# yhlleo/DWC-GAN

Hardware: AMD Instinct MI355X
Metric: CelebA 128x128 training images/sec (higher is better)
Workload: dtype f32; 1 GPU; BASELINE configs[1]: CelebA-shaped 128x128, per-GPU batch 16, fp32, full iteration (dis_update + gen_update + EMA + LR step), vgg_w=0, stride-1 3x3 / 5x5 and stride-2 4x4 layers (forward, data and weight gradient) as fp32-accurate TWO-plane f16 split products on the f16 MFMA (hi + lo 2^-11 per operand, per-tensor power-of-two scales, 3 products per multiply-add, matrix-core partial sums flushed to; image_size=128, per_gpu_batch=16, global_batch=16, parallelism=dp1

## Files before the change

dwc-gan_amd/csrc/conv_fold.h:

```cpp
#pragma once
#include "conv_geom.h"

namespace {

__device__ __forceinline__ int reflect_src(int p, int n, int pad, int (&out)[3]) {
    int c = 0;
    out[c++] = p + pad;
    if (p >= 1 && p <= pad) out[c++] = pad - p;
    if (p >= n - 1 - pad && p <= n - 2) out[c++] = pad + 2 * (n - 1) - p;
    return c;
}

template <typename T>
__global__ void fold_reflect_kernel(const T* __restrict__ gp, T* __restrict__ dx, int B, int H, int W, int C4, int pad,
                                    int Wp) {
    const size_t idx = (size_t)blockIdx.x * blockDim.x + threadIdx.x;
    const size_t total = (size_t)B * H * W * C4;
    if (idx >= total) return;
    const int c = idx % C4;
    size_t r = idx / C4;
    const int w = r % W;
    r /= W;
    const int h = r % H;
    const int n = r / H;
    const int Hp = H + 2 * pad;
    int hs[3], ws[3];
    const int nh = reflect_src(h, H, pad, hs), nw = reflect_src(w, W, pad, ws);
    f32x4 s = {0.f, 0.f, 0.f, 0.f};
    for (int a = 0; a < nh; ++a)
        for (int b = 0; b < nw; ++b) s += ld4(gp, ((size_t)(n * Hp + hs[a]) * Wp + ws[b]) * C4 + c);
    st4(dx, idx, s);
}

template <typename T>
int fold_reflect(const T* gp, T* dx, int B, int H, int W, int C4, int pad, int Wp, hipStream_t st) {
    const size_t total = (size_t)B * H * W * C4;
    hipLaunchKernelGGL(fold_reflect_kernel<T>, dim3((unsigned)((total + 255) / 256)), dim3(256), 0, st, gp, dx, B, H, W, C4, pad, Wp);
    DWC_LAUNCH_CHECK();
    return DWC_OK;
}

template <typename T>
__global__ __launch_bounds__(256) void fold_band_kernel(const T* __restrict__ gp, T* __restrict__ dx, int B, int H, int W, int CV,
                                                        int pad, int Wp) {
    constexpr int V = VecOf<T>::V;
    const size_t idx = (size_t)blockIdx.x * 256 + threadIdx.x;
    const int rows_done = 2 * pad, rest = H - 2 * pad;
    const int band = rows_done * W + rest * 2 * pad;
    const size_t total = (size_t)B * band * CV;
    if (idx >= total) return;
    const int c = idx % CV;
    size_t r = idx / CV;
    const int q = r % band;
    const size_t n = r / band;
    const int Hp = H + 2 * pad;
    int h, w;
    if (q < rows_done * W) {
        const int br = q / W;
        w = q - br * W;
        h = br < pad ? 1 + br : H - 1 - pad + (br - pad);
    } else {
        const int q2 = q - rows_done * W;
        const int hr = q2 / (2 * pad), k = q2 - hr * 2 * pad;
        h = hr == 0 ? 0 : (hr == rest - 1 ? H - 1 : pad + hr);
        w = k < pad ? 1 + k : W - 1 - pad + (k - pad);
    }
    int hs[3], ws[3];
    const int nh = reflect_src(h, H, pad, hs), nw = reflect_src(w, W, pad, ws);
    if (nh * nw == 1) return;
    const size_t o = ((n * H + h) * (size_t)W + w) * CV + c;
    float s[V], v[V];
    ldv(dx, o, s);
    for (int a = 0; a < nh; ++a)
        for (int b = 0; b < nw; ++b) {
            if (a == 0 && b == 0) continue;
            ldv(gp, ((n * Hp + hs[a]) * (size_t)Wp + ws[b]) * CV + c, v);
#pragma unroll
            for (int k = 0; k < V; ++k) s[k] += v[k];
        }
    stv(dx, o, s);
}

template <typename T>
int fold_band(const T* gp, T* dx, int B, int H, int W, int C, int pad, hipStream_t st) {
    const int CV = C / VecOf<T>::V;
    const size_t band_items = (size_t)B * (2 * pad * W + (H - 2 * pad) * 2 * pad) * CV;
    hipLaunchKernelGGL(fold_band_kernel<T>, dim3((unsigned)((band_items + 255) / 256)), dim3(256), 0, st, gp, dx, B, H, W, CV, pad,
                       W + 2 * pad);
    DWC_LAUNCH_CHECK();
    return DWC_OK;
}

template <typename T>
__global__ void fold_ring_kernel(T* __restrict__ dx, const float* __restrict__ ring, size_t off_bottom, size_t off_left,
                                 size_t off_right, int parts, size_t part_stride, int B, int H, int W, int C4, int pad) {
    const size_t idx = (size_t)blockIdx.x * blockDim.x + threadIdx.x;
    const int band = 2 * pad * (W + H);
    const size_t total = (size_t)B * band * C4;
    if (idx >= total) return;
    const int c = idx % C4;
    size_t r = idx / C4;
    const int q = r % band;
    const int n = r / band;
    int h, w;
    if (q < 2 * pad * W) {
        const int br = q / W;
        w = q - br * W;
        h = br < pad ? 1 + br : H - 1 - pad + (br - pad);
    } else {
        const int q2 = q - 2 * pad * W, bc = q2 / H;
        h = q2 - bc * H;
        w = bc < pad ? 1 + bc : W - 1 - pad + (bc - pad);
        if ((h >= 1 && h <= pad) || (h >= H - 1 - pad && h <= H - 2)) return;
    }
    if (h < 0 || h >= H || w < 0 || w >= W) return;
    const int Wp = W + 2 * pad;
    int hs[3], ws[3];
    const int nh = reflect_src(h, H, pad, hs), nw = reflect_src(w, W, pad, ws);
    const size_t o = ((size_t)(n * H + h) * W + w) * C4 + c;
    f32x4 s = ld4(dx, o);
    for (int a = 0; a < nh; ++a)
        for (int b = 0; b < nw; ++b) {
            if (a == 0 && b == 0) continue;
            const int rh = hs[a], rw = ws[b];
            size_t e;
            if (rh < pad) e = ((size_t)(n * pad + rh) * Wp + rw) * C4;
            else if (rh >= pad + H) e = off_bottom / 4 + ((size_t)(n * pad + rh - pad - H) * Wp + rw) * C4;
            else if (rw < pad) e = off_left / 4 + ((size_t)(n * H + rh - pad) * pad + rw) * C4;
            else e = off_right / 4 + ((size_t)(n * H + rh - pad) * pad + rw - pad - W) * C4;
            for (int p = 0; p < parts; ++p) s += ld4(ring + p * part_stride, e + c);
        }
    st4(dx, o, s);
}

template <typename T>
int fold_ring(T* dx, const float* ring, const SameDgrad& f, int B, int H, int W, int C, int pad, hipStream_t st) {
    const size_t total = (size_t)B * 2 * pad * (W + H) * (C / 4);
    hipLaunchKernelGGL(fold_ring_kernel<T>, dim3((unsigned)((total + 255) / 256)), dim3(256), 0, st, dx, ring, f.ring_elems[0],
                       f.ring_elems[0] + f.ring_elems[1], f.ring_elems[0] + f.ring_elems[1] + f.ring_elems[2], f.parts, f.ring_total,
                       B, H, W, C / 4, pad);
    DWC_LAUNCH_CHECK();
    return DWC_OK;
}

template <typename T>
__global__ __launch_bounds__(256) void splitk_reduce_kernel(const float* __restrict__ part, T* __restrict__ dst,
                                                            const float* __restrict__ bias, size_t total4, size_t stride4, int splits,
                                                            int N, int act) {
    const int nq = N >> 2;
    for (size_t i = (size_t)blockIdx.x * blockDim.x + threadIdx.x; i < total4; i += (size_t)gridDim.x * blockDim.x) {
        f32x4 s = ld4(part, i);
        for (int z = 1; z < splits; ++z) s += ld4(part, (size_t)z * stride4 + i);
        const int c4 = i % nq;
        if (bias) s += ld4(bias, c4);
#pragma unroll
        for (int k = 0; k < 4; ++k) s[k] = dwc_act_apply(s[k], act, c4 * 4 + k);
        st4(dst, i, s);
    }
}

template <typename T>
int splitk_reduce(const float* part, T* dst, const float* bias, size_t dst_elems, int splits, int N, int act, hipStream_t st) {
    const size_t total4 = dst_elems / 4;
    size_t blocks = (total4 + 255) / 256;
    if (blocks > 2048) blocks = 2048;
    hipLaunchKernelGGL(splitk_reduce_kernel<T>, dim3((unsigned)blocks), dim3(256), 0, st, part, dst, bias, total4, total4, splits, N, act);
    DWC_LAUNCH_CHECK();
    return DWC_OK;
}

template <typename T>
__global__ void weight_prepare_fwd_kernel(const float* __restrict__ w, T* __restrict__ out, int Cout, int Cin, int KHW,
                                          int cout_pad, int cin_pad, int Kp) {
    const size_t idx = (size_t)blockIdx.x * blockDim.x + threadIdx.x;
    if (idx >= (size_t)cout_pad * Kp) return;
    const int k = idx % Kp, co = idx / Kp;
    const int ci = k % cin_pad, tap = k / cin_pad;
    float v = 0.f;
    if (co < Cout && ci < Cin && tap < KHW) v = w[((size_t)co * Cin + ci) * KHW + tap];
    out[idx] = (T)v;
}

template <typename T>
__global__ void weight_prepare_dgrad_kernel(const float* __restrict__ w, T* __restrict__ out, int Cout, int Cin, int KH, int KW,
                                            int stride, int cout_pad, int cin_pad, int Kp) {
    const size_t idx = (size_t)blockIdx.x * blockDim.x + threadIdx.x;
    const size_t per_class = (size_t)cin_pad * Kp;
    const int classes = stride == 1 ? 1 : 4;
    if (idx >= per_class * classes) return;
    const int cls = idx / per_class;
    const size_t r = idx % per_class;
    const int k = r % Kp, ci = r / Kp;
    const int co = k % cout_pad, tapo = k / cout_pad;
    int kh, kw;
    bool ok = co < Cout && ci < Cin;
    if (stride == 1) {
        ok = ok && tapo < KH * KW;
        kh = KH - 1 - tapo / KW;
        kw = KW - 1 - tapo % KW;
    } else {
        ok = ok && tapo < 4;
        kh = (cls >> 1) + 2 * (tapo >> 1);
        kw = (cls & 1) + 2 * (tapo & 1);
    }
    out[idx] = (T)(ok ? w[((size_t)co * Cin + ci) * KH * KW + kh * KW + kw] : 0.f);
}

inline int weight_prepared_kp(int taps, int c_pad, int bk) { return (taps * c_pad + bk - 1) / bk * bk; }

inline size_t weight_prepared_elems(int KH, int KW, int stride, int cout_pad, int cin_pad, int for_dgrad, int bk) {
    if (!for_dgrad) return (size_t)cout_pad * weight_prepared_kp(KH * KW, cin_pad, bk);
    if (stride == 1) return (size_t)cin_pad * weight_prepared_kp(KH * KW, cout_pad, bk);
    return (size_t)4 * cin_pad * weight_prepared_kp(4, cout_pad, bk);
}

template <typename T>
int weight_prepare_fwd(const float* w, T* out, int Cout, int Cin, int KH, int KW, int cout_pad, int cin_pad, int bk, hipStream_t st) {
    const int Kp = weight_prepared_kp(KH * KW, cin_pad, bk);
    const size_t total = (size_t)cout_pad * Kp;
    hipLaunchKernelGGL(weight_prepare_fwd_kernel<T>, dim3((unsigned)((total + 255) / 256)), dim3(256), 0, st, w, out, Cout, Cin, KH * KW,
                       cout_pad, cin_pad, Kp);
    DWC_LAUNCH_CHECK();
    return DWC_OK;
}

template <typename T>
int weight_prepare_dgrad(const float* w, T* out, int Cout, int Cin, int KH, int KW, int stride, int cout_pad, int cin_pad, int bk,
                         hipStream_t st) {
    const int Kp = weight_prepared_kp(stride == 1 ? KH * KW : 4, cout_pad, bk);
    const size_t total = (size_t)(stride == 1 ? 1 : 4) * cin_pad * Kp;
    hipLaunchKernelGGL(weight_prepare_dgrad_kernel<T>, dim3((unsigned)((total + 255) / 256)), dim3(256), 0, st, w, out, Cout, Cin, KH, KW,
                       stride, cout_pad, cin_pad, Kp);
    DWC_LAUNCH_CHECK();
    return DWC_OK;
}

}
```

dwc-gan_amd/csrc/conv_igemm.hip:

```cpp
#include <type_traits>

#include <atomic>

#include "conv_im2col_entry.h"

namespace {

constexpr int BK = 32;


__device__ __attribute__((aligned(16))) float g_zero_page[64];

#ifdef DWC_CLOCK_PROBE
__device__ unsigned long long g_clock_probe[2];
struct ClockProbe {
    long long c0, r0;
    __device__ ClockProbe() : c0(clock64()), r0(wall_clock64()) {}
    __device__ ~ClockProbe() {
        if (blockIdx.x == 0 && blockIdx.y == 0 && blockIdx.z == 0 && threadIdx.x == 0) {
            atomicAdd(&g_clock_probe[0], (unsigned long long)(clock64() - c0));
            atomicAdd(&g_clock_probe[1], (unsigned long long)(wall_clock64() - r0));
        }
    }
};
#define DWC_PROBE() ClockProbe clock_probe_
#else
#define DWC_PROBE()
#endif

__device__ __forceinline__ void lds_dma_barrier() {
    asm volatile("s_waitcnt vmcnt(0)" ::: "memory");
    __syncthreads();
}

typedef __bf16 gx3_bf16x8 __attribute__((ext_vector_type(8)));
typedef unsigned gx3_u32x4 __attribute__((ext_vector_type(4)));

__device__ __forceinline__ void gx3_split8(const f32x4& a, const f32x4& b, gx3_bf16x8& p0, gx3_bf16x8& p1, gx3_bf16x8& p2) {
    unsigned h[8], m[8], l[8];
#pragma unroll
    for (int k = 0; k < 8; ++k) {
        const float v = k < 4 ? a[k] : b[k - 4];
        const unsigned hb = __float_as_uint(v) & 0xffff0000u;
        const float r = v - __uint_as_float(hb);
        const unsigned mb = __float_as_uint(r) & 0xffff0000u;
        const float q = r - __uint_as_float(mb);
        h[k] = hb; m[k] = mb; l[k] = __float_as_uint(q);
    }
    gx3_u32x4 u0, u1, u2;
#pragma unroll
    for (int k = 0; k < 4; ++k) {
        u0[k] = __builtin_amdgcn_perm(h[2 * k + 1], h[2 * k], 0x07060302u);
        u1[k] = __builtin_amdgcn_perm(m[2 * k + 1], m[2 * k], 0x07060302u);
        u2[k] = __builtin_amdgcn_perm(l[2 * k + 1], l[2 * k], 0x07060302u);
    }
    p0 = __builtin_bit_cast(gx3_bf16x8, u0);
    p1 = __builtin_bit_cast(gx3_bf16x8, u1);
    p2 = __builtin_bit_cast(gx3_bf16x8, u2);
}

template <int BM, int BN, int WM, int WN, int TM, int TN, bool X3 = false>
__device__ __forceinline__ void conv_gemm_body(const Gather& g, const float* __restrict__ wmat, const Scatter& o,
                                               const float* __restrict__ bias, int act, int tiles_n, int kt0, int kt1_in,
                                               size_t part_offset, bool partial, int oph, int opw, int bid, int nb) {
    static_assert(WM * WN == 4 && WM * TM * 32 == BM && WN * TN * 32 == BN, "tile shape");
    constexpr int A_PASSES = BM / 32, B_PASSES = BN / 32;
    constexpr int A_TILE = BM * BK, B_TILE = BN * BK;
    __shared__ __attribute__((aligned(16))) float smem[2 * (A_TILE + B_TILE)];
    float* sA = smem;
    float* sB = smem + 2 * A_TILE;

    const int t = threadIdx.x;
    const int lane = t & 63, wave = __builtin_amdgcn_readfirstlane(t >> 6);
    const int wm = wave / WN, wn = wave % WN;
    const int l31 = lane & 31, hi = lane >> 5;

    if (nb >= 16) {
        const int q = nb >> 3, r = nb & 7, x = bid & 7, y = bid >> 3;
        bid = (x < r ? x * (q + 1) : r * (q + 1) + (x - r) * q) + y;
    }
    const int tile_m = bid / tiles_n, tile_n = bid % tiles_n;
    const int m0 = tile_m * BM, n0 = tile_n * BN;

    const int arow = t >> 3;
    const int acol = (((t & 7) ^ ((arow >> 1) & 7))) * 4;
    int a_bh[A_PASSES], a_bw[A_PASSES], a_img[A_PASSES];
    const int ohw = g.OH * g.OW;
#pragma unroll
    for (int i = 0; i < A_PASSES; ++i) {
        const int mm = min(m0 + arow + 32 * i, g.M - 1);
        const int n = mm / ohw;
        const int rem = mm - n * ohw;
        const int oh = rem / g.OW, ow = rem - oh * g.OW;
        a_bh[i] = oh * g.mul_h + g.off_h;
        a_bw[i] = ow * g.mul_w + g.off_w;
        a_img[i] = n * g.SH * g.SW;
    }
    const int Kp = (g.K + BK - 1) / BK * BK;
    const float* b_ptr[B_PASSES];
#pragma unroll
    for (int p = 0; p < B_PASSES; ++p) b_ptr[p] = wmat + (size_t)min(n0 + arow + 32 * p, o.N - 1) * Kp + acol;

    const int nk_all = Kp / BK;
    const int kt1 = min(nk_all, kt1_in);
    const int n_taps = g.KH * g.KW;

    int cur_tap = -1;
    const float* a_src[A_PASSES];
    const bool tap_uniform = g.SC >= BK;
    auto row_sources = [&](int tap, int ci) {
        int kh = (tap * g.kw_magic) >> 16;
        int kw = tap - kh * g.KW;
        if (g.tap_t) {
            const int x = kh;
            kh = kw;
            kw = x;
        }
#pragma unroll
        for (int i = 0; i < A_PASSES; ++i) {
            int h = a_bh[i] + kh * g.kstep;
            int w = a_bw[i] + kw * g.kstep;
            bool inb = true;
            if (g.reflect) {
                h = reflect_idx(h, g.SH);
                w = reflect_idx(w, g.SW);
            } else {
                inb = h >= 0 && h < g.SH && w >= 0 && w < g.SW;
                h = min(max(h, 0), g.SH - 1);
                w = min(max(w, 0), g.SW - 1);
            }
            const float* p = (const float*)g.src + ((a_img[i] + h * g.SW + w) << g.logSC) + ci;
            a_src[i] = inb ? p : g_zero_page;
        }
    };
    auto stage_slab = [&](int kt, int buf) {
        int coff;
        if (tap_uniform) {
            const int kg0 = kt * BK;
            const int tap = min(kg0 >> g.logSC, n_taps - 1);
            if (tap != cur_tap) {
                row_sources(tap, acol);
                cur_tap = tap;
            }
            coff = kg0 & (g.SC - 1);
        } else {
            const int kg = kt * BK + acol;
            row_sources(min(kg >> g.logSC, n_taps - 1), kg & (g.SC - 1));
            coff = 0;
        }
        float* la = sA + buf * A_TILE + wave * (8 * BK);
        float* lb = sB + buf * B_TILE + wave * (8 * BK);
#pragma unroll
        for (int i = 0; i < A_PASSES; ++i) {
            const float* s = a_src[i];
            if (s != g_zero_page) s += coff;
            __builtin_amdgcn_global_load_lds((const __attribute__((address_space(1))) void*)s,
                                             (__attribute__((address_space(3))) void*)(la + i * 32 * BK), 16, 0, 0);
        }
#pragma unroll
        for (int p = 0; p < B_PASSES; ++p)
            __builtin_amdgcn_global_load_lds((const __attribute__((address_space(1))) void*)(b_ptr[p] + kt * BK),
                                             (__attribute__((address_space(3))) void*)(lb + p * 32 * BK), 16, 0, 0);
    };

    f32x16 acc[TM][TN];
#pragma unroll
    for (int i = 0; i < TM; ++i)
#pragma unroll
        for (int j = 0; j < TN; ++j)
#pragma unroll
            for (int r = 0; r < 16; ++r) acc[i][j][r] = 0.f;

    const int fsw = (l31 >> 1) & 7;
    int frag_off[4];
#pragma unroll
    for (int q = 0; q < 4; ++q) frag_off[q] = ((2 * q + hi) ^ fsw) * 4;
    const int a_row = (wm * TM * 32 + l31) * BK;
    const int b_row = (wn * TN * 32 + l31) * BK;
    f32x4 fa[2][TM], fb[2][TN];
    auto load_frags = [&](int set, int buf, int q) {
        const float* a = sA + buf * A_TILE + a_row + frag_off[q];
        const float* b = sB + buf * B_TILE + b_row + frag_off[q];
#pragma unroll
        for (int i = 0; i < TM; ++i) fa[set][i] = *reinterpret_cast<const f32x4*>(a + i * 32 * BK);
#pragma unroll
        for (int n = 0; n < TN; ++n) fb[set][n] = *reinterpret_cast<const f32x4*>(b + n * 32 * BK);
    };
    auto mfma_group = [&](int set) {
#pragma unroll
        for (int j = 0; j < 4; ++j)
#pragma unroll
            for (int i = 0; i < TM; ++i)
#pragma unroll
                for (int n = 0; n < TN; ++n)
                    acc[i][n] = __builtin_amdgcn_mfma_f32_32x32x2f32(fa[set][i][j], fb[set][n][j], acc[i][n], 0, 0, 0);
    };

    if constexpr (X3) {
        static_assert(TM * TN <= 2, "split accumulators: at most two 32x32 tiles per wave");
        f32x16 lo[TM][TN];
#pragma unroll
        for (int i = 0; i < TM; ++i)
#pragma unroll
            for (int j = 0; j < TN; ++j)
#pragma unroll
                for (int r = 0; r < 16; ++r) lo[i][j][r] = 0.f;
        int xoff[2][2];
#pragma unroll
        for (int ss = 0; ss < 2; ++ss)
#pragma unroll
            for (int e = 0; e < 2; ++e) xoff[ss][e] = ((4 * ss + 2 * hi + e) ^ fsw) * 4;
        gx3_bf16x8 pa[3][TM], pb[3][TN];
        auto frags_x3 = [&](int buf, int ss) {
            const float* a = sA + buf * A_TILE + a_row;
            const float* b = sB + buf * B_TILE + b_row;
#pragma unroll
            for (int i = 0; i < TM; ++i)
                gx3_split8(*reinterpret_cast<const f32x4*>(a + i * 32 * BK + xoff[ss][0]),
                           *reinterpret_cast<const f32x4*>(a + i * 32 * BK + xoff[ss][1]), pa[0][i], pa[1][i], pa[2][i]);
#pragma unroll
            for (int n = 0; n < TN; ++n)
                gx3_split8(*reinterpret_cast<const f32x4*>(b + n * 32 * BK + xoff[ss][0]),
                           *reinterpret_cast<const f32x4*>(b + n * 32 * BK + xoff[ss][1]), pb[0][n], pb[1][n], pb[2][n]);
        };
        auto mfma_x3 = [&]() {
            constexpr int TA[6] = {0, 1, 0, 2, 1, 0}, TB[6] = {0, 0, 1, 0, 1, 2};
#pragma unroll
            for (int term = 0; term < 6; ++term)
#pragma unroll
                for (int i = 0; i < TM; ++i)
#pragma unroll
                    for (int n = 0; n < TN; ++n) {
                        if (term == 0) acc[i][n] = __builtin_amdgcn_mfma_f32_32x32x16_bf16(pa[TA[term]][i], pb[TB[term]][n], acc[i][n], 0, 0, 0);
                        else lo[i][n] = __builtin_amdgcn_mfma_f32_32x32x16_bf16(pa[TA[term]][i], pb[TB[term]][n], lo[i][n], 0, 0, 0);
                    }
        };
        if (kt0 < kt1) {
            stage_slab(kt0, 0);
            lds_dma_barrier();
            int buf = 0;
            for (int kt = kt0; kt < kt1; ++kt) {
                if (kt + 1 < kt1) stage_slab(kt + 1, buf ^ 1);
                frags_x3(buf, 0);
                mfma_x3();
                frags_x3(buf, 1);
                lds_dma_barrier();
                mfma_x3();
                buf ^= 1;
            }
        }
#pragma unroll
        for (int i = 0; i < TM; ++i)
#pragma unroll
            for (int j = 0; j < TN; ++j)
#pragma unroll
                for (int r = 0; r < 16; ++r) acc[i][j][r] += lo[i][j][r];
    } else if (kt0 < kt1) {
        stage_slab(kt0, 0);
        lds_dma_barrier();
        int buf = 0;
        load_frags(0, 0, 0);
        for (int kt = kt0; kt < kt1; ++kt) {
            const bool more = kt + 1 < kt1;
            if (more) stage_slab(kt + 1, buf ^ 1);
            load_frags(1, buf, 1);
            mfma_group(0);
            load_frags(0, buf, 2);
            mfma_group(1);
            load_frags(1, buf, 3);
            mfma_group(0);
            lds_dma_barrier();
            if (more) load_frags(0, buf ^ 1, 0);
            mfma_group(1);
            buf ^= 1;
        }
    }

    float* dst = (float*)o.dst + part_offset;
    const float slope = dwc_act_slope(act);
    float bcol[TN];
#pragma unroll
    for (int n = 0; n < TN; ++n) bcol[n] = 0.f;
    if (bias && !partial) {
#pragma unroll
        for (int n = 0; n < TN; ++n) bcol[n] = bias[min(n0 + (wn * TN + n) * 32 + l31, o.N - 1)];
    }
    auto store = [&](auto general) {
#pragma unroll
        for (int i = 0; i < TM; ++i) {
#pragma unroll
            for (int r = 0; r < 16; ++r) {
                const int row = (wm * TM + i) * 32 + (r & 3) + 8 * (r >> 2) + 4 * hi;
                const int m = m0 + row;
                if (m >= g.M) continue;
                const int n_img = m / ohw;
                const int rem = m - n_img * ohw;
                const int oh = rem / g.OW, ow = rem - oh * g.OW;
                const int py = oh * o.os + oph, px = ow * o.os + opw;
                float* drow = dst + (((size_t)n_img * o.OHf + py) * o.OWf + px) * o.N;
                if (o.crop && !partial) {
                    const int yy = py - o.crop, xx = px - o.crop;
                    if ((unsigned)yy < (unsigned)o.IH && (unsigned)xx < (unsigned)o.IW)
                        drow = (float*)o.inner + (((size_t)n_img * o.IH + yy) * o.IW + xx) * o.N;
                }
#pragma unroll
                for (int n = 0; n < TN; ++n) {
                    const int col = n0 + (wn * TN + n) * 32 + l31;
                    if (col < o.N) {
                        float v = acc[i][n][r];
                        if (!partial) {
                            v += bcol[n];
                            if constexpr (decltype(general)::value) v = dwc_act_apply(v, act, col);
                            else v = dwc_act_simple(v, slope);
                        }
                        drow[col] = v;
                    }
                }
            }
        }
    };
    if (dwc_act_is_simple(act)) store(std::false_type{});
    else store(std::true_type{});
}

template <int BM, int BN, int WM, int WN, int TM, int TN, bool X3 = false>
__global__ __launch_bounds__(256) void conv_gemm_kernel(Gather g, const float* __restrict__ wmat, size_t w_class_stride,
                                                             Scatter o, const float* __restrict__ bias, int act, int tiles_n,
                                                             int kt_per_split, size_t part_stride) {
    DWC_PROBE();
    const int cls = blockIdx.z, split = blockIdx.y;
    conv_gemm_body<BM, BN, WM, WN, TM, TN, X3>(g, wmat + (size_t)cls * w_class_stride, o, bias, act, tiles_n, split * kt_per_split,
                                           (split + 1) * kt_per_split, (size_t)split * part_stride, part_stride != 0, cls >> 1,
                                           cls & 1, blockIdx.x, gridDim.x);
}

template <int BM, int BN, int WM, int WN, int TM, int TN, bool X3 = false>
__global__ __launch_bounds__(256) void conv_gemm_strips_kernel(StripSet ss) {
    const Strip& s = ss.s[blockIdx.z];
    if ((int)blockIdx.x >= s.tiles) return;
    const int kt0 = s.kt0 + blockIdx.y * ss.kt_per_part;
    conv_gemm_body<BM, BN, WM, WN, TM, TN, X3>(s.g, (const float*)s.w, s.o, nullptr, DWC_ACT_NONE, s.tiles_n, kt0, min(s.kt1, kt0 + ss.kt_per_part),
                                           blockIdx.y * ss.part_stride, false, s.oph, s.opw, blockIdx.x, s.tiles);
}

template <int BN, int WM, int WN, int TM, int TN, bool X3 = false>
__global__ __launch_bounds__(256) void conv_wgrad_kernel(Gather g, const float* __restrict__ dy, int N, float* __restrict__ slab,
                                                         int m_chunk, int splits_per_class = 0, size_t src_class_stride = 0,
                                                         size_t dy_class_stride = 0) {
    static_assert(WM * WN == 4 && WM * TM * 32 == 128 && WN * TN * 32 == BN, "tile shape");
    DWC_PROBE();
    constexpr int A_TILE = 32 * 128, B_TILE = 32 * BN;
    __shared__ __attribute__((aligned(16))) float smem[2 * (A_TILE + B_TILE)];
    float* sA = smem;
    float* sB = smem + 2 * A_TILE;
    const int t = threadIdx.x;
    const int lane = t & 63, wave = t >> 6;
    const int wm = wave / WN, wn = wave % WN;
    const int l31 = lane & 31, hi = lane >> 5;
    const int k0 = blockIdx.x * 128, n0 = blockIdx.y * BN;
    int split = blockIdx.z;
    if (splits_per_class > 0) {
        const int cls = blockIdx.z / splits_per_class;
        split = blockIdx.z - cls * splits_per_class;
        g.src = (const float*)g.src + (size_t)cls * src_class_stride;
        dy += (size_t)cls * dy_class_stride;
    }
    const int m_begin = split * m_chunk;
    const int m_end = min(g.M, m_begin + m_chunk);

    const int kg = k0 + (t & 31) * 4;
    const int tap = min(kg >> g.logSC, g.KH * g.KW - 1);
    const int ci = kg & (g.SC - 1);
    const int kh = (tap * g.kw_magic) >> 16;
    const int kw = tap - kh * g.KW;
    const int dh = kh * g.kstep + g.off_h, dw = kw * g.kstep + g.off_w;
    const int arow = t >> 5;
    constexpr int B_F4 = BN / 4;
    constexpr int B_ROWS_PER_PASS = 256 / B_F4;
    constexpr int B_PASSES = 32 / B_ROWS_PER_PASS;
    const int brow = t / B_F4, bcol = (t % B_F4) * 4;
    const int ohw = g.OH * g.OW;

    const int bcol_c = min(n0 + bcol, N - 4);
    const int wave_u = __builtin_amdgcn_readfirstlane(wave);
    auto stage_slab = [&](int mb, int buf) {
        float* la = sA + buf * A_TILE + wave_u * 256;
        float* lb = sB + buf * B_TILE + wave_u * 256;
#pragma unroll
        for (int i = 0; i < 4; ++i) {
            const int m = min(mb + arow + 8 * i, g.M - 1);
            int n, oh, ow;
            if (g.logOW >= 0) {
                n = m >> g.logOHW;
                const int rem = m & (ohw - 1);
                oh = rem >> g.logOW;
                ow = rem & (g.OW - 1);
            } else {
                n = m / ohw;
                const int rem = m - n * ohw;
                oh = rem / g.OW;
                ow = rem - oh * g.OW;
            }
            const int h = reflect_idx(oh * g.mul_h + dh, g.SH);
            const int w = reflect_idx(ow * g.mul_w + dw, g.SW);
            const float* s = (const float*)g.src + (((n * g.SH + h) * g.SW + w) << g.logSC) + ci;
            __builtin_amdgcn_global_load_lds((const __attribute__((address_space(1))) void*)s,
                                             (__attribute__((address_space(3))) void*)(la + i * 8 * 128), 16, 0, 0);
        }
#pragma unroll
        for (int p = 0; p < B_PASSES; ++p) {
            const int m = mb + brow + p * B_ROWS_PER_PASS;
            const float* s = m < m_end ? dy + (size_t)m * N + bcol_c : g_zero_page;
            __builtin_amdgcn_global_load_lds((const __attribute__((address_space(1))) void*)s,
                                             (__attribute__((address_space(3))) void*)(lb + p * B_ROWS_PER_PASS * BN), 16, 0, 0);
        }
    };

    f32x16 acc[TM][TN];
#pragma unroll
    for (int i = 0; i < TM; ++i)
#pragma unroll
        for (int j = 0; j < TN; ++j)
#pragma unroll
            for (int r = 0; r < 16; ++r) acc[i][j][r] = 0.f;

    float av[2][4][TM], bv[2][4][TN];
    auto load_ops = [&](int set, int buf, int grp) {
        const float* a = sA + buf * A_TILE + (wm * TM) * 32 + l31;
        const float* b = sB + buf * B_TILE + (wn * TN) * 32 + l31;
#pragma unroll
        for (int s = 0; s < 4; ++s) {
            const int ml = 2 * (4 * grp + s) + hi;
#pragma unroll
            for (int i = 0; i < TM; ++i) av[set][s][i] = a[ml * 128 + i * 32];
#pragma unroll
            for (int n = 0; n < TN; ++n) bv[set][s][n] = b[ml * BN + n * 32];
        }
    };
    auto mfma_ops = [&](int set) {
#pragma unroll
        for (int s = 0; s < 4; ++s)
#pragma unroll
            for (int i = 0; i < TM; ++i)
#pragma unroll
                for (int n = 0; n < TN; ++n)
                    acc[i][n] = __builtin_amdgcn_mfma_f32_32x32x2f32(av[set][s][i], bv[set][s][n], acc[i][n], 0, 0, 0);
    };
    if constexpr (X3) {
        f32x16 lo[TM][TN];
#pragma unroll
        for (int i = 0; i < TM; ++i)
#pragma unroll
            for (int j = 0; j < TN; ++j)
#pragma unroll
                for (int r = 0; r < 16; ++r) lo[i][j][r] = 0.f;
        gx3_bf16x8 pa[3][TM], pb[3][TN];
        auto ops_x3 = [&](int buf, int ss) {
            const float* a = sA + buf * A_TILE + (wm * TM) * 32 + l31 + (16 * ss + 8 * hi) * 128;
            const float* b = sB + buf * B_TILE + (wn * TN) * 32 + l31 + (16 * ss + 8 * hi) * BN;
#pragma unroll
            for (int i = 0; i < TM; ++i)
                gx3_split8(f32x4{a[i * 32], a[128 + i * 32], a[2 * 128 + i * 32], a[3 * 128 + i * 32]},
                           f32x4{a[4 * 128 + i * 32], a[5 * 128 + i * 32], a[6 * 128 + i * 32], a[7 * 128 + i * 32]}, pa[0][i], pa[1][i],
                           pa[2][i]);
#pragma unroll
            for (int n = 0; n < TN; ++n)
                gx3_split8(f32x4{b[n * 32], b[BN + n * 32], b[2 * BN + n * 32], b[3 * BN + n * 32]},
                           f32x4{b[4 * BN + n * 32], b[5 * BN + n * 32], b[6 * BN + n * 32], b[7 * BN + n * 32]}, pb[0][n], pb[1][n],
                           pb[2][n]);
        };
        auto mfma_x3 = [&]() {
            constexpr int TA[6] = {0, 1, 0, 2, 1, 0}, TB[6] = {0, 0, 1, 0, 1, 2};
#pragma unroll
            for (int term = 0; term < 6; ++term)
#pragma unroll
                for (int i = 0; i < TM; ++i)
#pragma unroll
                    for (int n = 0; n < TN; ++n) {
                        if (term == 0) acc[i][n] = __builtin_amdgcn_mfma_f32_32x32x16_bf16(pa[TA[term]][i], pb[TB[term]][n], acc[i][n], 0, 0, 0);
                        else lo[i][n] = __builtin_amdgcn_mfma_f32_32x32x16_bf16(pa[TA[term]][i], pb[TB[term]][n], lo[i][n], 0, 0, 0);
                    }
        };
        if (m_begin < m_end) {
            stage_slab(m_begin, 0);
            lds_dma_barrier();
            int buf = 0;
            for (int mb = m_begin; mb < m_end; mb += 32) {
                if (mb + 32 < m_end) stage_slab(mb + 32, buf ^ 1);
                ops_x3(buf, 0);
                mfma_x3();
                ops_x3(buf, 1);
                lds_dma_barrier();
                mfma_x3();
                buf ^= 1;
            }
        }
#pragma unroll
        for (int i = 0; i < TM; ++i)
#pragma unroll
            for (int j = 0; j < TN; ++j)
#pragma unroll
                for (int r = 0; r < 16; ++r) acc[i][j][r] += lo[i][j][r];
    } else if (m_begin < m_end) {
        stage_slab(m_begin, 0);
        lds_dma_barrier();
        int buf = 0;
        load_ops(0, 0, 0);
        for (int mb = m_begin; mb < m_end; mb += 32) {
            const bool more = mb + 32 < m_end;
            if (more) stage_slab(mb + 32, buf ^ 1);
            load_ops(1, buf, 1);
            mfma_ops(0);
            load_ops(0, buf, 2);
            mfma_ops(1);
            load_ops(1, buf, 3);
            mfma_ops(0);
            lds_dma_barrier();
            if (more) load_ops(0, buf ^ 1, 0);
            mfma_ops(1);
            buf ^= 1;
        }
    }
    float* out = slab + (size_t)blockIdx.z * g.K * N;
#pragma unroll
    for (int i = 0; i < TM; ++i)
#pragma unroll
        for (int r = 0; r < 16; ++r) {
            const int k = k0 + (wm * TM + i) * 32 + (r & 3) + 8 * (r >> 2) + 4 * hi;
            if (k >= g.K) continue;
#pragma unroll
            for (int n = 0; n < TN; ++n) {
                const int col = n0 + (wn * TN + n) * 32 + l31;
                if (col < N) out[(size_t)k * N + col] = acc[i][n][r];
            }
        }
}


template <int BM, int BN, int WM, int WN, int TM, int TN, bool X3 = false>
void launch_variant(const Gather& g, const float* w, size_t wcs, int classes, const Scatter& o, const float* bias, int act,
                    const Plan& p, size_t part_stride, hipStream_t st) {
    const int tiles_m = (g.M + BM - 1) / BM, tiles_n = (o.N + BN - 1) / BN;
    hipLaunchKernelGGL((conv_gemm_kernel<BM, BN, WM, WN, TM, TN, X3>), dim3(tiles_m * tiles_n, p.splits, classes), dim3(256), 0, st,
                       g, w, wcs, o, bias, act, tiles_n, p.kt_per_split, part_stride);
}

static std::atomic<int> g_x3_mode{-1};
static int x3_mode() {
    int m = g_x3_mode.load(std::memory_order_relaxed);
    if (m < 0) {
        const int a = getenv("DWC_X3_GEMM") ? atoi(getenv("DWC_X3_GEMM")) : 1;
        const int b = getenv("DWC_X3_WGRAD") ? atoi(getenv("DWC_X3_WGRAD")) : 1;
        m = (a ? 1 : 0) | (b ? 2 : 0);
        g_x3_mode.store(m, std::memory_order_relaxed);
    }
    return m;
}
static bool wgrad_x3_on() { return (x3_mode() & 2) != 0; }
static bool gemm_x3_on(int K) { return (x3_mode() & 1) != 0 && K >= 128; }

struct Im2colF32 {
    typedef float T;
    static constexpr int BK = ::BK;
    static constexpr int MIN_LOG_C = 2;
    static constexpr int CH_MASK = 3;
    static constexpr bool HALF_STRIPS = false;
    static constexpr int WGRAD_SLAB_ROWS = 32;
    static constexpr int IMAGE_PX = 8;
    static constexpr int IMAGE_GROUPS = 1;
    static constexpr TileCand TILES[] = {{128, 128, 2, 1.0f}, {128, 64, 3, 0.85f}, {64, 64, 5, 0.72f}, {128, 32, 4, 0.5f}};
    static constexpr int SPLIT_BELOW = 2 * NUM_CU;

    static int launch_gemm(const Gather& g, const float* w, size_t w_class_stride, int classes, Scatter o, const float* bias, int act,
                           size_t dst_elems, void* ws, size_t ws_bytes, hipStream_t st) {
        Plan p = im2col_plan<Im2colF32>(g.M, o.N, g.K, classes);
        float* final_dst = (float*)o.dst;
        size_t part_stride = 0;
        if (p.splits > 1) {
            if (!ws || ws_bytes < gemm_ws_bytes(p, dst_elems)) {
                p.splits = 1;
                p.kt_per_split = (g.K + BK - 1) / BK;
            } else {
                o.dst = (float*)ws;
                part_stride = dst_elems;
            }
        }
        if (gemm_x3_on(g.K)) {
            if (p.bm == 128 && p.bn >= 64) launch_variant<128, 64, 2, 2, 2, 1, true>(g, w, w_class_stride, classes, o, bias, act, p, part_stride, st);
            else if (p.bm == 64 && p.bn == 64) launch_variant<64, 64, 2, 2, 1, 1, true>(g, w, w_class_stride, classes, o, bias, act, p, part_stride, st);
            else launch_variant<128, 32, 4, 1, 1, 1, true>(g, w, w_class_stride, classes, o, bias, act, p, part_stride, st);
        } else if (p.bm == 128 && p.bn == 128) launch_variant<128, 128, 2, 2, 2, 2>(g, w, w_class_stride, classes, o, bias, act, p, part_stride, st);
        else if (p.bm == 128 && p.bn == 64) launch_variant<128, 64, 2, 2, 2, 1>(g, w, w_class_stride, classes, o, bias, act, p, part_stride, st);
        else if (p.bm == 64 && p.bn == 64) launch_variant<64, 64, 2, 2, 1, 1>(g, w, w_class_stride, classes, o, bias, act, p, part_stride, st);
        else launch_variant<128, 32, 4, 1, 1, 1>(g, w, w_class_stride, classes, o, bias, act, p, part_stride, st);
        DWC_LAUNCH_CHECK();
        if (p.splits > 1) return splitk_reduce((const float*)ws, final_dst, bias, dst_elems, p.splits, o.N, act, st);
        return DWC_OK;
    }

    static int launch_strips(const StripSet& ss, int bm, dim3 grid, hipStream_t st, bool ) {
        if (bm != 64) return DWC_EINVAL;
        if (gemm_x3_on(ss.s[0].g.K)) hipLaunchKernelGGL((conv_gemm_strips_kernel<64, 64, 2, 2, 1, 1, true>), grid, dim3(256), 0, st, ss);
        else hipLaunchKernelGGL((conv_gemm_strips_kernel<64, 64, 2, 2, 1, 1>), grid, dim3(256), 0, st, ss);
        DWC_LAUNCH_CHECK();
        return DWC_OK;
    }

    static int wgrad_launch(const FwdGeom& f, const float* dy, float* dw_oihw, int Cin, int Cout, int KHW, int cin_real, int cout_real,
                            void* ws, size_t ws_bytes, hipStream_t st) {
        const Gather& g = f.g;
        int splits, chunk;
        if (!ws || ws_bytes < wgrad_ws_bytes(g.M, g.K, Cout, WGRAD_SLAB_ROWS, &splits, &chunk)) return DWC_EWORKSPACE;
        float* slab = (float*)ws;
        const int tk = (g.K + 127) / 128;
        if (wgrad_x3_on()) {
            if (Cout > 64)
                hipLaunchKernelGGL((conv_wgrad_kernel<128, 2, 2, 2, 2, true>), dim3(tk, (Cout + 127) / 128, splits), dim3(256), 0, st, g, dy,
                                   Cout, slab, chunk);
            else if (Cout > 32)
                hipLaunchKernelGGL((conv_wgrad_kernel<64, 2, 2, 2, 1, true>), dim3(tk, 1, splits), dim3(256), 0, st, g, dy, Cout, slab, chunk);
            else
                hipLaunchKernelGGL((conv_wgrad_kernel<32, 4, 1, 1, 1, true>), dim3(tk, 1, splits), dim3(256), 0, st, g, dy, Cout, slab, chunk);
        } else if (Cout > 64) {
            hipLaunchKernelGGL((conv_wgrad_kernel<128, 2, 2, 2, 2>), dim3(tk, (Cout + 127) / 128, splits), dim3(256), 0, st, g, dy,
                               Cout, slab, chunk);
        } else if (Cout > 32) {
            hipLaunchKernelGGL((conv_wgrad_kernel<64, 2, 2, 2, 1>), dim3(tk, 1, splits), dim3(256), 0, st, g, dy, Cout, slab, chunk);
        } else {
            hipLaunchKernelGGL((conv_wgrad_kernel<32, 4, 1, 1, 1>), dim3(tk, 1, splits), dim3(256), 0, st, g, dy, Cout, slab, chunk);
        }
        DWC_LAUNCH_CHECK();
        wgrad_reduce(slab, dw_oihw, splits, g.K, Cout, Cin, KHW, cin_real, cout_real, st);
        DWC_LAUNCH_CHECK();
        return DWC_OK;
    }

    static int fold_image(const float* dxp, float* dx, int B, int H, int W, int C, int pad, hipStream_t st) {
        return fold_reflect(dxp, dx, B, H, W, C / 4, pad, W + 2 * pad, st);
    }

    static bool band_args_bad(const void* dxp, const void* dx, int , int , int C) { return !dxp || !dx || C <= 0; }
};

}

#define DWC_F32_NAME(x) dwc_##x
DWC_IM2COL_EXPORTS(DWC_F32_NAME, Im2colF32, float)
#undef DWC_F32_NAME

extern "C" {

int dwc_version(void) { return DWC_ABI_VERSION; }

int dwc_x3_gemm_mode(int mode) {
    const int prev = x3_mode();
    if (mode >= 0) g_x3_mode.store(mode & 3, std::memory_order_relaxed);
    return prev;
}

int dwc_reflect_pad_adjoint_pitch(const float* dxp, float* dx, int B, int H, int W, int C, int pad, int pitch, void* stream) {
    if (B <= 0 || H <= 0 || W <= 0 || C <= 0 || (C & 3) || pad < 0 || pad >= H || pad >= W || pitch < W + 2 * pad) return DWC_EINVAL;
    return fold_reflect(dxp, dx, B, H, W, C / 4, pad, pitch, (hipStream_t)stream);
}

}

#ifdef DWC_CLOCK_PROBE
extern "C" int dwc_debug_clock_probe(unsigned long long* out, int reset) {
    if (hipMemcpyFromSymbol(out, HIP_SYMBOL(g_clock_probe), 16) != hipSuccess) return DWC_ELAUNCH;
    if (reset) {
        const unsigned long long z[2] = {0, 0};
        if (hipMemcpyToSymbol(HIP_SYMBOL(g_clock_probe), z, 16) != hipSuccess) return DWC_ELAUNCH;
    }
    return 0;
}
#endif
```

dwc-gan_amd/csrc/conv_im2col_entry.h:

```cpp
#pragma once
#include "conv_fold.h"

namespace {

template <class P>
Plan im2col_plan(int M, int N, int K, int classes) {
    return plan_gemm(M, N, K, classes, P::BK, P::TILES, P::SPLIT_BELOW);
}

template <class P>
size_t im2col_weight_prepared_elems(int Cout, int Cin, int KH, int KW, int stride, int cout_pad, int cin_pad, int for_dgrad) {
    return weight_prepared_elems(KH, KW, stride, cout_pad, cin_pad, for_dgrad, P::BK);
}

template <class P>
int im2col_weight_prepare_fwd(const float* w, void* out, int Cout, int Cin, int KH, int KW, int cout_pad, int cin_pad, void* stream) {
    if (cout_pad < Cout || cin_pad < Cin) return DWC_EINVAL;
    return weight_prepare_fwd(w, (typename P::T*)out, Cout, Cin, KH, KW, cout_pad, cin_pad, P::BK, (hipStream_t)stream);
}

template <class P>
int im2col_weight_prepare_dgrad(const float* w, void* out, int Cout, int Cin, int KH, int KW, int stride, int cout_pad, int cin_pad,
                                void* stream) {
    if (cout_pad < Cout || cin_pad < Cin) return DWC_EINVAL;
    if (stride == 2 && !(KH == 4 && KW == 4)) return DWC_EINVAL;
    if (stride != 1 && stride != 2) return DWC_EINVAL;
    return weight_prepare_dgrad(w, (typename P::T*)out, Cout, Cin, KH, KW, stride, cout_pad, cin_pad, P::BK, (hipStream_t)stream);
}

template <class P>
size_t im2col_fwd_ws_bytes(int B, int H, int W, int Cin, int Cout, int KH, int KW, int stride, int pad) {
    FwdGeom f;
    if (!fwd_geom(nullptr, nullptr, B, H, W, Cin, Cout, KH, KW, stride, pad, &f, P::MIN_LOG_C)) return 0;
    return gemm_ws_bytes(im2col_plan<P>(f.g.M, Cout, f.g.K, 1), f.dst_elems);
}

template <class P>
int im2col_fwd(const void* x, const void* w_prepared, const float* bias, void* y, int B, int H, int W, int Cin, int Cout, int KH,
               int KW, int stride, int pad, int act, void* ws, size_t ws_bytes, void* stream, int reflect) {
    FwdGeom f;
    if ((Cout & P::CH_MASK) || !fwd_geom(x, y, B, H, W, Cin, Cout, KH, KW, stride, pad, &f, P::MIN_LOG_C)) return DWC_EINVAL;
    f.g.reflect = reflect;
    return P::launch_gemm(f.g, (const typename P::T*)w_prepared, 0, 1, f.o, bias, act, f.dst_elems, ws, ws_bytes, (hipStream_t)stream);
}

template <class P>
int im2col_fwd_ex(const void* x, const void* w_prepared, const float* bias, void* y, int B, int H, int W, int Cin, int Cout, int KH,
                  int KW, int stride_h, int stride_w, int pad_h, int pad_w, int act, void* stream) {
    FwdGeom f;
    if ((Cout & P::CH_MASK) || !fwd_geom_ex(x, y, B, H, W, Cin, Cout, KH, KW, stride_h, stride_w, pad_h, pad_w, &f, P::MIN_LOG_C))
        return DWC_EINVAL;
    return P::launch_gemm(f.g, (const typename P::T*)w_prepared, 0, 1, f.o, bias, act, f.dst_elems, nullptr, 0, (hipStream_t)stream);
}

template <class P>
size_t im2col_bwd_data_zeropad_ws_bytes(int B, int H, int W, int Cin, int Cout, int KH, int KW, int pad) {
    FwdGeom f;
    if ((Cin & P::CH_MASK) || (Cout & P::CH_MASK) || !zeropad_dgrad_geom(nullptr, nullptr, B, H, W, Cin, Cout, KH, KW, pad, &f)) return 0;
    return gemm_ws_bytes(im2col_plan<P>(f.g.M, Cin, f.g.K, 1), f.dst_elems);
}

template <class P>
int im2col_bwd_data_zeropad(const void* dy, const void* w_dgrad, void* dx, int B, int H, int W, int Cin, int Cout, int KH, int KW,
                            int pad, void* ws, size_t ws_bytes, void* stream) {
    FwdGeom f;
    if ((Cin & P::CH_MASK) || (Cout & P::CH_MASK) || !zeropad_dgrad_geom(dy, dx, B, H, W, Cin, Cout, KH, KW, pad, &f)) return DWC_EINVAL;
    return P::launch_gemm(f.g, (const typename P::T*)w_dgrad, 0, 1, f.o, nullptr, DWC_ACT_NONE, f.dst_elems, ws, ws_bytes,
                          (hipStream_t)stream);
}

template <class P>
size_t im2col_bwd_data_ws_bytes(int B, int H, int W, int Cin, int Cout, int KH, int KW, int stride, int pad) {
    BwdGeom f;
    if (!bwd_geom(nullptr, nullptr, B, H, W, Cin, Cout, KH, KW, stride, pad, &f, P::BK, P::MIN_LOG_C)) return 0;
    return gemm_ws_bytes(im2col_plan<P>(f.g.M, Cin, f.g.K, f.classes), f.dst_elems);
}

template <class P>
int im2col_bwd_data(const void* dy, const void* w_dgrad, void* dxp, int B, int H, int W, int Cin, int Cout, int KH, int KW, int stride,
                    int pad, void* ws, size_t ws_bytes, void* stream) {
    BwdGeom f;
    if ((Cin & P::CH_MASK) || !bwd_geom(dy, dxp, B, H, W, Cin, Cout, KH, KW, stride, pad, &f, P::BK, P::MIN_LOG_C)) return DWC_EINVAL;
    return P::launch_gemm(f.g, (const typename P::T*)w_dgrad, f.wcs, f.classes, f.o, nullptr, DWC_ACT_NONE, f.dst_elems, ws, ws_bytes,
                          (hipStream_t)stream);
}

template <class P>
int im2col_reflect_pad_adjoint(const void* dxp, void* dx, int B, int H, int W, int C, int pad, void* stream) {
    if (B <= 0 || H <= 0 || W <= 0 || C <= 0 || (C & 3) || pad < 0 || pad >= H || pad >= W) return DWC_EINVAL;
    return P::fold_image((const typename P::T*)dxp, (typename P::T*)dx, B, H, W, C, pad, (hipStream_t)stream);
}

template <class P>
int im2col_reflect_pad_adjoint_band(const void* dxp, void* dx, int B, int H, int W, int C, int pad, void* stream) {
    if (P::band_args_bad(dxp, dx, B, H, C) || B <= 0 || (C & P::CH_MASK) || pad <= 0 || H < 2 * pad + 2 || W < 2 * pad + 2)
        return DWC_EINVAL;
    return fold_band((const typename P::T*)dxp, (typename P::T*)dx, B, H, W, C, pad, (hipStream_t)stream);
}

template <class P>
int im2col_bwd_data_fold(const void* dy, const void* w_dgrad, void* dxp, void* dx, int B, int H, int W, int Cin, int Cout, int KH,
                         int KW, int stride, int pad, void* ws, size_t ws_bytes, void* stream) {
    BwdGeom f;
    if ((Cin & P::CH_MASK) || pad <= 0 || !bwd_geom(dy, dxp, B, H, W, Cin, Cout, KH, KW, stride, pad, &f, P::BK, P::MIN_LOG_C))
        return DWC_EINVAL;
    if (H < 2 * pad + 2 || W < 2 * pad + 2 || H > 65535 - 2 * pad || B > 65535) return DWC_EINVAL;
    hipStream_t st = (hipStream_t)stream;
    const bool direct = im2col_plan<P>(f.g.M, f.o.N, f.g.K, f.classes).splits == 1;
    if (direct) {
        f.o.crop = pad; f.o.IH = H; f.o.IW = W; f.o.inner = dx;
    }
    const int rc = P::launch_gemm(f.g, (const typename P::T*)w_dgrad, f.wcs, f.classes, f.o, nullptr, DWC_ACT_NONE, f.dst_elems, ws,
                                  ws_bytes, st);
    if (rc != DWC_OK) return rc;
    if (!direct) return im2col_reflect_pad_adjoint<P>(dxp, dx, B, H, W, Cin, pad, stream);
    return fold_band((const typename P::T*)dxp, (typename P::T*)dx, B, H, W, Cin, pad, st);
}

template <class P>
size_t im2col_bwd_data_same_ws_bytes(int B, int H, int W, int Cin, int Cout, int KH, int KW, int pad) {
    SameDgrad f;
    if (!same_dgrad_geom(nullptr, nullptr, nullptr, nullptr, nullptr, B, H, W, Cin, Cout, KH, KW, pad, &f, P::BK, P::HALF_STRIPS)) return 0;
    const size_t ring = (f.ring_total * f.parts * sizeof(float) + 255) / 256 * 256;
    return ring + gemm_ws_bytes(im2col_plan<P>(f.g.M, Cin, f.g.K, 1), f.dst_elems);
}

template <class P>
int im2col_bwd_data_same(const void* dy, const void* w_dgrad, const void* w_dgrad_t, void* dx, int B, int H, int W, int Cin, int Cout,
                         int KH, int KW, int pad, void* ws, size_t ws_bytes, void* stream, bool ring_only) {
    SameDgrad f;
    if ((Cin & P::CH_MASK) ||
        !same_dgrad_geom(dy, w_dgrad, w_dgrad_t, dx, (float*)ws, B, H, W, Cin, Cout, KH, KW, pad, &f, P::BK, P::HALF_STRIPS))
        return DWC_EINVAL;
    const size_t ring_bytes = (f.ring_total * f.parts * sizeof(float) + 255) / 256 * 256;
    if (!ws || ws_bytes < ring_bytes) return DWC_EWORKSPACE;
    hipStream_t st = (hipStream_t)stream;
    if (!ring_only) {
        const int rc = P::launch_gemm(f.g, (const typename P::T*)w_dgrad, 0, 1, f.o, nullptr, DWC_ACT_NONE, f.dst_elems,
                                      (char*)ws + ring_bytes, ws_bytes - ring_bytes, st);
        if (rc != DWC_OK) return rc;
    }
    const int rc = P::launch_strips(f.ss, f.bm, dim3(f.max_tiles, f.parts, 4), st, true);
    if (rc != DWC_OK) return rc;
    return fold_ring((typename P::T*)dx, (const float*)ws, f, B, H, W, Cin, pad, st);
}

template <class P>
int im2col_bwd_data_s2_ring(const void* dy, const void* w_dgrad, void* dxp, void* dx, int B, int H, int W, int Cin, int Cout,
                            void* stream) {
    S2Ring f;
    if (!dy || !w_dgrad || !dxp || !dx || (Cin & P::CH_MASK) || H > 65535 - 2 || B > 65535 ||
        !s2_ring_geom(dy, w_dgrad, dxp, sizeof(typename P::T), B, H, W, Cin, Cout, &f, P::BK, P::MIN_LOG_C, P::HALF_STRIPS))
        return DWC_EINVAL;
    hipStream_t st = (hipStream_t)stream;
    const int rc = P::launch_strips(f.ss, f.bm, dim3(f.max_tiles, 1, 8), st, false);
    if (rc != DWC_OK) return rc;
    return fold_band((const typename P::T*)dxp, (typename P::T*)dx, B, H, W, Cin, 1, st);
}

template <class P>
size_t im2col_bwd_data_image_ws_bytes(int B, int H, int W, int Cout, int KH, int KW, int pad) {
    FwdGeom f;
    if (!image_dgrad_geom(nullptr, nullptr, B, H, W, Cout, KH, KW, pad, &f, P::IMAGE_PX)) return 0;
    return f.dst_elems * sizeof(typename P::T);
}

template <class P>
int im2col_bwd_data_image(const void* dy, const void* w_wide, void* dx, int B, int H, int W, int Cout, int KH, int KW, int pad, void* ws,
                          size_t ws_bytes, void* stream) {
    FwdGeom f;
    if (!image_dgrad_geom(dy, ws, B, H, W, Cout, KH, KW, pad, &f, P::IMAGE_PX)) return DWC_EINVAL;
    if (!ws || ws_bytes < f.dst_elems * sizeof(typename P::T)) return DWC_EWORKSPACE;
    const int rc = P::launch_gemm(f.g, (const typename P::T*)w_wide, 0, 1, f.o, nullptr, DWC_ACT_NONE, f.dst_elems, nullptr, 0,
                                  (hipStream_t)stream);
    if (rc != DWC_OK) return rc;
    return fold_reflect((const typename P::T*)ws, (typename P::T*)dx, B, H, W, P::IMAGE_GROUPS, pad, f.g.OW * P::IMAGE_PX,
                        (hipStream_t)stream);
}

template <class P>
size_t im2col_bwd_weight_ws_bytes(int B, int H, int W, int Cin, int Cout, int KH, int KW, int stride, int pad) {
    const int Ho = (H + 2 * pad - KH) / stride + 1, Wo = (W + 2 * pad - KW) / stride + 1;
    int splits, chunk;
    return wgrad_ws_bytes(B * Ho * Wo, KH * KW * Cin, Cout, P::WGRAD_SLAB_ROWS, &splits, &chunk);
}

template <class P>
int im2col_bwd_weight(const void* x, const void* dy, float* dw_oihw, int B, int H, int W, int Cin, int Cout, int KH, int KW, int stride,
                      int pad, int cin_real, int cout_real, void* ws, size_t ws_bytes, void* stream) {
    FwdGeom f;
    if (!fwd_geom(x, nullptr, B, H, W, Cin, Cout, KH, KW, stride, pad, &f, P::MIN_LOG_C)) return DWC_EINVAL;
    if (cin_real > Cin || cout_real > Cout || (Cout & P::CH_MASK)) return DWC_EINVAL;
    return P::wgrad_launch(f, (const typename P::T*)dy, dw_oihw, Cin, Cout, KH * KW, cin_real, cout_real, ws, ws_bytes,
                           (hipStream_t)stream);
}

template <class P>
size_t im2col_bwd_weight_ex_ws_bytes(int B, int H, int W, int Cin, int Cout, int KH, int KW, int stride_h, int stride_w, int pad_h,
                                     int pad_w) {
    FwdGeom f;
    if (!fwd_geom_ex(nullptr, nullptr, B, H, W, Cin, Cout, KH, KW, stride_h, stride_w, pad_h, pad_w, &f, P::MIN_LOG_C)) return 0;
    int splits, chunk;
    return wgrad_ws_bytes(f.g.M, f.g.K, Cout, P::WGRAD_SLAB_ROWS, &splits, &chunk);
}

template <class P>
int im2col_bwd_weight_ex(const void* x, const void* dy, float* dw_oihw, int B, int H, int W, int Cin, int Cout, int KH, int KW,
                         int stride_h, int stride_w, int pad_h, int pad_w, int cin_real, int cout_real, void* ws, size_t ws_bytes,
                         void* stream) {
    FwdGeom f;
    if (!fwd_geom_ex(x, nullptr, B, H, W, Cin, Cout, KH, KW, stride_h, stride_w, pad_h, pad_w, &f, P::MIN_LOG_C)) return DWC_EINVAL;
    if (cin_real > Cin || cout_real > Cout || (Cout & P::CH_MASK)) return DWC_EINVAL;
    return P::wgrad_launch(f, (const typename P::T*)dy, dw_oihw, Cin, Cout, KH * KW, cin_real, cout_real, ws, ws_bytes,
                           (hipStream_t)stream);
}

}

#define DWC_IM2COL_EXPORTS(NAME, P, X)                                                                                                   \
    extern "C" {                                                                                                                         \
    size_t NAME(weight_prepared_elems)(int Cout, int Cin, int KH, int KW, int stride, int cout_pad, int cin_pad, int for_dgrad) {        \
        return im2col_weight_prepared_elems<P>(Cout, Cin, KH, KW, stride, cout_pad, cin_pad, for_dgrad);                                 \
    }                                                                                                                                    \
    int NAME(weight_prepare_fwd)(const float* w, X* out, int Cout, int Cin, int KH, int KW, int cout_pad, int cin_pad, void* stream) {   \
        return im2col_weight_prepare_fwd<P>(w, out, Cout, Cin, KH, KW, cout_pad, cin_pad, stream);                                       \
    }                                                                                                                                    \
    int NAME(weight_prepare_dgrad)(const float* w, X* out, int Cout, int Cin, int KH, int KW, int stride, int cout_pad, int cin_pad,     \
                                   void* stream) {                                                                                       \
        return im2col_weight_prepare_dgrad<P>(w, out, Cout, Cin, KH, KW, stride, cout_pad, cin_pad, stream);                             \
    }                                                                                                                                    \
    size_t NAME(conv2d_fwd_ws_bytes)(int B, int H, int W, int Cin, int Cout, int KH, int KW, int stride, int pad) {                      \
        return im2col_fwd_ws_bytes<P>(B, H, W, Cin, Cout, KH, KW, stride, pad);                                                          \
    }                                                                                                                                    \
    int NAME(conv2d_fwd)(const X* x, const X* w, const float* bias, X* y, int B, int H, int W, int Cin, int Cout, int KH, int KW,        \
                         int stride, int pad, int act, void* ws, size_t ws_bytes, void* stream) {                                        \
        return im2col_fwd<P>(x, w, bias, y, B, H, W, Cin, Cout, KH, KW, stride, pad, act, ws, ws_bytes, stream, 1);                      \
    }                                                                                                                                    \
    int NAME(conv2d_fwd_zeropad)(const X* x, const X* w, const float* bias, X* y, int B, int H, int W, int Cin, int Cout, int KH,        \
                                 int KW, int stride, int pad, int act, void* ws, size_t ws_bytes, void* stream) {                        \
        return im2col_fwd<P>(x, w, bias, y, B, H, W, Cin, Cout, KH, KW, stride, pad, act, ws, ws_bytes, stream, 0);                      \
    }                                                                                                                                    \
    int NAME(conv2d_fwd_ex)(const X* x, const X* w, const float* bias, X* y, int B, int H, int W, int Cin, int Cout, int KH, int KW,     \
                            int stride_h, int stride_w, int pad_h, int pad_w, int act, void* stream) {                                   \
        return im2col_fwd_ex<P>(x, w, bias, y, B, H, W, Cin, Cout, KH, KW, stride_h, stride_w, pad_h, pad_w, act, stream);               \
    }                                                                                                                                    \
    size_t NAME(conv2d_bwd_data_zeropad_ws_bytes)(int B, int H, int W, int Cin, int Cout, int KH, int KW, int pad) {                     \
        return im2col_bwd_data_zeropad_ws_bytes<P>(B, H, W, Cin, Cout, KH, KW, pad);                                                     \
    }                                                                                                                                    \
    int NAME(conv2d_bwd_data_zeropad)(const X* dy, const X* w, X* dx, int B, int H, int W, int Cin, int Cout, int KH, int KW, int pad,   \
                                      void* ws, size_t ws_bytes, void* stream) {                                                         \
        return im2col_bwd_data_zeropad<P>(dy, w, dx, B, H, W, Cin, Cout, KH, KW, pad, ws, ws_bytes, stream);                             \
    }                                                                                                                                    \
    size_t NAME(conv2d_bwd_data_ws_bytes)(int B, int H, int W, int Cin, int Cout, int KH, int KW, int stride, int pad) {                 \
        return im2col_bwd_data_ws_bytes<P>(B, H, W, Cin, Cout, KH, KW, stride, pad);                                                     \
    }                                                                                                                                    \
    int NAME(conv2d_bwd_data)(const X* dy, const X* w, X* dxp, int B, int H, int W, int Cin, int Cout, int KH, int KW, int stride,       \
                              int pad, void* ws, size_t ws_bytes, void* stream) {                                                        \
        return im2col_bwd_data<P>(dy, w, dxp, B, H, W, Cin, Cout, KH, KW, stride, pad, ws, ws_bytes, stream);                            \
    }                                                                                                                                    \
    int NAME(reflect_pad_adjoint)(const X* dxp, X* dx, int B, int H, int W, int C, int pad, void* stream) {                              \
        return im2col_reflect_pad_adjoint<P>(dxp, dx, B, H, W, C, pad, stream);                                                          \
    }                                                                                                                                    \
    int NAME(reflect_pad_adjoint_band)(const X* dxp, X* dx, int B, int H, int W, int C, int pad, void* stream) {                         \
        return im2col_reflect_pad_adjoint_band<P>(dxp, dx, B, H, W, C, pad, stream);                                                     \
    }                                                                                                                                    \
    int NAME(conv2d_bwd_data_fold)(const X* dy, const X* w, X* dxp, X* dx, int B, int H, int W, int Cin, int Cout, int KH, int KW,       \
                                   int stride, int pad, void* ws, size_t ws_bytes, void* stream) {                                       \
        return im2col_bwd_data_fold<P>(dy, w, dxp, dx, B, H, W, Cin, Cout, KH, KW, stride, pad, ws, ws_bytes, stream);                   \
    }                                                                                                                                    \
    size_t NAME(conv2d_bwd_data_same_ws_bytes)(int B, int H, int W, int Cin, int Cout, int KH, int KW, int pad) {                        \
        return im2col_bwd_data_same_ws_bytes<P>(B, H, W, Cin, Cout, KH, KW, pad);                                                        \
    }                                                                                                                                    \
    int NAME(conv2d_bwd_data_same)(const X* dy, const X* w, const X* w_t, X* dx, int B, int H, int W, int Cin, int Cout, int KH, int KW, \
                                   int pad, void* ws, size_t ws_bytes, void* stream) {                                                   \
        return im2col_bwd_data_same<P>(dy, w, w_t, dx, B, H, W, Cin, Cout, KH, KW, pad, ws, ws_bytes, stream, false);                    \
    }                                                                                                                                    \
    int NAME(conv2d_bwd_data_ring)(const X* dy, const X* w, const X* w_t, X* dx, int B, int H, int W, int Cin, int Cout, int KH, int KW, \
                                   int pad, void* ws, size_t ws_bytes, void* stream) {                                                   \
        return im2col_bwd_data_same<P>(dy, w, w_t, dx, B, H, W, Cin, Cout, KH, KW, pad, ws, ws_bytes, stream, true);                     \
    }                                                                                                                                    \
    int NAME(conv2d_bwd_data_s2_ring)(const X* dy, const X* w, X* dxp, X* dx, int B, int H, int W, int Cin, int Cout, void* stream) {    \
        return im2col_bwd_data_s2_ring<P>(dy, w, dxp, dx, B, H, W, Cin, Cout, stream);                                                   \
    }                                                                                                                                    \
    size_t NAME(conv2d_bwd_data_image_ws_bytes)(int B, int H, int W, int Cout, int KH, int KW, int pad) {                                \
        return im2col_bwd_data_image_ws_bytes<P>(B, H, W, Cout, KH, KW, pad);                                                            \
    }                                                                                                                                    \
    int NAME(conv2d_bwd_data_image)(const X* dy, const X* w, X* dx, int B, int H, int W, int Cout, int KH, int KW, int pad, void* ws,    \
                                    size_t ws_bytes, void* stream) {                                                                     \
        return im2col_bwd_data_image<P>(dy, w, dx, B, H, W, Cout, KH, KW, pad, ws, ws_bytes, stream);                                    \
    }                                                                                                                                    \
    size_t NAME(conv2d_bwd_weight_ws_bytes)(int B, int H, int W, int Cin, int Cout, int KH, int KW, int stride, int pad) {               \
        return im2col_bwd_weight_ws_bytes<P>(B, H, W, Cin, Cout, KH, KW, stride, pad);                                                   \
    }                                                                                                                                    \
    int NAME(conv2d_bwd_weight)(const X* x, const X* dy, float* dw, int B, int H, int W, int Cin, int Cout, int KH, int KW, int stride,  \
                                int pad, int cin_real, int cout_real, void* ws, size_t ws_bytes, void* stream) {                         \
        return im2col_bwd_weight<P>(x, dy, dw, B, H, W, Cin, Cout, KH, KW, stride, pad, cin_real, cout_real, ws, ws_bytes, stream);      \
    }                                                                                                                                    \
    size_t NAME(conv2d_bwd_weight_ex_ws_bytes)(int B, int H, int W, int Cin, int Cout, int KH, int KW, int stride_h, int stride_w,       \
                                               int pad_h, int pad_w) {                                                                   \
        return im2col_bwd_weight_ex_ws_bytes<P>(B, H, W, Cin, Cout, KH, KW, stride_h, stride_w, pad_h, pad_w);                           \
    }                                                                                                                                    \
    int NAME(conv2d_bwd_weight_ex)(const X* x, const X* dy, float* dw, int B, int H, int W, int Cin, int Cout, int KH, int KW,           \
                                   int stride_h, int stride_w, int pad_h, int pad_w, int cin_real, int cout_real, void* ws,              \
                                   size_t ws_bytes, void* stream) {                                                                      \
        return im2col_bwd_weight_ex<P>(x, dy, dw, B, H, W, Cin, Cout, KH, KW, stride_h, stride_w, pad_h, pad_w, cin_real, cout_real, ws, \
                                       ws_bytes, stream);                                                                                \
    }                                                                                                                                    \
    }
```

dwc-gan_amd/csrc/dwc_common.h:

```cpp
#pragma once
#include <hip/hip_runtime.h>
#include <stdint.h>
#include "../../include/dwcgan_hip.h"

typedef float f32x16 __attribute__((ext_vector_type(16)));
typedef float f32x4 __attribute__((ext_vector_type(4)));
typedef __bf16 dwc_bf16;
typedef __bf16 dwc_bf16x4 __attribute__((ext_vector_type(4)));
typedef __bf16 dwc_bf16x8 __attribute__((ext_vector_type(8)));

#ifdef __HIPCC__
__device__ __forceinline__ f32x4 ld4(const float* p, size_t i4) { return reinterpret_cast<const f32x4*>(p)[i4]; }
__device__ __forceinline__ f32x4 ld4(const dwc_bf16* p, size_t i4) {
    const dwc_bf16x4 v = reinterpret_cast<const dwc_bf16x4*>(p)[i4];
    return f32x4{(float)v[0], (float)v[1], (float)v[2], (float)v[3]};
}
__device__ __forceinline__ void st4(float* p, size_t i4, f32x4 v) { reinterpret_cast<f32x4*>(p)[i4] = v; }
__device__ __forceinline__ void st4(dwc_bf16* p, size_t i4, f32x4 v) {
    dwc_bf16x4 r;
    r[0] = (dwc_bf16)v[0]; r[1] = (dwc_bf16)v[1]; r[2] = (dwc_bf16)v[2]; r[3] = (dwc_bf16)v[3];
    reinterpret_cast<dwc_bf16x4*>(p)[i4] = r;
}
#endif

#ifdef __HIPCC__
template <typename T> struct VecOf { static constexpr int V = 4; };
template <> struct VecOf<dwc_bf16> { static constexpr int V = 8; };

__device__ __forceinline__ void ldv(const float* p, size_t iv, float (&o)[4]) {
    const f32x4 v = reinterpret_cast<const f32x4*>(p)[iv];
    o[0] = v[0]; o[1] = v[1]; o[2] = v[2]; o[3] = v[3];
}
__device__ __forceinline__ void ldv(const dwc_bf16* p, size_t iv, float (&o)[8]) {
    const dwc_bf16x8 v = reinterpret_cast<const dwc_bf16x8*>(p)[iv];
#pragma unroll
    for (int k = 0; k < 8; ++k) o[k] = (float)v[k];
}
__device__ __forceinline__ void stv(float* p, size_t iv, const float (&o)[4]) {
    reinterpret_cast<f32x4*>(p)[iv] = f32x4{o[0], o[1], o[2], o[3]};
}
__device__ __forceinline__ void stv(dwc_bf16* p, size_t iv, const float (&o)[8]) {
    dwc_bf16x8 r;
#pragma unroll
    for (int k = 0; k < 8; ++k) r[k] = (dwc_bf16)o[k];
    reinterpret_cast<dwc_bf16x8*>(p)[iv] = r;
}
template <int V>
__device__ __forceinline__ void ldf(const float* p, size_t e, float (&o)[V]) {
#pragma unroll
    for (int q = 0; q < V / 4; ++q) {
        const f32x4 v = reinterpret_cast<const f32x4*>(p + e)[q];
        o[4 * q] = v[0]; o[4 * q + 1] = v[1]; o[4 * q + 2] = v[2]; o[4 * q + 3] = v[3];
    }
}
template <int V>
__device__ __forceinline__ void stf(float* p, size_t e, const float (&o)[V]) {
#pragma unroll
    for (int q = 0; q < V / 4; ++q) reinterpret_cast<f32x4*>(p + e)[q] = f32x4{o[4 * q], o[4 * q + 1], o[4 * q + 2], o[4 * q + 3]};
}

#endif

#ifdef __HIPCC__
__device__ __forceinline__ void dwc_amax_publish(unsigned long long* slot, unsigned epoch, unsigned abs_bits) {
    atomicMax(slot, ((unsigned long long)epoch << 32) | abs_bits);
}
__device__ __forceinline__ unsigned dwc_abs_bits(float v) { return __float_as_uint(v) & 0x7fffffffu; }
__device__ __forceinline__ unsigned dwc_wave_max_u32(unsigned v) {
#pragma unroll
    for (int off = 32; off > 0; off >>= 1) v = max(v, (unsigned)__shfl_xor((int)v, off, 64));
    return v;
}
__device__ __forceinline__ void dwc_amax_wave_publish(unsigned long long* slot, unsigned epoch, unsigned abs_bits) {
    if (!slot) return;
    abs_bits = dwc_wave_max_u32(abs_bits);
    if ((threadIdx.x & 63) == 0) {
        const unsigned long long v = ((unsigned long long)epoch << 32) | abs_bits;
        if (*reinterpret_cast<volatile unsigned long long*>(slot) < v) atomicMax(slot, v);
    }
}
__device__ __forceinline__ void dwc_amax_block_publish(unsigned long long* slot, unsigned epoch, unsigned abs_bits, unsigned* sm) {
    if (!slot) return;
    abs_bits = dwc_wave_max_u32(abs_bits);
    if ((threadIdx.x & 63) == 0) sm[threadIdx.x >> 6] = abs_bits;
    __syncthreads();
    if (threadIdx.x == 0) {
        unsigned m = 0;
        for (unsigned w = 0; w < (blockDim.x + 63) / 64; ++w) m = max(m, sm[w]);
        const unsigned long long v = ((unsigned long long)epoch << 32) | m;
        if (*reinterpret_cast<volatile unsigned long long*>(slot) < v) atomicMax(slot, v);
    }
}
template <int V>
__device__ __forceinline__ unsigned dwc_amax_fold(unsigned am, const float (&o)[V]) {
#pragma unroll
    for (int k = 0; k < V; ++k) am = max(am, dwc_abs_bits(o[k]));
    return am;
}
struct H2Scale { float s, inv; };
__device__ __forceinline__ H2Scale h2_scale(const unsigned long long* slot, unsigned epoch) {
    const unsigned long long v = *slot;
    unsigned e = ((unsigned)v >> 23) & 0xffu;
    H2Scale r;
    if (e == 0xffu) {
        r.s = r.inv = 1.f;
    } else {
        e = min(max(e, 27u), 254u);
        r.s = __uint_as_float((267u - e) << 23);
        r.inv = __uint_as_float((e - 13u) << 23);
    }
    if ((unsigned)(v >> 32) != epoch) r.s = r.inv = __builtin_nanf("");
    return r;
}
#endif

#define DWC_LAUNCH_CHECK()                                   \
    do {                                                     \
        if (hipGetLastError() != hipSuccess) return DWC_ELAUNCH; \
    } while (0)

static inline int dwc_ilog2_exact(int v) {
    if (v <= 0 || (v & (v - 1))) return -1;
    int l = 0;
    while ((1 << l) < v) ++l;
    return l;
}

__device__ __forceinline__ float dwc_wave_sum(float v) {
#pragma unroll
    for (int off = 32; off > 0; off >>= 1) v += __shfl_xor(v, off, 64);
    return v;
}

__device__ __forceinline__ float dwc_block_sum_256(float v, float* sm) {
    v = dwc_wave_sum(v);
    const int wave = threadIdx.x >> 6;
    __syncthreads();
    if ((threadIdx.x & 63) == 0) sm[wave] = v;
    __syncthreads();
    return sm[0] + sm[1] + sm[2] + sm[3];
}

__device__ __forceinline__ float dwc_act_apply(float v, int act, int ch) {
    switch (act) {
        case DWC_ACT_RELU: return v < 0.f ? 0.f : v;
        case DWC_ACT_LRELU: return v > 0.f ? v : 0.1f * v;
        case DWC_ACT_TANH: return tanhf(v);
        case DWC_ACT_SIGMOID: return 1.f / (1.f + expf(-v));
        case DWC_ACT_HEADS: return ((ch & 3) == 3) ? 1.f / (1.f + expf(-v)) : tanhf(v);
        case DWC_ACT_HEADS8: return ((ch & 7) == 3) ? 1.f / (1.f + expf(-v)) : ((ch & 7) < 3 ? tanhf(v) : 0.f);
        default: return v;
    }
}

__device__ __forceinline__ bool dwc_act_is_simple(int act) { return act <= DWC_ACT_LRELU; }
static inline bool dwc_act_is_simple_host(int act) { return act <= DWC_ACT_LRELU; }
__device__ __forceinline__ float dwc_act_slope(int act) { return act == DWC_ACT_NONE ? 1.f : (act == DWC_ACT_RELU ? 0.f : 0.1f); }
__device__ __forceinline__ float dwc_act_simple(float v, float slope) { return v < 0.f ? (slope == 0.f ? 0.f : slope * v) : v; }

__device__ __forceinline__ float dwc_act_grad(float y, int act, int ch) {
    switch (act) {
        case DWC_ACT_RELU: return y > 0.f ? 1.f : 0.f;
        case DWC_ACT_LRELU: return y > 0.f ? 1.f : 0.1f;
        case DWC_ACT_TANH: return 1.f - y * y;
        case DWC_ACT_SIGMOID: return y * (1.f - y);
        case DWC_ACT_HEADS: return ((ch & 3) == 3) ? y * (1.f - y) : 1.f - y * y;
        case DWC_ACT_HEADS8: return ((ch & 7) == 3) ? y * (1.f - y) : ((ch & 7) < 3 ? 1.f - y * y : 0.f);
        default: return 1.f;
    }
}
```

dwc-gan_amd/csrc/weight_refresh.hip:

```cpp
#include "dwc_common.h"

namespace {

typedef __bf16 bf16;

__device__ __forceinline__ float im2col_elem(const dwc_refresh_desc& d, size_t idx, bool dgrad) {
    const float* w = d.src;
    if (!dgrad) {
        const int KHW = d.KH * d.KW;
        const int k = idx % d.Kp, co = idx / d.Kp;
        const int ci = k % d.cin_pad, tap = k / d.cin_pad;
        return (co < d.Cout && ci < d.Cin && tap < KHW) ? w[((size_t)co * d.Cin + ci) * KHW + tap] : 0.f;
    }
    const size_t per_class = (size_t)d.cin_pad * d.Kp;
    const int cls = idx / per_class;
    const size_t r = idx % per_class;
    const int k = r % d.Kp, ci = r / d.Kp;
    const int co = k % d.cout_pad, tapo = k / d.cout_pad;
    int kh, kw;
    bool ok = co < d.Cout && ci < d.Cin;
    if (d.stride == 1) {
        ok = ok && tapo < d.KH * d.KW;
        kh = d.KH - 1 - tapo / d.KW;
        kw = d.KW - 1 - tapo % d.KW;
    } else {
        ok = ok && tapo < 4;
        kh = (cls >> 1) + 2 * (tapo >> 1);
        kw = (cls & 1) + 2 * (tapo & 1);
    }
    const int off = d.transpose_hw ? kw * d.KH + kh : kh * d.KW + kw;
    return ok ? w[((size_t)co * d.Cin + ci) * d.KH * d.KW + off] : 0.f;
}

__device__ __forceinline__ float split_layout_elem(const dwc_refresh_desc& d, size_t idx, bool dgrad, int planes, size_t* base) {
    const int K = d.KH, rows = d.rows, kdim = d.kdim, CS = 16;
    const int ncs = (kdim + CS - 1) / CS;
    const int j = idx % CS;
    size_t r = idx / CS;
    const int row = r % rows;
    r /= rows;
    const int cs = r % ncs, tap = r / ncs;
    const int kh = tap / K, kw = tap - kh * K;
    const int kc = cs * CS + j;
    float v = 0.f;
    if (!dgrad) {
        if (row < d.Cout && kc < d.Cin) v = d.src[(((size_t)row * d.Cin + kc) * K + kh) * K + kw];
    } else {
        if (row < d.Cin && kc < d.Cout) v = d.src[(((size_t)kc * d.Cin + row) * K + (K - 1 - kh)) * K + (K - 1 - kw)];
    }
    *base = ((size_t)(tap * ncs + cs) * planes * rows + row) * CS + (j ^ (((row >> 3) & 1) << 3));
    return v;
}

template <bool AMAX_PASS>
__global__ __launch_bounds__(256) void weight_refresh_multi_kernel(const dwc_refresh_desc* __restrict__ descs,
                                                                   const int* __restrict__ chunk_desc,
                                                                   const unsigned* __restrict__ chunk_start, unsigned epoch) {
    const dwc_refresh_desc d = descs[chunk_desc[blockIdx.x]];
    const size_t i0 = chunk_start[blockIdx.x];
    const size_t i1 = min((size_t)d.n_items, i0 + DWC_OPT_CHUNK);
    const bool h2 = d.kind == DWC_REFRESH_H2_FWD || d.kind == DWC_REFRESH_H2_DGRAD;
    unsigned short* h2_planes = reinterpret_cast<unsigned short*>(d.dst);
    float* h2_tail = reinterpret_cast<float*>(h2_planes + 2 * d.n_items);
    unsigned long long* h2_slot = reinterpret_cast<unsigned long long*>(h2_tail + 2);
    if constexpr (AMAX_PASS) {
        if (!h2) return;
        unsigned am = 0;
        for (size_t idx = i0 + threadIdx.x; idx < i1; idx += 256) {
            size_t base;
            am = max(am, dwc_abs_bits(split_layout_elem(d, idx, d.kind == DWC_REFRESH_H2_DGRAD, 2, &base)));
        }
        dwc_amax_wave_publish(h2_slot, epoch, am);
        return;
    }
    H2Scale sw = {1.f, 1.f};
    if (h2) {
        sw = h2_scale(h2_slot, epoch);
        if (i0 == 0 && threadIdx.x == 0) h2_tail[0] = sw.s, h2_tail[1] = sw.inv;
    }
    for (size_t idx = i0 + threadIdx.x; idx < i1; idx += 256) {
        switch (d.kind) {
            case DWC_REFRESH_H2_FWD:
            case DWC_REFRESH_H2_DGRAD: {
                size_t base;
                const float v = split_layout_elem(d, idx, d.kind == DWC_REFRESH_H2_DGRAD, 2, &base) * sw.s;
                const _Float16 h = (_Float16)v;
                const _Float16 l = (_Float16)(v - (float)h);
                h2_planes[base] = __builtin_bit_cast(unsigned short, h);
                h2_planes[base + (size_t)d.rows * 16] = __builtin_bit_cast(unsigned short, l);
                break;
            }
            case DWC_REFRESH_FWD_F32: reinterpret_cast<float*>(d.dst)[idx] = im2col_elem(d, idx, false); break;
            case DWC_REFRESH_DGRAD_F32: reinterpret_cast<float*>(d.dst)[idx] = im2col_elem(d, idx, true); break;
            case DWC_REFRESH_FWD_BF16: reinterpret_cast<bf16*>(d.dst)[idx] = (bf16)im2col_elem(d, idx, false); break;
            case DWC_REFRESH_DGRAD_BF16: reinterpret_cast<bf16*>(d.dst)[idx] = (bf16)im2col_elem(d, idx, true); break;
            case DWC_REFRESH_X3_FWD:
            case DWC_REFRESH_X3_DGRAD: {
                const int K = d.KH, rows = d.rows, kdim = d.kdim, CS = 16;
                const int ncs = (kdim + CS - 1) / CS;
                const int j = idx % CS;
                size_t r = idx / CS;
                const int row = r % rows;
                r /= rows;
                const int cs = r % ncs, tap = r / ncs;
                const int kh = tap / K, kw = tap - kh * K;
                const int kc = cs * CS + j;
                float v = 0.f;
                if (d.kind == DWC_REFRESH_X3_FWD) {
                    if (row < d.Cout && kc < d.Cin) v = d.src[(((size_t)row * d.Cin + kc) * K + kh) * K + kw];
                } else {
                    if (row < d.Cin && kc < d.Cout) v = d.src[(((size_t)kc * d.Cin + row) * K + (K - 1 - kh)) * K + (K - 1 - kw)];
                }
                const unsigned hb = __float_as_uint(v) & 0xffff0000u;
                const float r1 = v - __uint_as_float(hb);
                const unsigned mb = __float_as_uint(r1) & 0xffff0000u;
                const float r2 = r1 - __uint_as_float(mb);
                unsigned short* o = reinterpret_cast<unsigned short*>(d.dst);
                const size_t base = ((size_t)(tap * ncs + cs) * 3 * rows + row) * CS + (j ^ (((row >> 3) & 1) << 3));
                o[base] = (unsigned short)(hb >> 16);
                o[base + (size_t)rows * CS] = (unsigned short)(mb >> 16);
                o[base + 2 * (size_t)rows * CS] = (unsigned short)(__float_as_uint(r2) >> 16);
                break;
            }
            default: break;
        }
    }
}

}

extern "C" {

int dwc_weight_refresh_multi(const dwc_refresh_desc* descs_dev, const int* chunk_desc_dev, const unsigned* chunk_start_dev, int n_chunks,
                             int has_h2, unsigned epoch, void* stream) {
    if (n_chunks <= 0) return DWC_OK;
    if (!descs_dev || !chunk_desc_dev || !chunk_start_dev) return DWC_EINVAL;
    if (has_h2) {
        hipLaunchKernelGGL(weight_refresh_multi_kernel<true>, dim3(n_chunks), dim3(256), 0, (hipStream_t)stream, descs_dev, chunk_desc_dev,
                           chunk_start_dev, epoch);
        DWC_LAUNCH_CHECK();
    }
    hipLaunchKernelGGL(weight_refresh_multi_kernel<false>, dim3(n_chunks), dim3(256), 0, (hipStream_t)stream, descs_dev, chunk_desc_dev,
                       chunk_start_dev, epoch);
    DWC_LAUNCH_CHECK();
    return DWC_OK;
}

}
```

dwc-gan_amd/hipdwc/_lib.py:

```python
import ctypes
import os

_HERE = os.path.dirname(os.path.abspath(__file__))
LIB_PATH = os.environ.get("DWC_HIP_LIB") or os.path.join(os.path.dirname(_HERE), "lib", "libdwcgan_hip.so")

c_fp = ctypes.c_void_p
c_int = ctypes.c_int
c_sz = ctypes.c_size_t
c_f = ctypes.c_float
c_u = ctypes.c_uint


class AdvSpec(ctypes.Structure):
    _fields_ = [("target", c_f * 4), ("w_src", c_f * 4), ("w_cls", c_f * 4)]


SIGNATURES = {
    "dwc_version": (c_int, []),
    "dwc_x3_gemm_mode": (c_int, [c_int]),
    "dwc_weight_prepared_elems": (c_sz, [c_int] * 8),
    "dwc_weight_prepare_fwd": (c_int, [c_fp, c_fp, c_int, c_int, c_int, c_int, c_int, c_int, c_fp]),
    "dwc_weight_prepare_dgrad": (c_int, [c_fp, c_fp, c_int, c_int, c_int, c_int, c_int, c_int, c_int, c_fp]),
    "dwc_conv2d_fwd_ws_bytes": (c_sz, [c_int] * 9),
    "dwc_conv2d_fwd": (c_int, [c_fp, c_fp, c_fp, c_fp] + [c_int] * 10 + [c_fp, c_sz, c_fp]),
    "dwc_conv2d_bwd_data_ws_bytes": (c_sz, [c_int] * 9),
    "dwc_conv2d_bwd_data": (c_int, [c_fp, c_fp, c_fp] + [c_int] * 9 + [c_fp, c_sz, c_fp]),
    "dwc_conv2d_bwd_data_fold": (c_int, [c_fp, c_fp, c_fp, c_fp] + [c_int] * 9 + [c_fp, c_sz, c_fp]),
    "dwc_reflect_pad_adjoint": (c_int, [c_fp, c_fp, c_int, c_int, c_int, c_int, c_int, c_fp]),
    "dwc_conv2d_bwd_data_same_ws_bytes": (c_sz, [c_int] * 8),
    "dwc_conv2d_bwd_data_same": (c_int, [c_fp] * 4 + [c_int] * 8 + [c_fp, c_sz, c_fp]),
    "dwc_conv2d_bwd_data_ring": (c_int, [c_fp] * 4 + [c_int] * 8 + [c_fp, c_sz, c_fp]),
    "dwc_conv2d_bwd_data_image_ws_bytes": (c_sz, [c_int] * 7),
    "dwc_conv2d_bwd_data_image": (c_int, [c_fp, c_fp, c_fp] + [c_int] * 7 + [c_fp, c_sz, c_fp]),
    "dwc_conv2d_fwd_zeropad": (c_int, [c_fp, c_fp, c_fp, c_fp] + [c_int] * 10 + [c_fp, c_sz, c_fp]),
    "dwc_conv2d_bwd_data_zeropad_ws_bytes": (c_sz, [c_int] * 8),
    "dwc_conv2d_bwd_data_zeropad": (c_int, [c_fp, c_fp, c_fp] + [c_int] * 8 + [c_fp, c_sz, c_fp]),
    "dwc_maxpool2_fwd": (c_int, [c_fp, c_fp, c_int, c_int, c_int, c_int, c_fp]),
    "dwc_maxpool2_bwd": (c_int, [c_fp, c_fp, c_fp, c_int, c_int, c_int, c_int, c_fp]),
    "dwc_conv2d_bwd_weight_ws_bytes": (c_sz, [c_int] * 9),
    "dwc_conv2d_bwd_weight": (c_int, [c_fp, c_fp, c_fp] + [c_int] * 11 + [c_fp, c_sz, c_fp]),
    "dwc_conv2d_fwd_ex": (c_int, [c_fp, c_fp, c_fp, c_fp] + [c_int] * 12 + [c_fp]),
    "dwc_conv2d_bwd_weight_ex_ws_bytes": (c_sz, [c_int] * 11),
    "dwc_conv2d_bwd_weight_ex": (c_int, [c_fp, c_fp, c_fp] + [c_int] * 13 + [c_fp, c_sz, c_fp]),
    "dwc_act_bwd_bias_ws_bytes": (c_sz, [c_int, c_int]),
    "dwc_act_bwd_bias": (c_int, [c_fp, c_fp, c_fp, c_fp, c_int, c_int, c_int, c_fp, c_sz, c_fp]),
    "dwc_linear_small_ok": (c_int, [c_int] * 3),
    "dwc_linear_small_fwd": (c_int, [c_fp] * 4 + [c_int] * 4 + [c_fp]),
    "dwc_linear_small_bwd": (c_int, [c_fp] * 7 + [c_int] * 3 + [c_fp]),
    "dwc_instnorm_ws_bytes": (c_sz, [c_int, c_int, c_int]),
    "dwc_instnorm_fwd": (c_int, [c_fp] * 7 + [c_int, c_int, c_int, c_f, c_int, c_fp, c_sz, c_fp]),
    "dwc_instnorm_bwd": (c_int, [c_fp] * 9 + [c_int, c_int, c_int, c_int, c_fp, c_sz, c_fp]),
    "dwc_layernorm_ws_bytes": (c_sz, [c_int, c_int, c_int]),
    "dwc_layernorm_fwd": (c_int, [c_fp] * 6 + [c_int, c_int, c_int, c_f, c_int, c_fp, c_sz, c_fp]),
    "dwc_layernorm_bwd": (c_int, [c_fp] * 9 + [c_int, c_int, c_int, c_f, c_int, c_fp, c_sz, c_fp]),
    "dwc_upsample2x_fwd": (c_int, [c_fp, c_fp, c_int, c_int, c_int, c_int, c_fp]),
    "dwc_upsample2x_bwd": (c_int, [c_fp, c_fp, c_int, c_int, c_int, c_int, c_fp]),
    "dwc_avgpool2_fwd": (c_int, [c_fp, c_fp, c_int, c_int, c_int, c_int, c_fp]),
    "dwc_avgpool2_bwd": (c_int, [c_fp, c_fp, c_int, c_int, c_int, c_int, c_fp]),
    "dwc_pack_nchw_to_nhwc4": (c_int, [c_fp, c_fp, c_int, c_int, c_int, c_int, c_fp]),
    "dwc_unpack_nhwc4_to_nchw": (c_int, [c_fp, c_fp, c_int, c_int, c_int, c_int, c_fp]),
    "dwc_blend_fwd": (c_int, [c_fp, c_fp, c_fp, c_int, c_fp]),
    "dwc_blend_bwd": (c_int, [c_fp, c_fp, c_fp, c_fp, c_int, c_fp]),
    "dwc_l1_ws_bytes": (c_sz, [c_sz]),
    "dwc_gmm_kl_sp_fwd": (c_int, [c_fp, c_fp, c_fp, c_int, c_int, c_int, c_int, c_f, c_fp, c_fp]),
    "dwc_gmm_kl_sp_bwd": (c_int, [c_fp, c_fp, c_fp, c_int, c_int, c_int, c_int, c_f, c_fp, c_fp, c_fp, c_fp]),
    "dwc_l1_mean_fwd": (c_int, [c_fp, c_fp, c_fp, c_sz, c_int, c_fp, c_sz, c_fp]),
    "dwc_l1_mean_bwd": (c_int, [c_fp, c_fp, c_fp, c_fp, c_fp, c_sz, c_int, c_fp]),
    "dwc_lstm_fwd": (c_int, [c_fp] * 6 + [c_int] * 4 + [c_fp]),
    "dwc_lstm_bwd": (c_int, [c_fp] * 8 + [c_int] * 4 + [c_fp]),
    "dwc_adam_step": (c_int, [c_fp, c_fp, c_fp, c_fp, c_sz, c_f, c_f, c_f, c_f, c_f, c_int, c_fp]),
    "dwc_ema_lerp": (c_int, [c_fp, c_fp, c_sz, c_f, c_fp]),
    "dwc_adam_multi": (c_int, [c_fp, c_fp, c_fp, c_int] + [ctypes.c_double] * 4 + [c_fp]),
    "dwc_ema_multi": (c_int, [c_fp, c_fp, c_fp, c_int, c_f, c_fp]),
    "dwc_bf16_weight_prepared_elems": (c_sz, [c_int] * 8),
    "dwc_bf16_weight_prepare_fwd": (c_int, [c_fp, c_fp, c_int, c_int, c_int, c_int, c_int, c_int, c_fp]),
    "dwc_bf16_weight_prepare_dgrad": (c_int, [c_fp, c_fp, c_int, c_int, c_int, c_int, c_int, c_int, c_int, c_fp]),
    "dwc_bf16_conv2d_fwd_ws_bytes": (c_sz, [c_int] * 9),
    "dwc_bf16_conv2d_fwd": (c_int, [c_fp, c_fp, c_fp, c_fp] + [c_int] * 10 + [c_fp, c_sz, c_fp]),
    "dwc_bf16_conv2d_fwd_ex": (c_int, [c_fp, c_fp, c_fp, c_fp] + [c_int] * 12 + [c_fp]),
    "dwc_bf16_conv2d_bwd_data_ws_bytes": (c_sz, [c_int] * 9),
    "dwc_bf16_conv2d_bwd_data": (c_int, [c_fp, c_fp, c_fp] + [c_int] * 9 + [c_fp, c_sz, c_fp]),
    "dwc_bf16_conv2d_bwd_data_fold": (c_int, [c_fp, c_fp, c_fp, c_fp] + [c_int] * 9 + [c_fp, c_sz, c_fp]),
    "dwc_bf16_reflect_pad_adjoint": (c_int, [c_fp, c_fp, c_int, c_int, c_int, c_int, c_int, c_fp]),
    "dwc_bf16_reflect_pad_adjoint_band": (c_int, [c_fp, c_fp, c_int, c_int, c_int, c_int, c_int, c_fp]),
    "dwc_bf16_conv2d_bwd_data_same_ws_bytes": (c_sz, [c_int] * 8),
    "dwc_bf16_conv2d_bwd_data_same": (c_int, [c_fp] * 4 + [c_int] * 8 + [c_fp, c_sz, c_fp]),
    "dwc_bf16_conv2d_bwd_data_ring": (c_int, [c_fp] * 4 + [c_int] * 8 + [c_fp, c_sz, c_fp]),
    "dwc_bf16_conv2d_same_halo_ok": (c_int, [c_int] * 6),
    "dwc_bf16_conv2d_same_halo": (c_int, [c_fp] * 4 + [c_int] * 8 + [c_fp]),
    "dwc_bf16_conv2d_same_halo_add": (c_int, [c_fp] * 5 + [c_int] * 8 + [c_fp]),
    "dwc_bf16_conv2d_bwd_data_same_fused_ok": (c_int, [c_int] * 6),
    "dwc_bf16_conv2d_bwd_data_same_fused": (c_int, [c_fp] * 4 + [c_int] * 6 + [c_fp]),
    "dwc_weight_refresh_multi": (c_int, [c_fp, c_fp, c_fp, c_int, c_int, c_u, c_fp]),
    "dwc_bf16_conv2d_fwd_zeropad": (c_int, [c_fp, c_fp, c_fp, c_fp] + [c_int] * 10 + [c_fp, c_sz, c_fp]),
    "dwc_bf16_conv2d_bwd_data_zeropad_ws_bytes": (c_sz, [c_int] * 8),
    "dwc_bf16_conv2d_bwd_data_zeropad": (c_int, [c_fp, c_fp, c_fp] + [c_int] * 8 + [c_fp, c_sz, c_fp]),
    "dwc_bf16_maxpool2_fwd": (c_int, [c_fp, c_fp, c_int, c_int, c_int, c_int, c_fp]),
    "dwc_bf16_maxpool2_bwd": (c_int, [c_fp, c_fp, c_fp, c_int, c_int, c_int, c_int, c_fp]),
    "dwc_lstm_seq_ws_bytes": (c_sz, [c_int, c_int]),
    "dwc_lstm_seq_fwd": (c_int, [c_fp] * 6 + [c_int] * 4 + [c_fp, c_sz, c_fp, c_int, c_fp]),
    "dwc_lstm_seq_bwd": (c_int, [c_fp] * 7 + [c_int] * 4 + [c_fp, c_sz, c_fp, c_int, c_fp]),
    "dwc_adv_tail_fwd": (c_int, [c_fp, c_fp, c_fp, c_fp, c_int, c_int, c_int, c_int, AdvSpec, c_fp]),
    "dwc_adv_tail_bwd": (c_int, [c_fp, c_fp, c_fp, c_fp, c_fp, c_fp, c_int, c_int, c_int, c_int, AdvSpec, c_fp]),
    "dwc_bf16_conv2d_s2_halo_ok": (c_int, [c_int] * 5),
    "dwc_bf16_conv2d_s2_halo": (c_int, [c_fp] * 4 + [c_int] * 6 + [c_fp]),
    "dwc_x3_conv2d_same_ok": (c_int, [c_int] * 6),
    "dwc_x3_weight_prepared_elems": (c_sz, [c_int] * 3),
    "dwc_x3_weight_prepare": (c_int, [c_fp, c_fp] + [c_int] * 5 + [c_fp]),
    "dwc_x3_conv2d_same": (c_int, [c_fp] * 4 + [c_int] * 9 + [c_fp]),
    "dwc_x3_conv2d_same_add": (c_int, [c_fp] * 5 + [c_int] * 9 + [c_fp]),
    "dwc_x3_conv2d_narrow_ok": (c_int, [c_int] * 8),
    "dwc_x3_conv2d_narrow_weight_elems": (c_sz, [c_int] * 2),
    "dwc_x3_conv2d_narrow": (c_int, [c_fp] * 4 + [c_int] * 12 + [c_fp]),
    "dwc_reflect_pad_adjoint_pitch": (c_int, [c_fp, c_fp] + [c_int] * 6 + [c_fp]),
    "dwc_x3_gather_split": (c_int, [c_fp, c_fp, c_fp, c_int, c_fp]),
    "dwc_x3_conv2d_stem_ok": (c_int, [c_int] * 7),
    "dwc_x3_conv2d_stem_weight_elems": (c_sz, []),
    "dwc_x3_conv2d_stem": (c_int, [c_fp] * 4 + [c_int] * 9 + [c_fp]),
    "dwc_x3_conv2d_stem_crop": (c_int, [c_fp] * 5 + [c_int] * 10 + [c_fp]),
    "dwc_x3_conv2d_stem_amax": (c_int, [c_fp] * 5 + [c_u] + [c_int] * 9 + [c_fp]),
    "dwc_reflect_pad_adjoint_band": (c_int, [c_fp, c_fp, c_int, c_int, c_int, c_int, c_int, c_fp]),
    "dwc_x3_conv2d_ksplit_ws_bytes": (c_sz, [c_int] * 7),
    "dwc_x3_conv2d_ksplit_ticket_words": (c_int, []),
    "dwc_x3_conv2d_same_add_ws": (c_int, [c_fp] * 5 + [c_int] * 9 + [c_fp, c_sz, c_fp, c_fp]),
    "dwc_x3_conv2d_s2_ws": (c_int, [c_fp] * 4 + [c_int] * 7 + [c_fp, c_sz, c_fp, c_fp]),
    "dwc_x3_conv2d_s2_ok": (c_int, [c_int] * 5),
    "dwc_x3_conv2d_s2": (c_int, [c_fp] * 4 + [c_int] * 7 + [c_fp]),
    "dwc_x3_conv2d_s2_bwd_data_ok": (c_int, [c_int] * 5),
    "dwc_x3_conv2d_s2_bwd_data": (c_int, [c_fp] * 3 + [c_int] * 6 + [c_fp]),
    "dwc_conv2d_bwd_data_s2_ring": (c_int, [c_fp] * 4 + [c_int] * 5 + [c_fp]),
    "dwc_bf16_conv2d_s2_halo_bwd_data_ok": (c_int, [c_int] * 5),
    "dwc_bf16_conv2d_s2_halo_bwd_data": (c_int, [c_fp] * 3 + [c_int] * 5 + [c_fp]),
    "dwc_bf16_conv2d_s2_halo_bwd_data_fused": (c_int, [c_fp] * 3 + [c_int] * 5 + [c_fp]),
    "dwc_bf16_conv2d_bwd_data_s2_ring": (c_int, [c_fp] * 4 + [c_int] * 5 + [c_fp]),
    "dwc_x3_conv2d_wgrad_ws_bytes": (c_sz, [c_int] * 6),
    "dwc_x3_conv2d_wgrad": (c_int, [c_fp, c_fp, c_fp] + [c_int] * 8 + [c_fp, c_sz, c_fp]),
    "dwc_absmax": (c_int, [c_fp, c_sz, c_fp, c_u, c_fp]),
    "dwc_instnorm_fwd_amax": (c_int, [c_fp] * 7 + [c_int, c_int, c_int, c_f, c_int, c_fp, c_sz, c_fp, c_u, c_fp]),
    "dwc_instnorm_bwd_amax": (c_int, [c_fp] * 9 + [c_int, c_int, c_int, c_int, c_fp, c_sz, c_fp, c_u, c_fp]),
    "dwc_layernorm_fwd_amax": (c_int, [c_fp] * 6 + [c_int, c_int, c_int, c_f, c_int, c_fp, c_sz, c_fp, c_u, c_fp]),
    "dwc_layernorm_bwd_amax": (c_int, [c_fp] * 9 + [c_int, c_int, c_int, c_f, c_int, c_fp, c_sz, c_fp, c_u, c_fp]),
    "dwc_act_bwd_bias_amax": (c_int, [c_fp, c_fp, c_fp, c_fp, c_int, c_int, c_int, c_fp, c_sz, c_fp, c_u, c_fp]),
    "dwc_h2_weight_prepared_elems": (c_sz, [c_int] * 3),
    "dwc_h2_weight_prepare": (c_int, [c_fp, c_fp] + [c_int] * 5 + [c_fp, c_u, c_fp]),
    "dwc_h2_conv2d_same_add_ws": (c_int, [c_fp, c_fp, c_u] + [c_fp] * 4 + [c_fp, c_u] + [c_int] * 9 + [c_fp, c_sz, c_fp, c_fp]),
    "dwc_h2_conv2d_bwd_data_same_fused": (c_int, [c_fp, c_fp, c_u] + [c_fp] * 3 + [c_int] * 7 + [c_fp, c_sz, c_fp, c_fp]),
    "dwc_h2_conv2d_s2_ws": (c_int, [c_fp, c_fp, c_u] + [c_fp] * 3 + [c_fp, c_u] + [c_int] * 7 + [c_fp, c_sz, c_fp, c_fp]),
    "dwc_h2_conv2d_s2_bwd_data": (c_int, [c_fp, c_fp, c_u, c_fp, c_fp] + [c_int] * 6 + [c_fp]),
    "dwc_h2_conv2d_s2_bwd_data_fused": (c_int, [c_fp, c_fp, c_u, c_fp, c_fp] + [c_int] * 6 + [c_fp]),
    "dwc_h2_conv2d_wgrad": (c_int, [c_fp, c_fp, c_u, c_fp, c_fp, c_u, c_fp] + [c_int] * 8 + [c_fp, c_sz, c_fp]),
    "dwc_bf16_conv2d_wgrad_halo_ws_bytes": (c_sz, [c_int] * 6),
    "dwc_bf16_conv2d_wgrad_halo": (c_int, [c_fp, c_fp, c_fp] + [c_int] * 8 + [c_fp, c_sz, c_fp]),
    "dwc_bf16_conv7_smallk_wgrad_ws_bytes": (c_sz, [c_int] * 4),
    "dwc_bf16_conv7_smallk_wgrad": (c_int, [c_fp, c_fp, c_fp] + [c_int] * 5 + [c_fp, c_sz, c_fp]),
    "dwc_x3_conv7_smallk_wgrad_ws_bytes": (c_sz, [c_int] * 4),
    "dwc_x3_conv7_smallk_wgrad": (c_int, [c_fp, c_fp, c_fp] + [c_int] * 5 + [c_fp, c_sz, c_fp]),
    "dwc_bf16_conv2d_stem_ok": (c_int, [c_int] * 7),
    "dwc_bf16_conv2d_stem": (c_int, [c_fp] * 4 + [c_int] * 9 + [c_fp]),
    "dwc_bf16_conv2d_stem_crop": (c_int, [c_fp] * 5 + [c_int] * 10 + [c_fp]),
    "dwc_bf16_conv2d_narrow_ok": (c_int, [c_int] * 8),
    "dwc_bf16_conv2d_narrow": (c_int, [c_fp] * 4 + [c_int] * 12 + [c_fp]),
    "dwc_bf16_conv2d_bwd_data_image_narrow": (c_int, [c_fp, c_fp, c_fp] + [c_int] * 7 + [c_fp, c_sz, c_fp]),
    "dwc_bf16_conv2d_bwd_data_image_ws_bytes": (c_sz, [c_int] * 7),
    "dwc_bf16_conv2d_bwd_data_image": (c_int, [c_fp, c_fp, c_fp] + [c_int] * 7 + [c_fp, c_sz, c_fp]),
    "dwc_bf16_conv2d_bwd_weight_ws_bytes": (c_sz, [c_int] * 9),
    "dwc_bf16_conv2d_bwd_weight": (c_int, [c_fp, c_fp, c_fp] + [c_int] * 11 + [c_fp, c_sz, c_fp]),
    "dwc_bf16_conv2d_bwd_weight_ex_ws_bytes": (c_sz, [c_int] * 11),
    "dwc_bf16_conv2d_bwd_weight_ex": (c_int, [c_fp, c_fp, c_fp] + [c_int] * 13 + [c_fp, c_sz, c_fp]),
    "dwc_bf16_act_bwd_bias": (c_int, [c_fp, c_fp, c_fp, c_fp, c_int, c_int, c_int, c_fp, c_sz, c_fp]),
    "dwc_bf16_instnorm_fwd": (c_int, [c_fp] * 7 + [c_int, c_int, c_int, c_f, c_int, c_fp, c_sz, c_fp]),
    "dwc_bf16_instnorm_bwd": (c_int, [c_fp] * 9 + [c_int, c_int, c_int, c_int, c_fp, c_sz, c_fp]),
    "dwc_bf16_layernorm_fwd": (c_int, [c_fp] * 6 + [c_int, c_int, c_int, c_f, c_int, c_fp, c_sz, c_fp]),
    "dwc_bf16_layernorm_bwd": (c_int, [c_fp] * 9 + [c_int, c_int, c_int, c_f, c_int, c_fp, c_sz, c_fp]),
    "dwc_bf16_upsample2x_fwd": (c_int, [c_fp, c_fp, c_int, c_int, c_int, c_int, c_fp]),
    "dwc_bf16_upsample2x_bwd": (c_int, [c_fp, c_fp, c_int, c_int, c_int, c_int, c_fp]),
    "dwc_bf16_avgpool2_fwd": (c_int, [c_fp, c_fp, c_int, c_int, c_int, c_int, c_fp]),
    "dwc_bf16_avgpool2_bwd": (c_int, [c_fp, c_fp, c_int, c_int, c_int, c_int, c_fp]),
    "dwc_pack_nchw_to_nhwc8_bf16": (c_int, [c_fp, c_fp, c_int, c_int, c_int, c_int, c_fp]),
    "dwc_unpack_nhwc8_bf16_to_nchw": (c_int, [c_fp, c_fp, c_int, c_int, c_int, c_int, c_fp]),
    "dwc_bf16_blend_fwd": (c_int, [c_fp, c_fp, c_fp, c_int, c_fp]),
    "dwc_bf16_blend_bwd": (c_int, [c_fp, c_fp, c_fp, c_fp, c_int, c_fp]),
    "dwc_bf16_l1_mean_fwd": (c_int, [c_fp, c_fp, c_fp, c_sz, c_int, c_fp, c_sz, c_fp]),
    "dwc_bf16_l1_mean_bwd": (c_int, [c_fp, c_fp, c_fp, c_fp, c_fp, c_sz, c_int, c_fp]),
    "dwc_sn_layer_saved_floats": (c_sz, [c_int] * 3),
    "dwc_sn_power_blocks": (c_int, [c_int, c_int, c_fp, c_fp]),
    "dwc_sn_power_iteration": (c_int, [c_fp, c_int, c_int, c_int, c_fp, c_int, c_fp]),
    "dwc_sn_epilogue_bwd_ws_bytes": (c_sz, [c_int] * 4),
    "dwc_sn_epilogue_fwd": (c_int, [c_fp] * 4 + [c_int] * 4 + [c_fp, c_u, c_fp]),
    "dwc_bf16_sn_epilogue_fwd": (c_int, [c_fp] * 4 + [c_int] * 4 + [c_fp]),
    "dwc_sn_epilogue_bwd": (c_int, [c_fp] * 7 + [c_int] * 4 + [c_fp, c_sz, c_fp, c_u, c_fp]),
    "dwc_bf16_sn_epilogue_bwd": (c_int, [c_fp] * 7 + [c_int] * 4 + [c_fp, c_sz, c_fp]),
    "dwc_sn_weight_grad": (c_int, [c_fp, c_int, c_fp, c_int, c_fp, c_fp, c_fp] + [c_int] * 4 + [c_fp]),
    "dwc_grad_penalty_fwd": (c_int, [c_fp] * 4 + [c_int] * 5 + [c_fp]),
    "dwc_grad_penalty_scale": (c_int, [c_fp] * 4 + [c_int] * 4 + [c_fp]),
    "dwc_src_head_seed": (c_int, [c_fp] * 3 + [c_int] * 3 + [c_fp]),
}

ABI_VERSION = 9
EINVAL = -1
_ERRORS = {-1: "DWC_EINVAL (unsupported shape/argument)", -2: "DWC_EWORKSPACE (scratch too small)",
           -3: "DWC_ELAUNCH (kernel launch failed)"}

_lib = None


class HipKernelError(RuntimeError):
    pass


def load():
    global _lib
    if _lib is not None:
        return _lib
    if not os.path.exists(LIB_PATH):
        raise ImportError(
            "libdwcgan_hip.so not found at %s — build it with `make -C dwc-gan_amd/csrc` "
            "(or python -c 'import __graft_entry__ as g; g.build()'). There is no CPU fallback." % LIB_PATH)
    import torch
    lib = ctypes.CDLL(LIB_PATH)
    for name, (res, args) in SIGNATURES.items():
        fn = getattr(lib, name)
        fn.restype = res
        fn.argtypes = args
    got = lib.dwc_version()
    if got != ABI_VERSION:
        raise ImportError("%s reports C-ABI version %d, this binding expects %d (include/dwcgan_hip.h DWC_ABI_VERSION): rebuild it with "
                          "`make -C dwc-gan_amd/csrc`" % (LIB_PATH, got, ABI_VERSION))
    _lib = lib
    return lib


def check(rc, what):
    if rc != 0:
        raise HipKernelError("%s failed: %s" % (what, _ERRORS.get(rc, rc)))
```

dwc-gan_amd/hipdwc/ops.py:

```python
import os
import weakref

import numpy as np
import torch

from . import _lib

ACT = {"none": 0, None: 0, "relu": 1, "lrelu": 2, "tanh": 3, "sigmoid": 4, "heads": 5, "heads8": 6}

PRECISION = "fp32"
BF16 = torch.bfloat16

_REMOVED_SWITCHES = ("DWC_WINOGRAD", "DWC_TXT_STREAM", "DWC_NORM_FUSED_FINAL", "DWC_GEMM_TILE", "DWC_STRIP_BM", "DWC_X3_DUO", "DWC_X3_BN",
                     "DWC_X3_BN32", "DWC_X3_WIDE", "DWC_X3_STAGGER", "DWC_HALO_STAGGER", "DWC_X3_WDUO", "DWC_HALO16", "DWC_HALO_DUO",
                     "DWC_HALO_BN128", "DWC_BF16_TILE", "DWC_BF16_STAGES3", "DWC_NARROW_ROWS16")
_set = [k for k in _REMOVED_SWITCHES if k in os.environ]
if _set:
    import warnings
    warnings.warn("hipdwc: %s no longer select%s anything (removed in round 5, DESIGN.md 10.3) and %s ignored" % (
        ", ".join(_set), "s" if len(_set) == 1 else "", "is" if len(_set) == 1 else "are"), stacklevel=2)
del _set


def set_precision(name):
# ... 28 lines not shown
    if _RAW_STREAM is not None:
        return _RAW_STREAM(torch.cuda.current_device())
    return torch.cuda.current_stream().cuda_stream


_WS = {}


def workspace(nbytes, device):
    key = (device.index if device.index is not None else torch.cuda.current_device(), _stream())
    buf = _WS.get(key)
    if buf is None or buf.numel() < nbytes:
        buf = torch.empty(max(int(nbytes), 1 << 20), dtype=torch.uint8, device=device)
        _WS[key] = buf
    return buf


def cl(x):
    if x.dtype not in (torch.float32, BF16):
        raise TypeError("fp32 or bf16 only")
    if x.dim() != 4:
        raise ValueError("expected a 4-D NCHW-shaped tensor")
    return x.contiguous(memory_format=torch.channels_last)


def empty_cl(b, c, h, w, device, dtype=torch.float32):
    return torch.empty((b, c, h, w), dtype=dtype, device=device, memory_format=torch.channels_last)


def _p(t):
    return None if t is None else t.data_ptr()


class KernelTimer:

    def __init__(self):
        self.spans = []
        self.details = []
        self.executed = []
        self.hbm = {}

    def run(self, tag, flops, fn, detail="", exec_flops=None):
        a, b = torch.cuda.Event(enable_timing=True), torch.cuda.Event(enable_timing=True)
        a.record()
        rc = fn()
        b.record()
        self.spans.append((tag, flops, a, b))
        self.details.append(detail)
        self.executed.append(flops if exec_flops is None else exec_flops)
        return rc

    def ledger(self):
        torch.cuda.synchronize()
        out = {}
        for (tag, flops, a, b), ex, det in zip(self.spans, self.executed, self.details):
            words = det.split()
            kind = words[0] if words else tag
            ksz = next((w for w in words[1:] if w[0] == "k" and w[1:].isdigit()), "")
            ent = out.setdefault(kind + ("/" + ksz if ksz else ""), {"launches": 0, "ms": 0.0, "flops": 0.0, "exec_flops": 0.0,
                                                                      "tag": tag.split("/")[-1], "shapes": {}, "shape_ms": {}})
            ms = a.elapsed_time(b)
            ent["launches"] += 1
            ent["ms"] += ms
            ent["flops"] += flops
            ent["exec_flops"] += ex
            ent["shapes"][det] = ent["shapes"].get(det, 0) + 1
            ent["shape_ms"][det] = round(ent["shape_ms"].get(det, 0.0) + ms, 4)
        return out

    def hbm_ledger(self):
        return {k: {"calls": v[0], "bytes": v[1]} for k, v in self.hbm.items()}

    def summary(self):
        torch.cuda.synchronize()
        out = {}
        for (tag, flops, a, b), ex in zip(self.spans, self.executed):
            ent = out.setdefault(tag, {"launches": 0, "ms": 0.0, "flops": 0.0, "exec_flops": 0.0})
            ent["launches"] += 1
            ent["ms"] += a.elapsed_time(b)
            ent["flops"] += flops
            ent["exec_flops"] += ex
        return out


TIMER = None


def _hbm(family, nbytes):
    if TIMER is not None:
        e = TIMER.hbm.setdefault(family, [0, 0])
        e[0] += 1
        e[1] += int(nbytes)
SCOPE = ""


class scope:

    def __init__(self, name):
        self.name = name

    def __enter__(self):
        global SCOPE
        self.prev, SCOPE = SCOPE, self.name

    def __exit__(self, *exc):
        global SCOPE
        SCOPE = self.prev


_G3_GEMM = {"fwd", "dgrad", "dgrad-image", "fwd-heads", "dgrad-heads", "fwd-zeropad", "dgrad-zeropad"}
_G3_WGRAD = {"wgrad", "wgrad-heads"}


def _timed(tag, flops, fn, scope_name=None, detail="", exec_flops=None):
    if TIMER is None:
        return fn()
    s = SCOPE if scope_name is None else scope_name
    words = detail.split()
    if PRECISION == "fp32" and words and (words[0] in _G3_GEMM or words[0] in _G3_WGRAD):
        mode = _lib.load().dwc_x3_gemm_mode(-1)
        try:
            ci = int(words[3].split(">")[0])
            k = int(next(w for w in words[4:] if w[0] == "k")[1:])
        except (IndexError, ValueError, StopIteration):
            ci, k = 0, 0
        on = (mode & 2) if words[0] in _G3_WGRAD else ((mode & 1) and k * k * ci >= 128)
        if on:
            detail = words[0] + "-g3 " + " ".join(words[1:])
            exec_flops = 6.0 * (flops if exec_flops is None else exec_flops)
            tag = "wgrad_x3_kernel+reduce" if words[0] in _G3_WGRAD else "conv_halo_x3_kernel"
    return TIMER.run((s + "/" + tag) if s else tag, flops, fn, detail, exec_flops)


def _pad4(n):
    return (n + 3) // 4 * 4


def _padc(n, dtype):
    return (n + 7) // 8 * 8 if dtype == BF16 else (n + 3) // 4 * 4


_WCACHE = {}


_X3_BANK_IDX = {}


def _x3_bank_recipe(kind, w, cout_pad, cin_pad):
    if kind in ("stem_steps_x3", "stem_steps_dgrad_x3"):
        wf = w.float()
        if kind == "stem_steps_dgrad_x3":
            wf = wf.flip(2, 3).permute(1, 0, 2, 3)
        co, pl, kh, kw = wf.shape
        assert co == 64 and pl <= 4 and kh == 7 and kw == 7
        bank = torch.zeros((64, 52, 4), dtype=torch.float32, device=w.device)
        bank[:, :49, :pl] = wf.permute(0, 2, 3, 1).reshape(64, 49, pl)
        steps = bank.view(64, 13, 2, 8).permute(1, 0, 2, 3).contiguous()
        swap = ((torch.arange(64, device=w.device) >> 3) & 1).bool()
        steps[:, swap] = steps[:, swap].flip(2)
        return steps.reshape(13, 64, 16)
    if kind == "heads_narrow_x3":
        px = 32 // w.shape[0]
        bank = _shifted_bank(w.float(), px).reshape(32, w.shape[1], w.shape[2], w.shape[3] + px - 1)
    else:
        co, ci, kh, kw = w.shape
        px = 32 // cin_pad
        wf = torch.zeros((cin_pad, cout_pad, kh, kw), dtype=torch.float32, device=w.device)
        wf[:ci, :co] = w.float().flip(2, 3).permute(1, 0, 2, 3)
        bank = _shifted_bank(wf, px).reshape(px * cin_pad, cout_pad, kh, kw + px - 1)
    rows_, ch, kh, kww = bank.shape
    assert rows_ == 32 and ch == 64
    v = bank.permute(2, 3, 1, 0).reshape(kh * kww, 4, 2, 8, 32).permute(1, 0, 2, 4, 3)
    ntp = (kh * kww + 7) // 8 * 8
    return torch.nn.functional.pad(v.reshape(4, kh * kww, 512), (0, 0, 0, ntp - kh * kww))


def _prepped(w, kind, cout_pad, cin_pad, stride, owner=None, half=False):
    owners = (w,) if owner is None else (tuple(owner) if isinstance(owner, (tuple, list)) else (owner,))
    anchor = owners[0]
    slot = _WCACHE.get(id(anchor))
    if slot is None or slot[0]() is not anchor:
        wid = id(anchor)
        slot = (weakref.ref(anchor, lambda _r, wid=wid: _WCACHE.pop(wid, None)), {})
        _WCACHE[wid] = slot
    ent = slot[1]
    key = (kind, cout_pad, cin_pad, stride, tuple(w.shape), bool(half))
    stamp = tuple((o._version, o.data_ptr()) for o in owners)
    if ent.get(key, (None, None))[0] == stamp:
        return ent[key][1]
    lib = _lib.load()
    if kind in ("x3_fwd", "x3_dgrad"):
        co, ci, kh, kw = w.shape
        wz = w.detach()
        if co != cout_pad or ci != cin_pad:
            wz = torch.zeros((cout_pad, cin_pad, kh, kw), dtype=torch.float32, device=w.device)
            wz[:co, :ci] = w.detach()
        dg = kind == "x3_dgrad"
        rows, kdim = (cin_pad, cout_pad) if dg else (cout_pad, cin_pad)
        out = torch.empty(lib.dwc_x3_weight_prepared_elems(rows, kdim, kh), dtype=BF16, device=w.device)
        _lib.check(lib.dwc_x3_weight_prepare(wz.contiguous().data_ptr(), out.data_ptr(), cout_pad, cin_pad, kh, rows, int(dg),
                                             _stream()), "x3_weight_prepare")
        recipe = None
        if co == cout_pad and ci == cin_pad:
            recipe = _recipe(w, owners, kind=5 if dg else 4, n_items=kh * kh * ((kdim + 15) // 16) * rows * 16, Cout=co, Cin=ci,
                             KH=kh, KW=kw, rows=rows, kdim=kdim)
        ent[key] = (stamp, out, recipe)
        return out
    if kind in ("h2_fwd", "h2_dgrad"):
        co, ci, kh, kw = w.shape
        wz = w.detach()
        if co != cout_pad or ci != cin_pad:
            wz = torch.zeros((cout_pad, cin_pad, kh, kw), dtype=torch.float32, device=w.device)
            wz[:co, :ci] = w.detach()
        wz = wz.contiguous()
        dg = kind == "h2_dgrad"
        rows, kdim = (cin_pad, cout_pad) if dg else (cout_pad, cin_pad)
        out = torch.zeros(lib.dwc_h2_weight_prepared_elems(rows, kdim, kh), dtype=torch.float16, device=w.device)
        slot, ep = amax_slot(w.device)
        _lib.check(lib.dwc_absmax(wz.data_ptr(), wz.numel(), slot, ep, _stream()), "absmax(weight)")
        _lib.check(lib.dwc_h2_weight_prepare(wz.data_ptr(), out.data_ptr(), cout_pad, cin_pad, kh, rows, int(dg), slot, ep, _stream()),
                   "h2_weight_prepare")
        recipe = None
        if co == cout_pad and ci == cin_pad:
            recipe = _recipe(w, owners, kind=9 if dg else 8, n_items=kh * kh * ((kdim + 15) // 16) * rows * 16, Cout=co, Cin=ci,
                             KH=kh, KW=kw, rows=rows, kdim=kdim)
        ent[key] = (stamp, out, recipe)
        return out
    if kind in ("stem_steps", "stem_steps_dgrad"):
        wf = w.detach().float()
        if kind == "stem_steps_dgrad":
            wf = wf.flip(2, 3).permute(1, 0, 2, 3)
        co, pl, kh, kw = wf.shape
        assert co == 64 and pl <= 8 and kh == 7 and kw == 7
        bank = torch.zeros((64, 50, 8), dtype=torch.float32, device=w.device)
        bank[:, :49, :pl] = wf.permute(0, 2, 3, 1).reshape(64, 49, pl)
        steps = bank.view(64, 25, 2, 8).permute(1, 0, 2, 3).contiguous()
        swap = ((torch.arange(64, device=w.device) >> 3) & 1).bool()
        steps = torch.where(swap.view(1, 64, 1, 1), steps.flip(2), steps)
        out = steps.reshape(25, 64, 16).to(BF16).contiguous()
        ent[key] = (stamp, out)
        return out
    if kind in ("stem_steps_x3", "stem_steps_dgrad_x3", "heads_narrow_x3", "dgrad_image_narrow_x3"):
        ikey = (kind, tuple(w.shape), cout_pad, cin_pad, str(w.device))
        idx = _X3_BANK_IDX.get(ikey)
        if idx is None:
            num = (torch.arange(w.numel(), dtype=torch.float32, device=w.device) + 1.0).view(w.shape)
            idx = (_x3_bank_recipe(kind, num, cout_pad, cin_pad).reshape(-1).round().to(torch.int32) - 1).contiguous()
            _X3_BANK_IDX[ikey] = idx
        n = idx.numel()
        src = w.detach()
        if src.dtype != torch.float32 or not src.is_contiguous():
            src = src.float().contiguous()
        out = torch.empty(3 * n, dtype=BF16, device=w.device)
        _lib.check(lib.dwc_x3_gather_split(src.data_ptr(), idx.data_ptr(), out.data_ptr(), n, _stream()), "x3_gather_split")
        if kind.startswith("stem_steps"):
            assert out.numel() == lib.dwc_x3_conv2d_stem_weight_elems()
        else:
            ntp = n // (4 * 512)
            out = out.view(3, 4, ntp, 512).permute(1, 2, 0, 3).contiguous().view(-1)
            assert out.numel() == lib.dwc_x3_conv2d_narrow_weight_elems(7, 14)
        ent[key] = (stamp, out)
        return out
    if kind in ("heads_narrow", "dgrad_image_narrow"):
        base = _prepped(w, "heads_wide" if kind == "heads_narrow" else "dgrad_image", cout_pad, cin_pad, stride, owner, True)
        ch = cout_pad if kind == "dgrad_image_narrow" else cin_pad
        taps = base.numel() // (32 * ch)
        out = base.view(32, taps, ch // 16, 2, 8).permute(1, 2, 3, 0, 4).reshape(taps, -1)
        out = torch.nn.functional.pad(out, (0, 0, 0, (taps + 7) // 8 * 8 - taps)).contiguous()
        ent[key] = (stamp, out)
        return out
    if kind == "heads_wide":
        px = 32 // w.shape[0]
        bank = _shifted_bank(w.detach(), px).reshape(32, w.shape[1], w.shape[2], w.shape[3] + px - 1)
        out = _prepped(bank, "fwd", 32, cin_pad, 1, half=half)
        ent[key] = (stamp, out)
        return out
    if kind == "dgrad_image":
        co, ci, kh, kw = w.shape
        px = 32 // cin_pad
        wf = torch.zeros((cin_pad, cout_pad, kh, kw), dtype=torch.float32, device=w.device)
        wf[:ci, :co] = w.detach().flip(2, 3).permute(1, 0, 2, 3)
        bank = _shifted_bank(wf, px).reshape(px * cin_pad, cout_pad, kh, kw + px - 1)
        out = _prepped(bank, "fwd", px * cin_pad, cout_pad, 1, half=half)
        ent[key] = (stamp, out)
        return out
    cout, cin, kh, kw = w.shape
    wc = w.detach().contiguous()
    transposed = kind == "dgrad_t"
    if transposed:
        wc = w.detach().transpose(2, 3).contiguous()
        kind = "dgrad"
    pre = "dwc_bf16_" if half else "dwc_"
    n = getattr(lib, pre + "weight_prepared_elems")(cout, cin, kh, kw, stride, cout_pad, cin_pad, int(kind == "dgrad"))
    out = torch.empty(n, dtype=BF16 if half else torch.float32, device=w.device)
    if kind == "fwd":
        _lib.check(getattr(lib, pre + "weight_prepare_fwd")(wc.data_ptr(), out.data_ptr(), cout, cin, kh, kw, cout_pad, cin_pad,
                                                            _stream()), "weight_prepare_fwd")
        rows, kdim = cout_pad, kh * kw * cin_pad
    else:
        _lib.check(getattr(lib, pre + "weight_prepare_dgrad")(wc.data_ptr(), out.data_ptr(), cout, cin, kh, kw, stride,
                                                              cout_pad, cin_pad, _stream()), "weight_prepare_dgrad")
        rows, kdim = (cin_pad, kh * kw * cout_pad) if stride == 1 else (4 * cin_pad, 4 * cout_pad)
    recipe = None
    if (not transposed or kh == kw) and n % rows == 0:
        recipe = _recipe(w, owners, kind=(2 if half else 0) + (kind == "dgrad"), n_items=n, Cout=cout, Cin=cin, KH=kh, KW=kw,
                         stride=stride, cout_pad=cout_pad, cin_pad=cin_pad, Kp=n // rows, transpose_hw=int(transposed))
    ent[key] = (stamp, out, recipe)
    return out


_PCAT = {}


class _CatParams(torch.autograd.Function):

    @staticmethod
    def forward(ctx, stack, *ps):
        anchor = ps[0]
        slot = _PCAT.get(id(anchor))
        if slot is None or slot[0]() is not anchor:
            aid = id(anchor)
            slot = (weakref.ref(anchor, lambda _r, aid=aid: _PCAT.pop(aid, None)), {})
            _PCAT[aid] = slot
        key = (bool(stack), tuple(id(p) for p in ps))
        stamp = tuple((p._version, p.data_ptr()) for p in ps)
        ent = slot[1].get(key)
        if ent is None or ent[0] != stamp:
            with torch.no_grad():
                buf = torch.stack([p.detach() for p in ps]) if stack else torch.cat([p.detach() for p in ps], 0)
            ent = (stamp, buf)
            slot[1][key] = ent
        ctx.stack = bool(stack)
        ctx.sizes = [p.shape[0] for p in ps]
        return ent[1].view_as(ent[1])

    @staticmethod
    def backward(ctx, g):
        parts = g.unbind(0) if ctx.stack else g.split(ctx.sizes, 0)
        return (None,) + tuple(parts)


_PCAT_LIVE = {}


def cat_params(params, stack=False):
    params = list(params)
    if not params[0].is_cuda:
        return torch.stack(params) if stack else torch.cat(params, 0)
    if not (torch.is_grad_enabled() and any(p.requires_grad for p in params)):
        return _CatParams.apply(stack, *params)
    key = (bool(stack), tuple(id(p) for p in params))
    stamp = tuple((p._version, p.data_ptr(), p.requires_grad) for p in params)
    ent = _PCAT_LIVE.get(key)
    if ent is not None and ent[0] == stamp and all(r() is p for r, p in zip(ent[1], params)):
        return ent[2]
    out = _CatParams.apply(stack, *params)
    if len(_PCAT_LIVE) > 256:
        for k in [k for k, e in _PCAT_LIVE.items() if any(r() is None for r in e[1])]:
            del _PCAT_LIVE[k]
    _PCAT_LIVE[key] = (stamp, [weakref.ref(p) for p in params], out)
    return out


def _shifted_bank(w, px):
    kw = w.shape[-1]
    bank = torch.zeros((px,) + tuple(w.shape[:-1]) + (kw + px - 1,), dtype=w.dtype, device=w.device)
    diag = bank.as_strided((px,) + tuple(w.shape), (bank.stride(0) + 1,) + tuple(bank.stride()[1:]))
    diag.copy_(w.unsqueeze(0).expand((px,) + tuple(w.shape)))
    return bank


_REFRESH_DT = np.dtype([("src", "<u8"), ("dst", "<u8"), ("n_items", "<u8"), ("kind", "<i4"), ("Cout", "<i4"), ("Cin", "<i4"),
                        ("KH", "<i4"), ("KW", "<i4"), ("stride", "<i4"), ("cout_pad", "<i4"), ("cin_pad", "<i4"), ("Kp", "<i4"),
                        ("rows", "<i4"), ("kdim", "<i4"), ("transpose_hw", "<i4"), ("reserved", "<i4"), ("tail_pad", "<i4")])
assert _REFRESH_DT.itemsize == 80
REFRESH_CHUNK = 8192
_REFRESH_TABLES = {}
REFRESH_STATS = {"launches": 0, "layouts": 0}
_REFRESH_EPOCH = 0


def _recipe(w, owners, **fields):
    if len(owners) != 1 or w.data_ptr() != owners[0].data_ptr() or not w.detach().is_contiguous() or w.dtype != torch.float32:
        return None
    return fields


def refresh_prepared(params):
    todo = []
    for p in params:
        slot = _WCACHE.get(id(p))
        if slot is None or slot[0]() is not p:
            continue
        stamp = ((p._version, p.data_ptr()),)
        for key, val in slot[1].items():
            if len(val) > 2 and val[2] is not None and val[0] != stamp:
                todo.append((p, slot[1], key, val, stamp))
    if not todo:
        return 0
    lib = _lib.load()
    dev = todo[0][0].device
    ident = tuple((p.data_ptr(), val[1].data_ptr(), tuple(sorted(val[2].items()))) for p, _, _, val, _ in todo)
    table = _REFRESH_TABLES.get(ident)
    if table is None:
        desc = np.zeros(len(todo), dtype=_REFRESH_DT)
        cd, cs = [], []
        for i, (p, _, _, val, _) in enumerate(todo):
            desc[i]["src"], desc[i]["dst"] = p.data_ptr(), val[1].data_ptr()
            for k, v in val[2].items():
                desc[i][k] = v
            for s0 in range(0, int(val[2]["n_items"]), REFRESH_CHUNK):
                cd.append(i)
                cs.append(s0)
        host = torch.from_numpy(desc.view(np.uint8).reshape(-1)).pin_memory()
        table = (host.to(dev, non_blocking=True), torch.tensor(cd, dtype=torch.int32, device=dev),
                 torch.tensor(np.array(cs, dtype=np.uint32).view(np.int32), dtype=torch.int32, device=dev), len(cd),
                 int(any(int(v[3][2]["kind"]) in (8, 9) for v in todo)))
        if len(_REFRESH_TABLES) > 16:
            _REFRESH_TABLES.clear()
        _REFRESH_TABLES[ident] = table
    global _REFRESH_EPOCH
    _REFRESH_EPOCH += 1
    _lib.check(lib.dwc_weight_refresh_multi(table[0].data_ptr(), table[1].data_ptr(), table[2].data_ptr(), table[3], table[4],
                                            _REFRESH_EPOCH, _stream()), "weight_refresh_multi")
    for p, ent, key, val, stamp in todo:
        ent[key] = (stamp, val[1], val[2])
    REFRESH_STATS["launches"] += 1
    REFRESH_STATS["layouts"] += len(todo)
    return len(todo)


X3 = int(os.environ.get("DWC_X3", "2"))
HALO = int(os.environ.get("DWC_BF16_HALO", "1"))
WGRAD_HALO = int(os.environ.get("DWC_BF16_WGRAD_HALO", "1"))
STEM = int(os.environ.get("DWC_BF16_STEM", "1"))
NARROW = int(os.environ.get("DWC_BF16_NARROW", "1"))
NARROW_X3 = int(os.environ.get("DWC_X3_NARROW", "1"))
SMALLK_X3 = int(os.environ.get("DWC_X3_SMALLK", "1"))
LSTM_SEQ = int(os.environ.get("DWC_LSTM_SEQ", "1"))
DGRAD_FOLD = int(os.environ.get("DWC_DGRAD_FOLD", "1"))
X3_S2 = int(os.environ.get("DWC_X3_S2", "1"))
S2HALO = int(os.environ.get("DWC_BF16_S2_HALO", "1"))
S2DGRAD = int(os.environ.get("DWC_S2_DGRAD_HALO", "1"))
X3_WGRAD_HALO3 = int(os.environ.get("DWC_X3_WGRAD_HALO3", "1"))
PINNED_STAGE = int(os.environ.get("DWC_PINNED_STAGE", "1"))
ZERO_GRAD_BY_FLAG = int(os.environ.get("DWC_ZERO_GRAD_FLAG", "1"))
RING_FUSED = int(os.environ.get("DWC_RING_FUSED", "1"))
PENALTY_HIP = int(os.environ.get("DWC_PENALTY_HIP", "0"))
S2DGRAD_MIN_WGS = 192


X3_PLANES = int(os.environ.get("DWC_X3_PLANES", "2"))
AMAX_SLOTS = 1 << 16
_AMAX = {}


def amax_slot(dev):
    key = dev.index if dev.index is not None else torch.cuda.current_device()
    pool = _AMAX.get(key)
    if pool is None:
        pool = [torch.zeros(AMAX_SLOTS, dtype=torch.int64, device=dev), 0]
        _AMAX[key] = pool
    i = pool[1]
    pool[1] = i + 1
    return pool[0].data_ptr() + 8 * (i % AMAX_SLOTS), i // AMAX_SLOTS + 1


def amax_live(t, c=False):
    if c is False:
        c = getattr(t, "_dwc_amax", None)
    if c is None or c[2] != t._version or c[3] != t.data_ptr():
        return None
    pool = _AMAX.get(t.device.index if t.device.index is not None else torch.cuda.current_device())
    if pool is None:
        return None
    index = (c[1] - 1) * AMAX_SLOTS + (c[0] - pool[0].data_ptr()) // 8
    return (c[0], c[1]) if 0 <= pool[1] - index < AMAX_SLOTS - 4096 else None


def amax_of(t):
    c = amax_live(t)
    if c is not None:
        if AMAX_CHECK:
            _amax_verify(t, c)
        return c
    if t.dtype != torch.float32 or not (t.is_contiguous() or t.is_contiguous(memory_format=torch.channels_last)):
        raise ValueError("amax_of: dense fp32 tensor expected")
    slot, ep = amax_slot(t.device)
    _lib.check(_lib.load().dwc_absmax(t.data_ptr(), t.numel(), slot, ep, _stream()), "absmax")
    set_amax(t, slot, ep)
    return slot, ep


def h2_fits(t):
    return X3_PLANES == 2 and t.numel() * 4 < (1 << 31)


def set_amax(t, slot, ep):
    t._dwc_amax = (slot, ep, t._version, t.data_ptr())
    return t


AMAX_CHECK = int(os.environ.get("DWC_AMAX_CHECK", "0"))


def _amax_verify(t, c):
    pool = _AMAX[t.device.index if t.device.index is not None else torch.cuda.current_device()][0]
    word = int(pool[(c[0] - pool.data_ptr()) // 8])
    bits = word & 0xffffffff
    if (word >> 32) != c[1]:
        raise RuntimeError("DWC_AMAX_CHECK: slot epoch %d, tag says %d" % (word >> 32, c[1]))
    true_bits = int(t.detach().abs().max().view(torch.int32)) if t.numel() else 0
    if true_bits > bits:
        raise RuntimeError("DWC_AMAX_CHECK: stale absmax tag -- slot holds %g, the tensor's largest magnitude is %g" % (
            np.uint32(bits).view(np.float32), np.uint32(true_bits).view(np.float32)))


def out_amax(t):
    if X3_PLANES != 2 or t.dtype != torch.float32:
        return None, 0
    return amax_slot(t.device)


def pass_amax(src, dst):
    c = amax_live(src)
    if c is not None:
        set_amax(dst, c[0], c[1])
    return dst


def _x3_use(lib, B, H, W, c_in, c_out, KH, KW, stride, pad, free=False):
    if not X3 or stride != 1 or KH != KW or 2 * pad != KH - 1 or c_in % 16 or c_out % 16:
        return False
    if KH == 3 and X3 < 2 and not free:
        return False
    return bool(lib.dwc_x3_conv2d_same_ok(B, H, W, c_in, c_out, KH))


class ResGradToken:
    __slots__ = ("g",)

    def __init__(self):
        self.g = None


RES_FUSE = int(os.environ.get("DWC_RES_FUSE", "1"))


def res_token(x):
    return ResGradToken() if RES_FUSE and torch.is_grad_enabled() and x.requires_grad else None


_X3_TICKETS = {}


def _x3_ksplit(lib, dev, B, H, W, Cx, cop, K, stride, at_least=0):
    need = lib.dwc_x3_conv2d_ksplit_ws_bytes(B, H, W, Cx, cop, K, stride)
    if not need:
        ws = workspace(at_least, dev) if at_least else None
        return ws, at_least, None
    key = (dev.index if dev.index is not None else torch.cuda.current_device(), _stream())
    row = _X3_TICKETS.get(key)
    if row is None:
        row = torch.zeros(int(lib.dwc_x3_conv2d_ksplit_ticket_words()), dtype=torch.int32, device=dev)
        _X3_TICKETS[key] = row
    n = max(int(need), int(at_least))
    return workspace(n, dev), n, row.data_ptr()


_KSPLIT_POLL = {}


def ksplit_status_poll(wait=False):
    for key, row in list(_X3_TICKETS.items()):
        if key[1] != _stream():
            continue
        ent = _KSPLIT_POLL.get(key)
        if ent is None:
            ent = [torch.zeros(1, dtype=torch.int32).pin_memory(), None]
            _KSPLIT_POLL[key] = ent
        if ent[1] is not None and (wait or ent[1].query()):
            if wait:
                ent[1].synchronize()
            ent[1] = None
            status = int(ent[0][0])
            if status != 0:
                row.zero_()
                ent[0].zero_()
                raise _lib.HipKernelError(
                    "contraction split of a split-product convolution: the two halves of a tile did not meet (status %d); the tile was "
                    "overwritten with NaN and the ticket row has been re-zeroed.  DWC_X3_KSPLIT=0 runs these launches unsplit." % status)
        if ent[1] is None:
            ent[0].copy_(row[-1:], non_blocking=True)
            ent[1] = torch.cuda.Event()
            ent[1].record()


class _Conv2d(torch.autograd.Function):

    @staticmethod
    def forward(ctx, x, w, b, stride, pad, act, bias_grad=True, owner=None, token=None, nograd=False):
        _require_device(x)
        lib = _lib.load()
        x = cl(x)
        half = x.dtype == BF16
        ctx.token = token
        B, Cx, H, W = x.shape
        Cout, Cin, KH, KW = w.shape
        if Cin > Cx:
            raise ValueError("input has %d channels, weight expects %d" % (Cx, Cin))
        ctx.bias_grad = bias_grad
        ctx.zero_flag = bool(b is not None and getattr(b, "_dwc_zero_grad", False))
        ctx.owner = owner
        cop = _padc(Cout, x.dtype)
        Ho = (H + 2 * pad - KH) // stride + 1
        Wo = (W + 2 * pad - KW) // stride + 1
        w_grad = ctx.needs_input_grad[1] and not nograd
        use_x3 = (not half) and _x3_use(lib, B, H, W, Cx, cop, KH, KW, stride, pad, free=not w_grad)
        use_x3s2 = bool((not half) and X3 and X3_S2 and stride == 2 and KH == 4 and KW == 4 and pad == 1 and cop % 64 == 0
                        and B * (H // 32) * (W // 32) * (cop // 64) >= 160 and lib.dwc_x3_conv2d_s2_ok(B, H, W, Cx, cop))
        use_stem = bool(half and NARROW and STEM and Cx == 8 and cop == 64 and stride == 1 and KH == 7 and KW == 7 and pad == 3
                        and lib.dwc_bf16_conv2d_stem_ok(B, H, W, H, W, KH, act))
        use_stem_x3 = bool((not half) and X3 and NARROW_X3 and Cx == 4 and cop == 64 and stride == 1 and KH == 7 and KW == 7 and pad == 3
                           and lib.dwc_x3_conv2d_stem_ok(B, H, W, H, W, KH, act))
        w_hwio = None if use_x3 or use_x3s2 or use_stem or use_stem_x3 else _prepped(w, "fwd", cop, Cx, stride, owner, half)
        bias = None
        if b is not None:
            bias = b.detach() if cop == Cout else torch.nn.functional.pad(b.detach(), (0, cop - Cout))
            bias = bias.contiguous()
        y = empty_cl(B, cop, Ho, Wo, x.device, x.dtype)
        flops = 2.0 * B * Ho * Wo * Cout * Cin * KH * KW
        st = _stream()
        if use_x3 and h2_fits(x):
            w_h2 = _prepped(w, "h2_fwd", cop, Cx, 1, owner)
            ks_ws, ks_n, ks_t = _x3_ksplit(lib, x.device, B, H, W, Cx, cop, KH, 1)
            x_amax = amax_of(x)
            ya, yep = out_amax(y)
            _lib.check(_timed("conv_halo_x3_kernel", flops, lambda: lib.dwc_h2_conv2d_same_add_ws(
                x.data_ptr(), x_amax[0], x_amax[1], w_h2.data_ptr(), _p(bias), None, y.data_ptr(), ya, yep, B, H, W, Cx, cop, cop, KH, act, 1,
                _p(ks_ws), ks_n, ks_t, st), detail="fwd-h2 B%d %dx%d %d>%d k%d s%d" % (B, H, W, Cx, cop, KH, stride), exec_flops=3 * flops),
                "h2_conv2d_same")
            set_amax(y, ya, yep)
        elif use_x3:
            w_x3 = _prepped(w, "x3_fwd", cop, Cx, 1, owner)
            ks_ws, ks_n, ks_t = _x3_ksplit(lib, x.device, B, H, W, Cx, cop, KH, 1)
            _lib.check(_timed("conv_halo_x3_kernel", flops, lambda: lib.dwc_x3_conv2d_same_add_ws(
                x.data_ptr(), w_x3.data_ptr(), _p(bias), None, y.data_ptr(), B, H, W, Cx, cop, cop, KH, act, 1, _p(ks_ws), ks_n, ks_t, st),
                detail="fwd-x3 B%d %dx%d %d>%d k%d s%d" % (B, H, W, Cx, cop, KH, stride), exec_flops=6 * flops), "x3_conv2d_same")
        elif use_x3s2 and h2_fits(x):
            w_h2 = _prepped(w, "h2_fwd", cop, Cx, 1, owner)
            ks_ws, ks_n, ks_t = _x3_ksplit(lib, x.device, B, H, W, Cx, cop, KH, 2)
            x_amax = amax_of(x)
            ya, yep = out_amax(y)
            _lib.check(_timed("conv_halo_x3_kernel", flops, lambda: lib.dwc_h2_conv2d_s2_ws(
                x.data_ptr(), x_amax[0], x_amax[1], w_h2.data_ptr(), _p(bias), y.data_ptr(), ya, yep, B, H, W, Cx, cop, cop, act, _p(ks_ws), ks_n,
                ks_t, st), detail="fwd-h2s2 B%d %dx%d %d>%d k%d s%d" % (B, H, W, Cx, cop, KH, stride), exec_flops=3 * flops), "h2_conv2d_s2")
            set_amax(y, ya, yep)
        elif use_x3s2:
            w_x3 = _prepped(w, "x3_fwd", cop, Cx, 1, owner)
            ks_ws, ks_n, ks_t = _x3_ksplit(lib, x.device, B, H, W, Cx, cop, KH, 2)
            _lib.check(_timed("conv_halo_x3_kernel", flops, lambda: lib.dwc_x3_conv2d_s2_ws(
                x.data_ptr(), w_x3.data_ptr(), _p(bias), y.data_ptr(), B, H, W, Cx, cop, cop, act, _p(ks_ws), ks_n, ks_t, st),
                detail="fwd-x3s2 B%d %dx%d %d>%d k%d s%d" % (B, H, W, Cx, cop, KH, stride), exec_flops=6 * flops), "x3_conv2d_s2")
        elif use_stem_x3:
            w_st = _prepped(w, "stem_steps_x3", cop, Cx, 1, owner)
            ya, yep = out_amax(y)
            _lib.check(_timed("conv_halo_x3_kernel", flops, lambda: lib.dwc_x3_conv2d_stem_amax(
                x.data_ptr(), w_st.data_ptr(), _p(bias), y.data_ptr(), ya, yep, B, H, W, H, W, KH, -pad, act, 1, st),
                detail="fwd-stem-x3 B%d %dx%d %d>%d k%d s%d" % (B, H, W, Cx, cop, KH, stride), exec_flops=6 * flops), "x3_conv2d_stem")
            if ya is not None:
                set_amax(y, ya, yep)
        elif use_stem:
            w_st = _prepped(w, "stem_steps", cop, Cx, 1, owner, True)
            _lib.check(_timed("conv_gemm_kernel", flops, lambda: lib.dwc_bf16_conv2d_stem(
                x.data_ptr(), w_st.data_ptr(), _p(bias), y.data_ptr(), B, H, W, H, W, KH, -pad, act, 1, st),
                detail="fwd-stem B%d %dx%d %d>%d k%d s%d" % (B, H, W, Cx, cop, KH, stride)), "conv2d_stem")
        elif (half and HALO and S2HALO and stride == 2 and KH == 4 and KW == 4 and pad == 1
# ... 1190 lines not shown
```

include/dwcgan_hip.h:

```cpp
#ifndef DWCGAN_HIP_H
#define DWCGAN_HIP_H

#include <stddef.h>
#include <stdint.h>

#ifdef __cplusplus
extern "C" {
#endif

#define DWC_OK 0
#define DWC_EINVAL (-1)
#define DWC_EWORKSPACE (-2)
#define DWC_ELAUNCH (-3)

#define DWC_ACT_NONE 0
#define DWC_ACT_RELU 1
#define DWC_ACT_LRELU 2
#define DWC_ACT_TANH 3
#define DWC_ACT_SIGMOID 4
#define DWC_ACT_HEADS 5
#define DWC_ACT_HEADS8 6

#define DWC_ABI_VERSION 9
int dwc_version(void);
int dwc_x3_gemm_mode(int mode);

size_t dwc_weight_prepared_elems(int Cout, int Cin, int KH, int KW, int stride, int cout_pad, int cin_pad,
                                 int for_dgrad);
int dwc_weight_prepare_fwd(const float* w_oihw, float* w_prepared, int Cout, int Cin, int KH, int KW,
                           int cout_pad, int cin_pad, void* stream);
int dwc_weight_prepare_dgrad(const float* w_oihw, float* w_prepared, int Cout, int Cin, int KH, int KW,
                             int stride, int cout_pad, int cin_pad, void* stream);

size_t dwc_conv2d_fwd_ws_bytes(int B, int H, int W, int Cin, int Cout, int KH, int KW, int stride, int pad);
int dwc_conv2d_fwd(const float* x, const float* w_prepared, const float* bias, float* y,
                   int B, int H, int W, int Cin, int Cout, int KH, int KW, int stride, int pad,
                   int act, void* ws, size_t ws_bytes, void* stream);
size_t dwc_conv2d_bwd_data_ws_bytes(int B, int H, int W, int Cin, int Cout, int KH, int KW, int stride, int pad);
int dwc_conv2d_bwd_data(const float* dy, const float* w_dgrad, float* dxp,
                        int B, int H, int W, int Cin, int Cout, int KH, int KW, int stride, int pad,
                        void* ws, size_t ws_bytes, void* stream);
int dwc_reflect_pad_adjoint(const float* dxp, float* dx, int B, int H, int W, int C, int pad,
                            void* stream);
int dwc_conv2d_bwd_data_fold(const float* dy, const float* w_dgrad, float* dxp, float* dx, int B, int H, int W, int Cin, int Cout, int KH,
                             int KW, int stride, int pad, void* ws, size_t ws_bytes, void* stream);
size_t dwc_conv2d_bwd_data_same_ws_bytes(int B, int H, int W, int Cin, int Cout, int KH, int KW, int pad);
int dwc_conv2d_bwd_data_same(const float* dy, const float* w_dgrad, const float* w_dgrad_t, float* dx,
                             int B, int H, int W, int Cin, int Cout, int KH, int KW, int pad,
                             void* ws, size_t ws_bytes, void* stream);
int dwc_conv2d_bwd_data_ring(const float* dy, const float* w_dgrad, const float* w_dgrad_t, float* dx,
                             int B, int H, int W, int Cin, int Cout, int KH, int KW, int pad,
                             void* ws, size_t ws_bytes, void* stream);
size_t dwc_conv2d_bwd_data_image_ws_bytes(int B, int H, int W, int Cout, int KH, int KW, int pad);
int dwc_conv2d_bwd_data_image(const float* dy, const float* w_wide, float* dx,
                              int B, int H, int W, int Cout, int KH, int KW, int pad,
                              void* ws, size_t ws_bytes, void* stream);
size_t dwc_conv2d_bwd_weight_ws_bytes(int B, int H, int W, int Cin, int Cout, int KH, int KW,
                                      int stride, int pad);
int dwc_conv2d_bwd_weight(const float* x, const float* dy, float* dw_oihw,
                          int B, int H, int W, int Cin, int Cout, int KH, int KW, int stride, int pad,
                          int cin_real, int cout_real, void* ws, size_t ws_bytes, void* stream);
int dwc_conv2d_fwd_ex(const float* x, const float* w_prepared, const float* bias, float* y,
                      int B, int H, int W, int Cin, int Cout, int KH, int KW,
                      int stride_h, int stride_w, int pad_h, int pad_w, int act, void* stream);
size_t dwc_conv2d_bwd_weight_ex_ws_bytes(int B, int H, int W, int Cin, int Cout, int KH, int KW,
                                         int stride_h, int stride_w, int pad_h, int pad_w);
int dwc_conv2d_bwd_weight_ex(const float* x, const float* dy, float* dw_oihw,
                             int B, int H, int W, int Cin, int Cout, int KH, int KW,
                             int stride_h, int stride_w, int pad_h, int pad_w,
                             int cin_real, int cout_real, void* ws, size_t ws_bytes, void* stream);
size_t dwc_act_bwd_bias_ws_bytes(int rows, int C);
int dwc_act_bwd_bias(const float* dy, const float* y, float* g, float* db, int rows, int C, int act,
                     void* ws, size_t ws_bytes, void* stream);

size_t dwc_instnorm_ws_bytes(int B, int HW, int C);
int dwc_instnorm_fwd(const float* x, const float* gamma, const float* beta, const float* residual,
                     float* y, float* mean, float* rstd, int B, int HW, int C, float eps, int relu,
                     void* ws, size_t ws_bytes, void* stream);
int dwc_instnorm_bwd(const float* dy, const float* x, const float* mean, const float* rstd,
                     const float* gamma, const float* beta, float* dx, float* dgamma, float* dbeta,
                     int B, int HW, int C, int relu, void* ws, size_t ws_bytes, void* stream);

int dwc_linear_small_ok(int M, int N, int K);
int dwc_linear_small_fwd(const float* x, const float* w, const float* bias, float* y, int M, int N, int K, int relu, void* stream);
int dwc_linear_small_bwd(const float* dy, const float* y_relu, const float* x, const float* w, float* dx, float* dw, float* db, int M,
                         int N, int K, void* stream);

size_t dwc_layernorm_ws_bytes(int B, int HW, int C);
int dwc_layernorm_fwd(const float* x, const float* gamma, const float* beta, float* y,
                      float* mean, float* inv, int B, int HW, int C, float eps, int relu,
                      void* ws, size_t ws_bytes, void* stream);
int dwc_layernorm_bwd(const float* dy, const float* x, const float* mean, const float* inv,
                      const float* gamma, const float* beta, float* dx, float* dgamma, float* dbeta,
                      int B, int HW, int C, float eps, int relu, void* ws, size_t ws_bytes, void* stream);

int dwc_upsample2x_fwd(const float* x, float* y, int B, int H, int W, int C, void* stream);
int dwc_upsample2x_bwd(const float* dy, float* dx, int B, int H, int W, int C, void* stream);
int dwc_avgpool2_fwd(const float* x, float* y, int B, int H, int W, int C, void* stream);
int dwc_avgpool2_bwd(const float* dy, float* dx, int B, int H, int W, int C, void* stream);

int dwc_pack_nchw_to_nhwc4(const float* x_nchw, float* y_nhwc4, int B, int C, int H, int W, void* stream);
int dwc_unpack_nhwc4_to_nchw(const float* x_nhwc4, float* y_nchw, int B, int C, int H, int W, void* stream);

int dwc_conv2d_fwd_zeropad(const float* x, const float* w_prepared, const float* bias, float* y,
                           int B, int H, int W, int Cin, int Cout, int KH, int KW, int stride, int pad,
                           int act, void* ws, size_t ws_bytes, void* stream);
size_t dwc_conv2d_bwd_data_zeropad_ws_bytes(int B, int H, int W, int Cin, int Cout, int KH, int KW, int pad);
int dwc_conv2d_bwd_data_zeropad(const float* dy, const float* w_dgrad, float* dx,
                                int B, int H, int W, int Cin, int Cout, int KH, int KW, int pad,
                                void* ws, size_t ws_bytes, void* stream);
int dwc_maxpool2_fwd(const float* x, float* y, int B, int H, int W, int C, void* stream);
int dwc_maxpool2_bwd(const float* x, const float* dy, float* dx, int B, int H, int W, int C, void* stream);

int dwc_blend_fwd(const float* heads, const float* real, float* out, int npix, void* stream);
int dwc_blend_bwd(const float* dout, const float* heads, const float* real, float* dheads, int npix,
                  void* stream);

int dwc_gmm_kl_sp_fwd(const float* mu, const float* lv, const float* centre, int centre_stride, int B, int K, int D, float sigma,
                      float* out_scalar, void* stream);
int dwc_gmm_kl_sp_bwd(const float* mu, const float* lv, const float* centre, int centre_stride, int B, int K, int D, float sigma,
                      const float* dout_scalar, float* dmu, float* dlv, void* stream);

size_t dwc_l1_ws_bytes(size_t n);
int dwc_l1_mean_fwd(const float* a, const float* b, float* out_scalar, size_t n, int skip4, void* ws,
                    size_t ws_bytes, void* stream);
int dwc_l1_mean_bwd(const float* a, const float* b, const float* dout_scalar, float* da, float* db,
                    size_t n, int skip4, void* stream);

int dwc_lstm_fwd(const float* xproj, const float* w_hh, const int* lens, float* out, float* c, float* gates,
                 int T, int B, int H, int dirs, void* stream);
size_t dwc_lstm_seq_ws_bytes(int B, int dirs);
int dwc_lstm_seq_fwd(const float* xproj, const float* w_hh, const int* lens, float* out, float* c, float* gates, int T, int B, int H,
                     int dirs, void* ws, size_t ws_bytes, unsigned* status, int max_workgroups, void* stream);
int dwc_lstm_seq_bwd(const float* d_out, const float* d_c, const float* w_hh_t, const int* lens, const float* c, const float* gates,
                     float* dgates, int T, int B, int H, int dirs, void* ws, size_t ws_bytes, unsigned* status, int max_workgroups,
                     void* stream);
int dwc_lstm_bwd(const float* d_out, const float* d_c, const float* w_hh_t, const int* lens, const float* c,
                 const float* gates, float* dgates, float* dc_carry, int T, int B, int H, int dirs, void* stream);

int dwc_adam_step(float* p, const float* g, float* m, float* v, size_t n, float lr, float beta1,
                  float beta2, float eps, float weight_decay, int step, void* stream);
int dwc_ema_lerp(const float* p, float* ema, size_t n, float beta, void* stream);

#define DWC_OPT_CHUNK 8192
typedef struct {
    float* p;
    const float* g;
    float* m;
    float* v;
    unsigned long long n;
    float step_size;
    float bc2_sqrt;
} dwc_adam_tensor;
typedef struct {
    const float* p;
    float* ema;
    unsigned long long n;
} dwc_ema_tensor;
int dwc_adam_multi(const dwc_adam_tensor* tensors_dev, const int* chunk_tensor_dev,
                   const unsigned* chunk_start_dev, int n_chunks, double beta1, double beta2, double eps,
                   double weight_decay, void* stream);
int dwc_ema_multi(const dwc_ema_tensor* tensors_dev, const int* chunk_tensor_dev,
                  const unsigned* chunk_start_dev, int n_chunks, float beta, void* stream);

typedef struct {
    float target[4], w_src[4], w_cls[4];
} dwc_adv_spec;
int dwc_adv_tail_fwd(const float* src, const float* cls, const float* labels, float* out, int segs, int B, int src_per_sample, int ncls,
                     dwc_adv_spec spec, void* stream);
int dwc_adv_tail_bwd(const float* src, const float* cls, const float* labels, const float* dout, float* dsrc, float* dcls, int segs,
                     int B, int src_per_sample, int ncls, dwc_adv_spec spec, void* stream);

enum { DWC_REFRESH_FWD_F32 = 0, DWC_REFRESH_DGRAD_F32 = 1, DWC_REFRESH_FWD_BF16 = 2, DWC_REFRESH_DGRAD_BF16 = 3,
       DWC_REFRESH_X3_FWD = 4, DWC_REFRESH_X3_DGRAD = 5,
       DWC_REFRESH_H2_FWD = 8, DWC_REFRESH_H2_DGRAD = 9 };
typedef struct {
    const float* src;
    void* dst;
    unsigned long long n_items;
    int kind;
    int Cout, Cin, KH, KW, stride, cout_pad, cin_pad, Kp;
    int rows, kdim;
    int transpose_hw;
    int reserved;
} dwc_refresh_desc;
int dwc_weight_refresh_multi(const dwc_refresh_desc* descs_dev, const int* chunk_desc_dev, const unsigned* chunk_start_dev,
                             int n_chunks, int has_h2, unsigned epoch, void* stream);

int dwc_x3_conv2d_same_ok(int B, int H, int W, int Cin, int Cout, int K);
size_t dwc_x3_weight_prepared_elems(int rows, int kdim, int K);
int dwc_x3_weight_prepare(const float* w_oihw, void* out, int Cout, int Cin, int K, int rows, int dgrad, void* stream);
int dwc_x3_conv2d_same(const float* x, const void* w_prepared, const float* bias, float* y, int B, int H, int W, int Cin, int N,
                       int rows, int K, int act, int reflect, void* stream);
int dwc_x3_conv2d_same_add(const float* x, const void* w_prepared, const float* bias, const float* add, float* y, int B, int H, int W,
                           int Cin, int N, int rows, int K, int act, int reflect, void* stream);
int dwc_x3_conv2d_narrow_ok(int B, int IH, int IW, int Cin, int OH, int OWg, int KH, int KWW);
size_t dwc_x3_conv2d_narrow_weight_elems(int KH, int KWW);
int dwc_x3_conv2d_narrow(const float* x, const void* w_frag, const float* bias32, float* y, int B, int IH, int IW, int Cin, int OH,
                         int OWg, int KH, int KWW, int off_h, int off_w, int act, int reflect, void* stream);
int dwc_reflect_pad_adjoint_pitch(const float* dxp, float* dx, int B, int H, int W, int C, int pad, int pitch, void* stream);
int dwc_x3_gather_split(const float* src, const int* idx, void* out_3planes, int n, void* stream);
int dwc_x3_conv2d_stem_ok(int B, int IH, int IW, int OH, int OW, int K, int act);
size_t dwc_x3_conv2d_stem_weight_elems(void);
int dwc_x3_conv2d_stem(const float* x, const void* w_steps, const float* bias, float* y, int B, int IH, int IW, int OH, int OW, int K,
                       int off, int act, int reflect, void* stream);
int dwc_x3_conv2d_stem_crop(const float* x, const void* w_steps, const float* bias, float* y, float* inner, int crop, int B, int IH, int IW,
                            int OH, int OW, int K, int off, int act, int reflect, void* stream);
int dwc_x3_conv2d_stem_amax(const float* x, const void* w_steps, const float* bias, float* y, void* y_amax, unsigned y_epoch, int B, int IH,
                            int IW, int OH, int OW, int K, int off, int act, int reflect, void* stream);
int dwc_reflect_pad_adjoint_band(const float* dxp, float* dx, int B, int H, int W, int C, int pad, void* stream);
size_t dwc_x3_conv7_smallk_wgrad_ws_bytes(int B, int H, int W, int heads);
int dwc_x3_conv7_smallk_wgrad(const float* img4, const float* t64, float* dw, int B, int H, int W, int planes, int heads, void* ws,
                              size_t ws_bytes, void* stream);
size_t dwc_x3_conv2d_ksplit_ws_bytes(int B, int H, int W, int Cin, int N, int K, int stride);
int dwc_x3_conv2d_ksplit_ticket_words(void);
int dwc_x3_conv2d_same_add_ws(const float* x, const void* w_prepared, const float* bias, const float* add, float* y, int B, int H, int W,
                              int Cin, int N, int rows, int K, int act, int reflect, void* ws, size_t ws_bytes, unsigned* tickets,
                              void* stream);
int dwc_x3_conv2d_s2_ws(const float* x, const void* w_prepared, const float* bias, float* y, int B, int H, int W, int Cin, int N, int rows,
                        int act, void* ws, size_t ws_bytes, unsigned* tickets, void* stream);
int dwc_x3_conv2d_s2_ok(int B, int H, int W, int Cin, int Cout);
int dwc_x3_conv2d_s2(const float* x, const void* w_prepared, const float* bias, float* y, int B, int H, int W, int Cin, int N, int rows,
                     int act, void* stream);
int dwc_x3_conv2d_s2_bwd_data_ok(int B, int H, int W, int Cin, int Cout);
int dwc_x3_conv2d_s2_bwd_data(const float* dy, const void* w_prepared, float* dx, int B, int H, int W, int Cin, int Cout, int rows,
                              void* stream);
int dwc_conv2d_bwd_data_s2_ring(const float* dy, const float* w_dgrad, float* dxp, float* dx, int B, int H, int W, int Cin, int Cout,
                                void* stream);
int dwc_absmax(const float* x, size_t n, void* slot, unsigned epoch, void* stream);
int dwc_instnorm_fwd_amax(const float* x, const float* gamma, const float* beta, const float* residual, float* y, float* mean,
                          float* rstd, int B, int HW, int C, float eps, int relu, void* ws, size_t ws_bytes,
                          void* out_amax, unsigned out_epoch, void* stream);
int dwc_instnorm_bwd_amax(const float* dy, const float* x, const float* mean, const float* rstd, const float* gamma,
                          const float* beta, float* dx, float* dgamma, float* dbeta, int B, int HW, int C, int relu, void* ws,
                          size_t ws_bytes, void* out_amax, unsigned out_epoch, void* stream);
int dwc_layernorm_fwd_amax(const float* x, const float* gamma, const float* beta, float* y, float* mean, float* inv, int B, int HW,
                           int C, float eps, int relu, void* ws, size_t ws_bytes, void* out_amax, unsigned out_epoch, void* stream);
int dwc_layernorm_bwd_amax(const float* dy, const float* x, const float* mean, const float* inv, const float* gamma,
                           const float* beta, float* dx, float* dgamma, float* dbeta, int B, int HW, int C, float eps, int relu,
                           void* ws, size_t ws_bytes, void* out_amax, unsigned out_epoch, void* stream);
int dwc_act_bwd_bias_amax(const float* dy, const float* y, float* g, float* db, int rows, int C, int act, void* ws, size_t ws_bytes,
                          void* g_amax, unsigned g_epoch, void* stream);
size_t dwc_h2_weight_prepared_elems(int rows, int kdim, int K);
int dwc_h2_weight_prepare(const float* w_oihw, void* out, int Cout, int Cin, int K, int rows, int dgrad, const void* w_amax,
                          unsigned w_epoch, void* stream);
int dwc_h2_conv2d_same_add_ws(const float* x, const void* x_amax, unsigned x_epoch, const void* w_prepared, const float* bias,
                              const float* add, float* y, void* y_amax, unsigned y_epoch, int B, int H, int W, int Cin, int N, int rows,
                              int K, int act, int reflect, void* ws, size_t ws_bytes, unsigned* tickets, void* stream);
int dwc_h2_conv2d_bwd_data_same_fused(const float* dy, const void* dy_amax, unsigned dy_epoch, const void* w_prepared, const float* add,
                                      float* dx, int B, int H, int W, int Cout, int N, int rows, int K, void* ws, size_t ws_bytes,
                                      unsigned* tickets, void* stream);
int dwc_h2_conv2d_s2_ws(const float* x, const void* x_amax, unsigned x_epoch, const void* w_prepared, const float* bias, float* y,
                        void* y_amax, unsigned y_epoch, int B, int H, int W, int Cin, int N, int rows, int act, void* ws, size_t ws_bytes,
                        unsigned* tickets, void* stream);
int dwc_h2_conv2d_s2_bwd_data(const float* dy, const void* dy_amax, unsigned dy_epoch, const void* w_prepared, float* dx, int B, int H, int W,
                              int Cin, int Cout, int rows, void* stream);
int dwc_h2_conv2d_s2_bwd_data_fused(const float* dy, const void* dy_amax, unsigned dy_epoch, const void* w_prepared, float* dx, int B, int H,
                                    int W, int Cin, int Cout, int rows, void* stream);
int dwc_h2_conv2d_wgrad(const float* x, const void* x_amax, unsigned x_epoch, const float* dy, const void* dy_amax, unsigned dy_epoch,
                        float* dw_oihw, int B, int H, int W, int Cin, int Cout, int K, int cin_real, int cout_real, void* ws, size_t ws_bytes,
                        void* stream);
size_t dwc_x3_conv2d_wgrad_ws_bytes(int B, int H, int W, int Cin, int Cout, int K);
int dwc_x3_conv2d_wgrad(const float* x, const float* dy, float* dw_oihw, int B, int H, int W, int Cin, int Cout, int K, int cin_real,
                        int cout_real, void* ws, size_t ws_bytes, void* stream);

size_t dwc_bf16_weight_prepared_elems(int Cout, int Cin, int KH, int KW, int stride, int cout_pad, int cin_pad, int for_dgrad);
int dwc_bf16_weight_prepare_fwd(const float* w_oihw, void* w_prepared, int Cout, int Cin, int KH, int KW, int cout_pad,
                                int cin_pad, void* stream);
int dwc_bf16_weight_prepare_dgrad(const float* w_oihw, void* w_prepared, int Cout, int Cin, int KH, int KW, int stride,
                                  int cout_pad, int cin_pad, void* stream);
size_t dwc_bf16_conv2d_fwd_ws_bytes(int B, int H, int W, int Cin, int Cout, int KH, int KW, int stride, int pad);
int dwc_bf16_conv2d_fwd(const void* x, const void* w_prepared, const float* bias, void* y, int B, int H, int W, int Cin,
                        int Cout, int KH, int KW, int stride, int pad, int act, void* ws, size_t ws_bytes, void* stream);
int dwc_bf16_conv2d_fwd_ex(const void* x, const void* w_prepared, const float* bias, void* y, int B, int H, int W, int Cin,
                           int Cout, int KH, int KW, int stride_h, int stride_w, int pad_h, int pad_w, int act, void* stream);
size_t dwc_bf16_conv2d_bwd_data_ws_bytes(int B, int H, int W, int Cin, int Cout, int KH, int KW, int stride, int pad);
int dwc_bf16_conv2d_bwd_data(const void* dy, const void* w_dgrad, void* dxp, int B, int H, int W, int Cin, int Cout, int KH,
                             int KW, int stride, int pad, void* ws, size_t ws_bytes, void* stream);
int dwc_bf16_reflect_pad_adjoint(const void* dxp, void* dx, int B, int H, int W, int C, int pad, void* stream);
int dwc_bf16_conv2d_bwd_data_fold(const void* dy, const void* w_dgrad, void* dxp, void* dx, int B, int H, int W, int Cin, int Cout,
                                  int KH, int KW, int stride, int pad, void* ws, size_t ws_bytes, void* stream);
int dwc_bf16_reflect_pad_adjoint_band(const void* dxp, void* dx, int B, int H, int W, int C, int pad, void* stream);
size_t dwc_bf16_conv2d_bwd_data_same_ws_bytes(int B, int H, int W, int Cin, int Cout, int KH, int KW, int pad);
int dwc_bf16_conv2d_bwd_data_same(const void* dy, const void* w_dgrad, const void* w_dgrad_t, void* dx, int B, int H, int W,
                                  int Cin, int Cout, int KH, int KW, int pad, void* ws, size_t ws_bytes, void* stream);
int dwc_bf16_conv2d_bwd_data_ring(const void* dy, const void* w_dgrad, const void* w_dgrad_t, void* dx, int B, int H, int W,
                                  int Cin, int Cout, int KH, int KW, int pad, void* ws, size_t ws_bytes, void* stream);
int dwc_bf16_conv2d_fwd_zeropad(const void* x, const void* w_prepared, const float* bias, void* y, int B, int H, int W, int Cin,
                                int Cout, int KH, int KW, int stride, int pad, int act, void* ws, size_t ws_bytes, void* stream);
size_t dwc_bf16_conv2d_bwd_data_zeropad_ws_bytes(int B, int H, int W, int Cin, int Cout, int KH, int KW, int pad);
int dwc_bf16_conv2d_bwd_data_zeropad(const void* dy, const void* w_dgrad, void* dx, int B, int H, int W, int Cin, int Cout, int KH,
                                     int KW, int pad, void* ws, size_t ws_bytes, void* stream);
int dwc_bf16_maxpool2_fwd(const void* x, void* y, int B, int H, int W, int C, void* stream);
int dwc_bf16_maxpool2_bwd(const void* x, const void* dy, void* dx, int B, int H, int W, int C, void* stream);

int dwc_bf16_conv2d_same_halo_ok(int B, int H, int W, int Cin, int Cout, int K);
int dwc_bf16_conv2d_same_halo(const void* x, const void* w_prepared, const float* bias, void* y, int B, int H, int W, int Cin,
                              int Cout, int K, int act, int reflect, void* stream);
int dwc_bf16_conv2d_same_halo_add(const void* x, const void* w_prepared, const float* bias, const void* add, void* y, int B, int H,
                                  int W, int Cin, int Cout, int K, int act, int reflect, void* stream);
int dwc_bf16_conv2d_bwd_data_same_fused_ok(int B, int H, int W, int Cin, int Cout, int K);
int dwc_bf16_conv2d_bwd_data_same_fused(const void* dy, const void* w_dgrad, const void* add, void* dx, int B, int H, int W, int Cin,
                                        int Cout, int K, void* stream);

int dwc_bf16_conv2d_s2_halo_ok(int B, int H, int W, int Cin, int Cout);
int dwc_bf16_conv2d_s2_halo(const void* x, const void* w_prepared, const float* bias, void* y, int B, int H, int W, int Cin, int Cout,
                            int act, void* stream);
int dwc_bf16_conv2d_s2_halo_bwd_data_ok(int B, int H, int W, int Cin, int Cout);
int dwc_bf16_conv2d_s2_halo_bwd_data(const void* dy, const void* w_dgrad, void* dx, int B, int H, int W, int Cin, int Cout, void* stream);
int dwc_bf16_conv2d_s2_halo_bwd_data_fused(const void* dy, const void* w_dgrad, void* dx, int B, int H, int W, int Cin, int Cout, void* stream);
int dwc_bf16_conv2d_bwd_data_s2_ring(const void* dy, const void* w_dgrad, void* dxp, void* dx, int B, int H, int W, int Cin, int Cout,
                                     void* stream);
size_t dwc_bf16_conv2d_wgrad_halo_ws_bytes(int B, int H, int W, int Cin, int Cout, int K);
int dwc_bf16_conv2d_wgrad_halo(const void* x, const void* dy, float* dw_oihw, int B, int H, int W, int Cin, int Cout, int K,
                               int cin_real, int cout_real, void* ws, size_t ws_bytes, void* stream);
int dwc_bf16_conv2d_narrow_ok(int B, int IH, int IW, int Cin, int OH, int OWg, int KH, int KWW);
int dwc_bf16_conv2d_narrow(const void* x, const void* w_frag, const float* bias32, void* y, int B, int IH, int IW, int Cin, int OH,
                           int OWg, int KH, int KWW, int off_h, int off_w, int act, int reflect, void* stream);
int dwc_bf16_conv2d_bwd_data_image_narrow(const void* dy, const void* w_frag, void* dx, int B, int H, int W, int Cout, int KH, int KW,
                                          int pad, void* ws, size_t ws_bytes, void* stream);
int dwc_bf16_conv2d_stem_ok(int B, int IH, int IW, int OH, int OW, int K, int act);
int dwc_bf16_conv2d_stem(const void* x, const void* w_steps, const float* bias, void* y, int B, int IH, int IW, int OH, int OW, int K,
                         int off, int act, int reflect, void* stream);
int dwc_bf16_conv2d_stem_crop(const void* x, const void* w_steps, const float* bias, void* y, void* inner, int crop, int B, int IH, int IW,
                              int OH, int OW, int K, int off, int act, int reflect, void* stream);
size_t dwc_bf16_conv7_smallk_wgrad_ws_bytes(int B, int H, int W, int heads);
int dwc_bf16_conv7_smallk_wgrad(const void* img8, const void* t64, float* dw, int B, int H, int W, int planes, int heads, void* ws,
                                size_t ws_bytes, void* stream);
size_t dwc_bf16_conv2d_bwd_data_image_ws_bytes(int B, int H, int W, int Cout, int KH, int KW, int pad);
int dwc_bf16_conv2d_bwd_data_image(const void* dy, const void* w_wide, void* dx, int B, int H, int W, int Cout, int KH, int KW,
                                   int pad, void* ws, size_t ws_bytes, void* stream);
size_t dwc_bf16_conv2d_bwd_weight_ws_bytes(int B, int H, int W, int Cin, int Cout, int KH, int KW, int stride, int pad);
int dwc_bf16_conv2d_bwd_weight(const void* x, const void* dy, float* dw_oihw, int B, int H, int W, int Cin, int Cout, int KH,
                               int KW, int stride, int pad, int cin_real, int cout_real, void* ws, size_t ws_bytes, void* stream);
size_t dwc_bf16_conv2d_bwd_weight_ex_ws_bytes(int B, int H, int W, int Cin, int Cout, int KH, int KW, int stride_h,
                                              int stride_w, int pad_h, int pad_w);
int dwc_bf16_conv2d_bwd_weight_ex(const void* x, const void* dy, float* dw_oihw, int B, int H, int W, int Cin, int Cout, int KH,
                                  int KW, int stride_h, int stride_w, int pad_h, int pad_w, int cin_real, int cout_real,
                                  void* ws, size_t ws_bytes, void* stream);
int dwc_bf16_act_bwd_bias(const void* dy, const void* y, void* g, float* db, int rows, int C, int act, void* ws,
                          size_t ws_bytes, void* stream);
int dwc_bf16_instnorm_fwd(const void* x, const float* gamma, const float* beta, const void* residual, void* y, float* mean,
                          float* rstd, int B, int HW, int C, float eps, int relu, void* ws, size_t ws_bytes, void* stream);
int dwc_bf16_instnorm_bwd(const void* dy, const void* x, const float* mean, const float* rstd, const float* gamma,
                          const float* beta, void* dx, float* dgamma, float* dbeta, int B, int HW, int C, int relu, void* ws,
                          size_t ws_bytes, void* stream);
int dwc_bf16_layernorm_fwd(const void* x, const float* gamma, const float* beta, void* y, float* mean, float* inv, int B,
                           int HW, int C, float eps, int relu, void* ws, size_t ws_bytes, void* stream);
int dwc_bf16_layernorm_bwd(const void* dy, const void* x, const float* mean, const float* inv, const float* gamma,
                           const float* beta, void* dx, float* dgamma, float* dbeta, int B, int HW, int C, float eps, int relu,
                           void* ws, size_t ws_bytes, void* stream);
int dwc_bf16_upsample2x_fwd(const void* x, void* y, int B, int H, int W, int C, void* stream);
int dwc_bf16_upsample2x_bwd(const void* dy, void* dx, int B, int H, int W, int C, void* stream);
int dwc_bf16_avgpool2_fwd(const void* x, void* y, int B, int H, int W, int C, void* stream);
int dwc_bf16_avgpool2_bwd(const void* dy, void* dx, int B, int H, int W, int C, void* stream);
int dwc_pack_nchw_to_nhwc8_bf16(const float* x, void* y, int B, int C, int H, int W, void* stream);
int dwc_unpack_nhwc8_bf16_to_nchw(const void* x, float* y, int B, int C, int H, int W, void* stream);
int dwc_bf16_blend_fwd(const void* heads, const void* real, void* out, int npix, void* stream);
int dwc_bf16_blend_bwd(const void* dout, const void* heads, const void* real, void* dheads, int npix, void* stream);
int dwc_bf16_l1_mean_fwd(const void* a, const void* b, float* out, size_t n, int skip4, void* ws, size_t ws_bytes, void* stream);
int dwc_bf16_l1_mean_bwd(const void* a, const void* b, const float* dout, void* da, void* db, size_t n, int skip4, void* stream);

typedef struct {
    const float* w;
    float* u;
    float* v;
    long long off_u, off_v, off_r;
    int cout, k, col_blk0, row_blk0, vec, reserved;
} dwc_sn_desc;
size_t dwc_sn_layer_saved_floats(int S, int cout, int k);
int dwc_sn_power_blocks(int cout, int k, int* col_blocks, int* row_blocks);
int dwc_sn_power_iteration(const dwc_sn_desc* desc_dev, int L, int col_blocks, int row_blocks, float* base, int S, void* stream);
size_t dwc_sn_epilogue_bwd_ws_bytes(int rows, int C, int S, int vec);
int dwc_sn_epilogue_fwd(const float* Z, const float* r, const float* b, float* y, int rows, int C, int S, int act, void* y_amax,
                        unsigned y_epoch, void* stream);
int dwc_bf16_sn_epilogue_fwd(const void* Z, const float* r, const float* b, void* y, int rows, int C, int S, int act, void* stream);
int dwc_sn_epilogue_bwd(const float* dy, const float* Z, const float* r, const float* b, float* dZ, float* db, float* c, int rows, int C,
                        int S, int act, void* ws, size_t ws_bytes, void* dz_amax, unsigned dz_epoch, void* stream);
int dwc_bf16_sn_epilogue_bwd(const void* dy, const void* Z, const float* r, const float* b, void* dZ, float* db, float* c, int rows,
                             int C, int S, int act, void* ws, size_t ws_bytes, void* stream);
int dwc_sn_weight_grad(const float* U, int u_stride, const float* V, int v_stride, const float* r, const float* c, float* dw, int S,
                       int cout, int k, int accumulate, void* stream);

#define DWC_PENALTY_GP 0
#define DWC_PENALTY_R1 1
int dwc_grad_penalty_fwd(const float* g, float* q, float* k, float* out, int B, int pixels, int planes, int real_planes, int mode,
                         void* stream);
int dwc_grad_penalty_scale(const float* g, const float* k, const float* dout, float* ghat, int B, int pixels, int planes,
                           int real_planes, void* stream);
int dwc_src_head_seed(const float* a, const float* w_s, float* d, int rows, int C, int act, void* stream);

#ifdef __cplusplus
}
#endif
#endif
```

Baseline: 398.0 images/s.

## Pre-split im2col GEMM weights into three bf16 planes at prepare time

```diff
diff --git a/dwc-gan_amd/csrc/conv_fold.h b/dwc-gan_amd/csrc/conv_fold.h
--- a/dwc-gan_amd/csrc/conv_fold.h
+++ b/dwc-gan_amd/csrc/conv_fold.h
@@ -1,4 +1,6 @@
 #pragma once
+#include <type_traits>
+
 #include "conv_geom.h"
 
 namespace {
@@ -169,21 +171,31 @@
     return DWC_OK;
 }
 
+constexpr int X3_GEMM_MIN_K = 128;
+
+template <typename T>
+__device__ __forceinline__ void weight_prepared_store(T* out, size_t total, size_t idx, float v, bool planes) {
+    out[idx] = (T)v;
+    if constexpr (std::is_same<T, float>::value) {
+        if (planes) dwc_split3_store(reinterpret_cast<unsigned short*>(out + total), total, idx, v);
+    }
+}
+
 template <typename T>
 __global__ void weight_prepare_fwd_kernel(const float* __restrict__ w, T* __restrict__ out, int Cout, int Cin, int KHW,
-                                          int cout_pad, int cin_pad, int Kp) {
+                                          int cout_pad, int cin_pad, int Kp, bool planes) {
     const size_t idx = (size_t)blockIdx.x * blockDim.x + threadIdx.x;
     if (idx >= (size_t)cout_pad * Kp) return;
     const int k = idx % Kp, co = idx / Kp;
     const int ci = k % cin_pad, tap = k / cin_pad;
     float v = 0.f;
     if (co < Cout && ci < Cin && tap < KHW) v = w[((size_t)co * Cin + ci) * KHW + tap];
-    out[idx] = (T)v;
+    weight_prepared_store(out, (size_t)cout_pad * Kp, idx, v, planes);
 }
 
 template <typename T>
 __global__ void weight_prepare_dgrad_kernel(const float* __restrict__ w, T* __restrict__ out, int Cout, int Cin, int KH, int KW,
-                                            int stride, int cout_pad, int cin_pad, int Kp) {
+                                            int stride, int cout_pad, int cin_pad, int Kp, bool planes) {
     const size_t idx = (size_t)blockIdx.x * blockDim.x + threadIdx.x;
     const size_t per_class = (size_t)cin_pad * Kp;
     const int classes = stride == 1 ? 1 : 4;
@@ -203,15 +215,23 @@
         kh = (cls >> 1) + 2 * (tapo >> 1);
         kw = (cls & 1) + 2 * (tapo & 1);
     }
-    out[idx] = (T)(ok ? w[((size_t)co * Cin + ci) * KH * KW + kh * KW + kw] : 0.f);
+    weight_prepared_store(out, per_class * classes, idx, ok ? w[((size_t)co * Cin + ci) * KH * KW + kh * KW + kw] : 0.f, planes);
 }
 
 inline int weight_prepared_kp(int taps, int c_pad, int bk) { return (taps * c_pad + bk - 1) / bk * bk; }
 
+template <typename T>
+inline bool weight_prepared_planes(int taps, int c_pad) {
+    return std::is_same<T, float>::value && taps * c_pad >= X3_GEMM_MIN_K;
+}
+
+template <typename T>
 inline size_t weight_prepared_elems(int KH, int KW, int stride, int cout_pad, int cin_pad, int for_dgrad, int bk) {
-    if (!for_dgrad) return (size_t)cout_pad * weight_prepared_kp(KH * KW, cin_pad, bk);
-    if (stride == 1) return (size_t)cin_pad * weight_prepared_kp(KH * KW, cout_pad, bk);
-    return (size_t)4 * cin_pad * weight_prepared_kp(4, cout_pad, bk);
+    const int taps = for_dgrad && stride != 1 ? 4 : KH * KW;
+    const int c_pad = for_dgrad ? cout_pad : cin_pad;
+    const size_t rows = !for_dgrad ? (size_t)cout_pad : (size_t)(stride == 1 ? 1 : 4) * cin_pad;
+    const size_t n = rows * weight_prepared_kp(taps, c_pad, bk);
+    return weight_prepared_planes<T>(taps, c_pad) ? n + n / 2 * 3 : n;
 }
 
 template <typename T>
@@ -219,7 +239,7 @@
     const int Kp = weight_prepared_kp(KH * KW, cin_pad, bk);
     const size_t total = (size_t)cout_pad * Kp;
     hipLaunchKernelGGL(weight_prepare_fwd_kernel<T>, dim3((unsigned)((total + 255) / 256)), dim3(256), 0, st, w, out, Cout, Cin, KH * KW,
-                       cout_pad, cin_pad, Kp);
+                       cout_pad, cin_pad, Kp, weight_prepared_planes<T>(KH * KW, cin_pad));
     DWC_LAUNCH_CHECK();
     return DWC_OK;
 }
@@ -227,12 +247,13 @@
 template <typename T>
 int weight_prepare_dgrad(const float* w, T* out, int Cout, int Cin, int KH, int KW, int stride, int cout_pad, int cin_pad, int bk,
                          hipStream_t st) {
-    const int Kp = weight_prepared_kp(stride == 1 ? KH * KW : 4, cout_pad, bk);
+    const int taps = stride == 1 ? KH * KW : 4;
+    const int Kp = weight_prepared_kp(taps, cout_pad, bk);
     const size_t total = (size_t)(stride == 1 ? 1 : 4) * cin_pad * Kp;
     hipLaunchKernelGGL(weight_prepare_dgrad_kernel<T>, dim3((unsigned)((total + 255) / 256)), dim3(256), 0, st, w, out, Cout, Cin, KH, KW,
-                       stride, cout_pad, cin_pad, Kp);
-    DWC_LAUNCH_CHECK();
-    return DWC_OK;
-}
-
-}
+                       stride, cout_pad, cin_pad, Kp, weight_prepared_planes<T>(taps, cout_pad));
+    DWC_LAUNCH_CHECK();
+    return DWC_OK;
+}
+
+}
diff --git a/dwc-gan_amd/csrc/conv_igemm.hip b/dwc-gan_amd/csrc/conv_igemm.hip
--- a/dwc-gan_amd/csrc/conv_igemm.hip
+++ b/dwc-gan_amd/csrc/conv_igemm.hip
@@ -39,14 +39,7 @@
 __device__ __forceinline__ void gx3_split8(const f32x4& a, const f32x4& b, gx3_bf16x8& p0, gx3_bf16x8& p1, gx3_bf16x8& p2) {
     unsigned h[8], m[8], l[8];
 #pragma unroll
-    for (int k = 0; k < 8; ++k) {
-        const float v = k < 4 ? a[k] : b[k - 4];
-        const unsigned hb = __float_as_uint(v) & 0xffff0000u;
-        const float r = v - __uint_as_float(hb);
-        const unsigned mb = __float_as_uint(r) & 0xffff0000u;
-        const float q = r - __uint_as_float(mb);
-        h[k] = hb; m[k] = mb; l[k] = __float_as_uint(q);
-    }
+    for (int k = 0; k < 8; ++k) dwc_split3(k < 4 ? a[k] : b[k - 4], h[k], m[k], l[k]);
     gx3_u32x4 u0, u1, u2;
 #pragma unroll
     for (int k = 0; k < 4; ++k) {
@@ -59,13 +52,18 @@
     p2 = __builtin_bit_cast(gx3_bf16x8, u2);
 }
 
-template <int BM, int BN, int WM, int WN, int TM, int TN, bool X3 = false>
-__device__ __forceinline__ void conv_gemm_body(const Gather& g, const float* __restrict__ wmat, const Scatter& o,
-                                               const float* __restrict__ bias, int act, int tiles_n, int kt0, int kt1_in,
-                                               size_t part_offset, bool partial, int oph, int opw, int bid, int nb) {
+template <int BM, int BN, int WM, int WN, int TM, int TN, bool PRE = false, bool X3 = false>
+__device__ __forceinline__ void conv_gemm_body(const Gather& g, const float* __restrict__ wmat, const unsigned short* __restrict__ wplanes,
+                                               size_t plane_stride, const Scatter& o, const float* __restrict__ bias, int act,
+                                               int tiles_n, int kt0, int kt1_in, size_t part_offset, bool partial, int oph, int opw,
+                                               int bid, int nb) {
     static_assert(WM * WN == 4 && WM * TM * 32 == BM && WN * TN * 32 == BN, "tile shape");
+    static_assert(X3 || !PRE, "split planes feed the split-product form only");
     constexpr int A_PASSES = BM / 32, B_PASSES = BN / 32;
-    constexpr int A_TILE = BM * BK, B_TILE = BN * BK;
+    constexpr int A_TILE = BM * BK, B_TILE = PRE ? BN * 48 : BN * BK;
+    constexpr int P_DEPOSITS = BN * 3 / 16;
+    constexpr int P_PASSES = (P_DEPOSITS + 3) / 4;
+    static_assert(2 * (A_TILE + B_TILE) * sizeof(float) <= 65536, "LDS of one workgroup");
     __shared__ __attribute__((aligned(16))) float smem[2 * (A_TILE + B_TILE)];
     float* sA = smem;
     float* sB = smem + 2 * A_TILE;
@@ -98,8 +96,18 @@
     }
     const int Kp = (g.K + BK - 1) / BK * BK;
     const float* b_ptr[B_PASSES];
-#pragma unroll
-    for (int p = 0; p < B_PASSES; ++p) b_ptr[p] = wmat + (size_t)min(n0 + arow + 32 * p, o.N - 1) * Kp + acol;
+    const unsigned short* p_ptr[P_PASSES];
+    if constexpr (PRE) {
+#pragma unroll
+        for (int i = 0; i < P_PASSES; ++i) {
+            const int c = (4 * i + wave) * 64 + lane;
+            const int pl = min(c / (BN * 4), 2), row = (c >> 2) & (BN - 1);
+            p_ptr[i] = wplanes + pl * plane_stride + (size_t)min(n0 + row, o.N - 1) * Kp + (((c & 3) ^ ((row >> 2) & 3)) * 8);
+        }
+    } else {
+#pragma unroll
+        for (int p = 0; p < B_PASSES; ++p) b_ptr[p] = wmat + (size_t)min(n0 + arow + 32 * p, o.N - 1) * Kp + acol;
+    }
 
     const int nk_all = Kp / BK;
     const int kt1 = min(nk_all, kt1_in);
@@ -157,10 +165,19 @@
             __builtin_amdgcn_global_load_lds((const __attribute__((address_space(1))) void*)s,
                                              (__attribute__((address_space(3))) void*)(la + i * 32 * BK), 16, 0, 0);
         }
-#pragma unroll
-        for (int p = 0; p < B_PASSES; ++p)
-            __builtin_amdgcn_global_load_lds((const __attribute__((address_space(1))) void*)(b_ptr[p] + kt * BK),
-                                             (__attribute__((address_space(3))) void*)(lb + p * 32 * BK), 16, 0, 0);
+        if constexpr (PRE) {
+            float* lp = sB + buf * B_TILE;
+#pragma unroll
+            for (int i = 0; i < P_PASSES; ++i)
+                if (4 * i + wave < P_DEPOSITS)
+                    __builtin_amdgcn_global_load_lds((const __attribute__((address_space(1))) void*)(p_ptr[i] + kt * BK),
+                                                     (__attribute__((address_space(3))) void*)(lp + (4 * i + wave) * 256), 16, 0, 0);
+        } else {
+#pragma unroll
+            for (int p = 0; p < B_PASSES; ++p)
+                __builtin_amdgcn_global_load_lds((const __attribute__((address_space(1))) void*)(b_ptr[p] + kt * BK),
+                                                 (__attribute__((address_space(3))) void*)(lb + p * 32 * BK), 16, 0, 0);
+        }
     };
 
     f32x16 acc[TM][TN];
@@ -218,10 +235,19 @@
             for (int i = 0; i < TM; ++i)
                 gx3_split8(*reinterpret_cast<const f32x4*>(a + i * 32 * BK + xoff[ss][0]),
                            *reinterpret_cast<const f32x4*>(a + i * 32 * BK + xoff[ss][1]), pa[0][i], pa[1][i], pa[2][i]);
-#pragma unroll
-            for (int n = 0; n < TN; ++n)
-                gx3_split8(*reinterpret_cast<const f32x4*>(b + n * 32 * BK + xoff[ss][0]),
-                           *reinterpret_cast<const f32x4*>(b + n * 32 * BK + xoff[ss][1]), pb[0][n], pb[1][n], pb[2][n]);
+            if constexpr (PRE) {
+                const char* bp = reinterpret_cast<const char*>(sB + buf * B_TILE) + (wn * TN * 32 + l31) * 64 +
+                                 (((2 * ss + hi) ^ ((l31 >> 2) & 3)) * 16);
+#pragma unroll
+                for (int n = 0; n < TN; ++n)
+#pragma unroll
+                    for (int p = 0; p < 3; ++p) pb[p][n] = *reinterpret_cast<const gx3_bf16x8*>(bp + (p * BN + n * 32) * 64);
+            } else {
+#pragma unroll
+                for (int n = 0; n < TN; ++n)
+                    gx3_split8(*reinterpret_cast<const f32x4*>(b + n * 32 * BK + xoff[ss][0]),
+                               *reinterpret_cast<const f32x4*>(b + n * 32 * BK + xoff[ss][1]), pb[0][n], pb[1][n], pb[2][n]);
+            }
         };
         auto mfma_x3 = [&]() {
             constexpr int TA[6] = {0, 1, 0, 2, 1, 0}, TB[6] = {0, 0, 1, 0, 1, 2};
@@ -323,15 +349,17 @@
     else store(std::true_type{});
 }
 
-template <int BM, int BN, int WM, int WN, int TM, int TN, bool X3 = false>
+template <int BM, int BN, int WM, int WN, int TM, int TN, bool PRE = false, bool X3 = false>
 __global__ __launch_bounds__(256) void conv_gemm_kernel(Gather g, const float* __restrict__ wmat, size_t w_class_stride,
                                                              Scatter o, const float* __restrict__ bias, int act, int tiles_n,
                                                              int kt_per_split, size_t part_stride) {
     DWC_PROBE();
     const int cls = blockIdx.z, split = blockIdx.y;
-    conv_gemm_body<BM, BN, WM, WN, TM, TN, X3>(g, wmat + (size_t)cls * w_class_stride, o, bias, act, tiles_n, split * kt_per_split,
-                                           (split + 1) * kt_per_split, (size_t)split * part_stride, part_stride != 0, cls >> 1,
-                                           cls & 1, blockIdx.x, gridDim.x);
+    const size_t plane_stride = (size_t)gridDim.z * o.N * ((g.K + BK - 1) / BK * BK);
+    const unsigned short* planes = reinterpret_cast<const unsigned short*>(wmat + plane_stride) + (size_t)cls * w_class_stride;
+    conv_gemm_body<BM, BN, WM, WN, TM, TN, PRE, X3>(g, wmat + (size_t)cls * w_class_stride, planes, plane_stride, o, bias, act, tiles_n,
+                                                split * kt_per_split, (split + 1) * kt_per_split, (size_t)split * part_stride,
+                                                part_stride != 0, cls >> 1, cls & 1, blockIdx.x, gridDim.x);
 }
 
 template <int BM, int BN, int WM, int WN, int TM, int TN, bool X3 = false>
@@ -339,8 +367,9 @@
     const Strip& s = ss.s[blockIdx.z];
     if ((int)blockIdx.x >= s.tiles) return;
     const int kt0 = s.kt0 + blockIdx.y * ss.kt_per_part;
-    conv_gemm_body<BM, BN, WM, WN, TM, TN, X3>(s.g, (const float*)s.w, s.o, nullptr, DWC_ACT_NONE, s.tiles_n, kt0, min(s.kt1, kt0 + ss.kt_per_part),
-                                           blockIdx.y * ss.part_stride, false, s.oph, s.opw, blockIdx.x, s.tiles);
+    conv_gemm_body<BM, BN, WM, WN, TM, TN, false, X3>(s.g, (const float*)s.w, nullptr, 0, s.o, nullptr, DWC_ACT_NONE, s.tiles_n, kt0,
+                                                  min(s.kt1, kt0 + ss.kt_per_part), blockIdx.y * ss.part_stride, false, s.oph, s.opw,
+                                                  blockIdx.x, s.tiles);
 }
 
 template <int BN, int WM, int WN, int TM, int TN, bool X3 = false>
@@ -537,11 +566,11 @@
 }
 
 
-template <int BM, int BN, int WM, int WN, int TM, int TN, bool X3 = false>
+template <int BM, int BN, int WM, int WN, int TM, int TN, bool PRE = false, bool X3 = false>
 void launch_variant(const Gather& g, const float* w, size_t wcs, int classes, const Scatter& o, const float* bias, int act,
                     const Plan& p, size_t part_stride, hipStream_t st) {
     const int tiles_m = (g.M + BM - 1) / BM, tiles_n = (o.N + BN - 1) / BN;
-    hipLaunchKernelGGL((conv_gemm_kernel<BM, BN, WM, WN, TM, TN, X3>), dim3(tiles_m * tiles_n, p.splits, classes), dim3(256), 0, st,
+    hipLaunchKernelGGL((conv_gemm_kernel<BM, BN, WM, WN, TM, TN, PRE, X3>), dim3(tiles_m * tiles_n, p.splits, classes), dim3(256), 0, st,
                        g, w, wcs, o, bias, act, tiles_n, p.kt_per_split, part_stride);
 }
 
@@ -551,13 +580,15 @@
     if (m < 0) {
         const int a = getenv("DWC_X3_GEMM") ? atoi(getenv("DWC_X3_GEMM")) : 1;
         const int b = getenv("DWC_X3_WGRAD") ? atoi(getenv("DWC_X3_WGRAD")) : 1;
-        m = (a ? 1 : 0) | (b ? 2 : 0);
+        const int c = getenv("DWC_X3_GEMM_PRESPLIT") ? atoi(getenv("DWC_X3_GEMM_PRESPLIT")) : 1;
+        m = (a ? 1 : 0) | (b ? 2 : 0) | (c ? 0 : 4);
         g_x3_mode.store(m, std::memory_order_relaxed);
     }
     return m;
 }
 static bool wgrad_x3_on() { return (x3_mode() & 2) != 0; }
-static bool gemm_x3_on(int K) { return (x3_mode() & 1) != 0 && K >= 128; }
+static bool gemm_x3_on(int K) { return (x3_mode() & 1) != 0 && K >= X3_GEMM_MIN_K; }
+static bool gemm_presplit_on() { return (x3_mode() & 4) == 0; }
 
 struct Im2colF32 {
     typedef float T;
@@ -570,6 +601,7 @@
     static constexpr int IMAGE_GROUPS = 1;
     static constexpr TileCand TILES[] = {{128, 128, 2, 1.0f}, {128, 64, 3, 0.85f}, {64, 64, 5, 0.72f}, {128, 32, 4, 0.5f}};
     static constexpr int SPLIT_BELOW = 2 * NUM_CU;
+    static constexpr int PRESPLIT_MIN_M = 512;
 
     static int launch_gemm(const Gather& g, const float* w, size_t w_class_stride, int classes, Scatter o, const float* bias, int act,
                            size_t dst_elems, void* ws, size_t ws_bytes, hipStream_t st) {
@@ -585,10 +617,14 @@
                 part_stride = dst_elems;
             }
         }
-        if (gemm_x3_on(g.K)) {
-            if (p.bm == 128 && p.bn >= 64) launch_variant<128, 64, 2, 2, 2, 1, true>(g, w, w_class_stride, classes, o, bias, act, p, part_stride, st);
-            else if (p.bm == 64 && p.bn == 64) launch_variant<64, 64, 2, 2, 1, 1, true>(g, w, w_class_stride, classes, o, bias, act, p, part_stride, st);
-            else launch_variant<128, 32, 4, 1, 1, 1, true>(g, w, w_class_stride, classes, o, bias, act, p, part_stride, st);
+        if (gemm_x3_on(g.K) && gemm_presplit_on() && g.M >= PRESPLIT_MIN_M) {
+            if (p.bm == 128 && p.bn >= 64) launch_variant<128, 64, 4, 1, 1, 2, true, true>(g, w, w_class_stride, classes, o, bias, act, p, part_stride, st);
+            else if (p.bm == 64 && p.bn == 64) launch_variant<64, 64, 2, 2, 1, 1, true, true>(g, w, w_class_stride, classes, o, bias, act, p, part_stride, st);
+            else launch_variant<128, 32, 4, 1, 1, 1, true, true>(g, w, w_class_stride, classes, o, bias, act, p, part_stride, st);
+        } else if (gemm_x3_on(g.K)) {
+            if (p.bm == 128 && p.bn >= 64) launch_variant<128, 64, 2, 2, 2, 1, false, true>(g, w, w_class_stride, classes, o, bias, act, p, part_stride, st);
+            else if (p.bm == 64 && p.bn == 64) launch_variant<64, 64, 2, 2, 1, 1, false, true>(g, w, w_class_stride, classes, o, bias, act, p, part_stride, st);
+            else launch_variant<128, 32, 4, 1, 1, 1, false, true>(g, w, w_class_stride, classes, o, bias, act, p, part_stride, st);
         } else if (p.bm == 128 && p.bn == 128) launch_variant<128, 128, 2, 2, 2, 2>(g, w, w_class_stride, classes, o, bias, act, p, part_stride, st);
         else if (p.bm == 128 && p.bn == 64) launch_variant<128, 64, 2, 2, 2, 1>(g, w, w_class_stride, classes, o, bias, act, p, part_stride, st);
         else if (p.bm == 64 && p.bn == 64) launch_variant<64, 64, 2, 2, 1, 1>(g, w, w_class_stride, classes, o, bias, act, p, part_stride, st);
@@ -654,7 +690,7 @@
 
 int dwc_x3_gemm_mode(int mode) {
     const int prev = x3_mode();
-    if (mode >= 0) g_x3_mode.store(mode & 3, std::memory_order_relaxed);
+    if (mode >= 0) g_x3_mode.store(mode & 7, std::memory_order_relaxed);
     return prev;
 }
 
diff --git a/dwc-gan_amd/csrc/conv_im2col_entry.h b/dwc-gan_amd/csrc/conv_im2col_entry.h
--- a/dwc-gan_amd/csrc/conv_im2col_entry.h
+++ b/dwc-gan_amd/csrc/conv_im2col_entry.h
@@ -10,7 +10,7 @@
 
 template <class P>
 size_t im2col_weight_prepared_elems(int Cout, int Cin, int KH, int KW, int stride, int cout_pad, int cin_pad, int for_dgrad) {
-    return weight_prepared_elems(KH, KW, stride, cout_pad, cin_pad, for_dgrad, P::BK);
+    return weight_prepared_elems<typename P::T>(KH, KW, stride, cout_pad, cin_pad, for_dgrad, P::BK);
 }
 
 template <class P>
diff --git a/dwc-gan_amd/csrc/dwc_common.h b/dwc-gan_amd/csrc/dwc_common.h
--- a/dwc-gan_amd/csrc/dwc_common.h
+++ b/dwc-gan_amd/csrc/dwc_common.h
@@ -57,6 +57,20 @@
 __device__ __forceinline__ void stf(float* p, size_t e, const float (&o)[V]) {
 #pragma unroll
     for (int q = 0; q < V / 4; ++q) reinterpret_cast<f32x4*>(p + e)[q] = f32x4{o[4 * q], o[4 * q + 1], o[4 * q + 2], o[4 * q + 3]};
+}
+
+__device__ __forceinline__ void dwc_split3(float v, unsigned& h, unsigned& m, unsigned& l) {
+    h = __float_as_uint(v) & 0xffff0000u;
+    const float r = v - __uint_as_float(h);
+    m = __float_as_uint(r) & 0xffff0000u;
+    l = __float_as_uint(r - __uint_as_float(m));
+}
+__device__ __forceinline__ void dwc_split3_store(unsigned short* planes, size_t n_f32, size_t e, float v) {
+    unsigned h, m, l;
+    dwc_split3(v, h, m, l);
+    planes[e] = (unsigned short)(h >> 16);
+    planes[n_f32 + e] = (unsigned short)(m >> 16);
+    planes[2 * n_f32 + e] = (unsigned short)(l >> 16);
 }
 
 #endif
diff --git a/dwc-gan_amd/csrc/weight_refresh.hip b/dwc-gan_amd/csrc/weight_refresh.hip
--- a/dwc-gan_amd/csrc/weight_refresh.hip
+++ b/dwc-gan_amd/csrc/weight_refresh.hip
@@ -90,8 +90,14 @@
                 h2_planes[base + (size_t)d.rows * 16] = __builtin_bit_cast(unsigned short, l);
                 break;
             }
-            case DWC_REFRESH_FWD_F32: reinterpret_cast<float*>(d.dst)[idx] = im2col_elem(d, idx, false); break;
-            case DWC_REFRESH_DGRAD_F32: reinterpret_cast<float*>(d.dst)[idx] = im2col_elem(d, idx, true); break;
+            case DWC_REFRESH_FWD_F32:
+            case DWC_REFRESH_DGRAD_F32: {
+                const float v = im2col_elem(d, idx, d.kind == DWC_REFRESH_DGRAD_F32);
+                float* o = reinterpret_cast<float*>(d.dst);
+                o[idx] = v;
+                if (d.x3_planes) dwc_split3_store(reinterpret_cast<unsigned short*>(o + d.n_items), d.n_items, idx, v);
+                break;
+            }
             case DWC_REFRESH_FWD_BF16: reinterpret_cast<bf16*>(d.dst)[idx] = (bf16)im2col_elem(d, idx, false); break;
             case DWC_REFRESH_DGRAD_BF16: reinterpret_cast<bf16*>(d.dst)[idx] = (bf16)im2col_elem(d, idx, true); break;
             case DWC_REFRESH_X3_FWD:
@@ -111,15 +117,13 @@
                 } else {
                     if (row < d.Cin && kc < d.Cout) v = d.src[(((size_t)kc * d.Cin + row) * K + (K - 1 - kh)) * K + (K - 1 - kw)];
                 }
-                const unsigned hb = __float_as_uint(v) & 0xffff0000u;
-                const float r1 = v - __uint_as_float(hb);
-                const unsigned mb = __float_as_uint(r1) & 0xffff0000u;
-                const float r2 = r1 - __uint_as_float(mb);
+                unsigned hb, mb, lb;
+                dwc_split3(v, hb, mb, lb);
                 unsigned short* o = reinterpret_cast<unsigned short*>(d.dst);
                 const size_t base = ((size_t)(tap * ncs + cs) * 3 * rows + row) * CS + (j ^ (((row >> 3) & 1) << 3));
                 o[base] = (unsigned short)(hb >> 16);
                 o[base + (size_t)rows * CS] = (unsigned short)(mb >> 16);
-                o[base + 2 * (size_t)rows * CS] = (unsigned short)(__float_as_uint(r2) >> 16);
+                o[base + 2 * (size_t)rows * CS] = (unsigned short)(lb >> 16);
                 break;
             }
             default: break;
diff --git a/dwc-gan_amd/hipdwc/_lib.py b/dwc-gan_amd/hipdwc/_lib.py
--- a/dwc-gan_amd/hipdwc/_lib.py
+++ b/dwc-gan_amd/hipdwc/_lib.py
@@ -196,7 +196,7 @@
     "dwc_src_head_seed": (c_int, [c_fp] * 3 + [c_int] * 3 + [c_fp]),
 }
 
-ABI_VERSION = 9
+ABI_VERSION = 10
 EINVAL = -1
 _ERRORS = {-1: "DWC_EINVAL (unsupported shape/argument)", -2: "DWC_EWORKSPACE (scratch too small)",
            -3: "DWC_ELAUNCH (kernel launch failed)"}
diff --git a/dwc-gan_amd/hipdwc/ops.py b/dwc-gan_amd/hipdwc/ops.py
--- a/dwc-gan_amd/hipdwc/ops.py
+++ b/dwc-gan_amd/hipdwc/ops.py
@@ -354,9 +354,12 @@
                                                               cout_pad, cin_pad, _stream()), "weight_prepare_dgrad")
         rows, kdim = (cin_pad, kh * kw * cout_pad) if stride == 1 else (4 * cin_pad, 4 * cout_pad)
     recipe = None
-    if (not transposed or kh == kw) and n % rows == 0:
-        recipe = _recipe(w, owners, kind=(2 if half else 0) + (kind == "dgrad"), n_items=n, Cout=cout, Cin=cin, KH=kh, KW=kw,
-                         stride=stride, cout_pad=cout_pad, cin_pad=cin_pad, Kp=n // rows, transpose_hw=int(transposed))
+    slab = 64 if half else 32
+    Kp = (kdim + slab - 1) // slab * slab
+    if (not transposed or kh == kw) and n in (rows * Kp, rows * Kp * 5 // 2):
+        recipe = _recipe(w, owners, kind=(2 if half else 0) + (kind == "dgrad"), n_items=rows * Kp, Cout=cout, Cin=cin, KH=kh, KW=kw,
+                         stride=stride, cout_pad=cout_pad, cin_pad=cin_pad, Kp=Kp, transpose_hw=int(transposed),
+                         x3_planes=int(n != rows * Kp))
     ent[key] = (stamp, out, recipe)
     return out
 
@@ -424,7 +427,7 @@
 
 _REFRESH_DT = np.dtype([("src", "<u8"), ("dst", "<u8"), ("n_items", "<u8"), ("kind", "<i4"), ("Cout", "<i4"), ("Cin", "<i4"),
                         ("KH", "<i4"), ("KW", "<i4"), ("stride", "<i4"), ("cout_pad", "<i4"), ("cin_pad", "<i4"), ("Kp", "<i4"),
-                        ("rows", "<i4"), ("kdim", "<i4"), ("transpose_hw", "<i4"), ("reserved", "<i4"), ("tail_pad", "<i4")])
+                        ("rows", "<i4"), ("kdim", "<i4"), ("transpose_hw", "<i4"), ("x3_planes", "<i4"), ("tail_pad", "<i4")])
 assert _REFRESH_DT.itemsize == 80
 REFRESH_CHUNK = 8192
 _REFRESH_TABLES = {}
diff --git a/include/dwcgan_hip.h b/include/dwcgan_hip.h
--- a/include/dwcgan_hip.h
+++ b/include/dwcgan_hip.h
@@ -21,7 +21,7 @@
 #define DWC_ACT_HEADS 5
 #define DWC_ACT_HEADS8 6
 
-#define DWC_ABI_VERSION 9
+#define DWC_ABI_VERSION 10
 int dwc_version(void);
 int dwc_x3_gemm_mode(int mode);
 
@@ -182,7 +182,7 @@
     int Cout, Cin, KH, KW, stride, cout_pad, cin_pad, Kp;
     int rows, kdim;
     int transpose_hw;
-    int reserved;
+    int x3_planes;
 } dwc_refresh_desc;
 int dwc_weight_refresh_multi(const dwc_refresh_desc* descs_dev, const int* chunk_desc_dev, const unsigned* chunk_start_dev,
                              int n_chunks, int has_h2, unsigned epoch, void* stream);
```

Result: no change. 398.9 images/s (median of 5 runs) (+0.2%).
